# MCG-NJU/MeMOTR

Hardware: AMD Instinct MI355X
Metric: train_frames_per_sec (higher is better)
Workload: dtype f32

## Files before the change

include/clip_ops_hip.h:

```cpp
#ifndef CLIP_OPS_HIP_H
#define CLIP_OPS_HIP_H

#include <stdint.h>

#ifdef __cplusplus
extern "C" {
#endif

#define CLIPOPS_ABI_VERSION 12

int clipops_abi_version(void);
const char *clipops_last_error(void);

int clipops_match_cost_f32(const float *logits, long logit_sl, long logit_sq, const float *boxes, long box_sl,
                           long box_sq, const int64_t *gt_labels, const float *gt_boxes, int n_layers, int Q, int K,
                           int T, float w_class, float w_bbox, float w_giou, float *cost, void *stream);

int clipops_pair_box_loss_fwd_f32(const float *boxes, const int64_t *lay, const int64_t *qidx, long row_mul,
                                  long row_add, const float *tgt_boxes, const int64_t *gidx, const float *weight,
                                  int n, float *l1, float *giou_loss, void *stream);
int clipops_pair_box_loss_bwd_f32(const float *boxes, const int64_t *lay, const int64_t *qidx, long row_mul,
                                  long row_add, const float *tgt_boxes, const int64_t *gidx, const float *weight,
                                  int n, const float *grad_l1, const float *grad_giou, float *grad_boxes,
                                  void *stream);

int clipops_pair_iou_f32(const float *boxes, const float *tgt_boxes, const int64_t *gidx, int n, float *iou,
                         void *stream);

int clipops_track_ownership_i64(const int64_t *track_ids, int n_tracks, const int64_t *gt_ids, int n_gt,
                                int64_t *matched_idx, float *gt_free, void *stream);
int clipops_focal_labels_i64(const int64_t *lay, const int64_t *q, const int64_t *g, int n_pairs,
                             const int64_t *gt_labels, int n_gt, const int64_t *matched_idx, int n_tracks,
                             const uint8_t *late, int n_layers, int n_det, int K, int64_t *labels, void *stream);

int clipops_focal_fwd_f32(const float *logits, long sl, long sq, const int64_t *labels, int n_layers, int Nq, int K,
                          float alpha, float gamma, float *loss, void *stream);
int clipops_focal_bwd_f32(const float *logits, long sl, long sq, const int64_t *labels, int n_layers, int Nq, int K,
                          float alpha, float gamma, const float *grad_loss, float *grad_logits, void *stream);

int clipops_sine_embed_fwd_f32(const float *pos, const float *dim_t, long n, int K, int F, float scale, float *out,
                               void *stream);
int clipops_sine_embed_bwd_f32(const float *pos, const float *dim_t, long n, int K, int F, float scale,
                               const float *grad_out, float *grad_pos, void *stream);

int clipops_inverse_sigmoid_fwd_f32(const float *x, long n, float eps, float *y, void *stream);
int clipops_inverse_sigmoid_bwd_f32(const float *x, const float *grad_y, long n, float eps, float *grad_x, void *stream);

int clipops_refine_boxes_fwd_f32(const float *delta, const float *ref, long n, float eps, float *out, void *stream);
int clipops_refine_boxes_bwd_f32(const float *out, const float *ref, const float *grad_out, long n, float eps,
                                 float *grad_delta, float *grad_ref, void *stream);

int clipops_refine_boxes_split_fwd_f32(const float *delta, const float *ref, long n_rows, float eps,
                                       float *out_head, float *out_dec, void *stream);

int clipops_colsum_f32(const float *x, long rows, int cols, float *out, void *stream);
int clipops_colsum_partial_f32(const float *x, long rows, int cols, int chunk_rows, float *partial, void *stream);
int clipops_colsum_partial_bf16(const uint16_t *x, long rows, int cols, int chunk_rows, float *partial, void *stream);

#define CLIPOPS_MHA_MAX_L 512
int clipops_mha_fwd_f32(const float *q, const float *k, const float *v, long q_bs, long q_rs, long k_bs, long k_rs,
                        long v_bs, long v_rs, const uint8_t *key_mask, int B, int H, int L, float scale, float *out,
                        float *lse, void *stream);
int clipops_mha_bwd_f32(const float *q, const float *k, const float *v, long q_bs, long q_rs, long k_bs, long k_rs,
                        long v_bs, long v_rs, const uint8_t *key_mask, const float *out, const float *lse,
                        const float *grad_out, int B, int H, int L, float scale, float *grad_q, long gq_bs, long gq_rs,
                        float *grad_k, long gk_bs, long gk_rs, float *grad_v, long gv_bs, long gv_rs, void *stream);

#define CLIPOPS_LN_COLS 256
int clipops_add_layer_norm_fwd_f32(const float *x, const float *res, const float *gamma, const float *beta, long rows,
                                   float eps, float *sum, float *y, float *stats, void *stream);
int clipops_add_layer_norm_bwd_f32(const float *grad_y, const float *sum, const float *stats, const float *gamma,
                                   long rows, int chunk_rows, float *grad_sum, float *partial, void *stream);

int clipops_add_layer_norm_pos_fwd_f32(const float *x, const float *res, const float *gamma, const float *beta,
                                       const float *pos, long rows, float eps, float *sum, float *y, float *q,
                                       float *stats, void *stream);
int clipops_add_layer_norm_fanin_bwd_f32(const float *g0, const float *g1, const float *g2, const float *sum,
                                         const float *stats, const float *gamma, long rows, int chunk_rows,
                                         float *grad_sum, float *partial, float *colsum_partial, void *stream);

#define CLIPOPS_ASSIGN_MAX_DIM 2048
int clipops_assign_f32(const float *cost, long stride_problem, long stride_row, long stride_col, int n_problems,
                       int n_rows, int n_cols, int32_t *row_ind, int32_t *col_ind, int32_t *status, void *stream);

int clipops_shift_relu_f32(float *x, const float *shift, const float *res, long planes, int C, long HW, void *stream);
int clipops_shift_relu_bf16(uint16_t *x, const float *shift, const uint16_t *res, long planes, int C, long HW,
                            void *stream);

int clipops_linear_bwd_f32(const float *grad_y, const float *y_relu, const float *x, const float *w, int rows,
                           int in_features, int out_features, float *grad_x, float *grad_w, float *grad_b,
                           void *stream);

int clipops_linear_fwd_f32(const float *x, const float *w, const float *bias, int rows, int in_features,
                           int out_features, int relu, float *y, void *stream);

int clipops_relu_bwd_colsum_partial_f32(const float *g, const float *y, long rows, int cols, int chunk_rows, float *g2,
                                        float *partial, void *stream);

int clipops_result_rows_f32(const float *boxes, const float *scores, const int64_t *ids, const int64_t *labels, int n,
                            int K, int64_t frame, float ori_w, float ori_h, float score_thresh, float area_thresh,
                            float *rows_f, int64_t *rows_i, int32_t *counters, int capacity, void *stream);

#ifdef __cplusplus
}
#endif
#endif
```

memotr_amd/_clip_lib.py:

```python
from __future__ import annotations

import ctypes

from . import _cabi

LIB_PATH = _cabi.lib_path("libclip_ops_hip.so")

ABI_VERSION = 12

c_int, c_long, c_float, c_void_p = ctypes.c_int, ctypes.c_long, ctypes.c_float, ctypes.c_void_p

_PAIR = [c_void_p, c_void_p, c_void_p, c_long, c_long, c_void_p, c_void_p, c_void_p, c_int]
_FOCAL = [c_void_p, c_long, c_long, c_void_p, c_int, c_int, c_int, c_float, c_float]

SYMBOLS = {
    "clipops_abi_version": ([], c_int),
    "clipops_last_error": ([], ctypes.c_char_p),
    "clipops_match_cost_f32": ([c_void_p, c_long, c_long, c_void_p, c_long, c_long, c_void_p, c_void_p] + [c_int] * 4 +
                               [c_float] * 3 + [c_void_p, c_void_p], c_int),
    "clipops_pair_box_loss_fwd_f32": (_PAIR + [c_void_p, c_void_p, c_void_p], c_int),
    "clipops_pair_box_loss_bwd_f32": (_PAIR + [c_void_p, c_void_p, c_void_p, c_void_p], c_int),
    "clipops_pair_iou_f32": ([c_void_p, c_void_p, c_void_p, c_int, c_void_p, c_void_p], c_int),
    "clipops_track_ownership_i64": ([c_void_p, c_int, c_void_p, c_int, c_void_p, c_void_p, c_void_p], c_int),
    "clipops_focal_labels_i64": ([c_void_p, c_void_p, c_void_p, c_int, c_void_p, c_int, c_void_p, c_int, c_void_p, c_int,
                                  c_int, c_int, c_void_p, c_void_p], c_int),
    "clipops_focal_fwd_f32": (_FOCAL + [c_void_p, c_void_p], c_int),
    "clipops_focal_bwd_f32": (_FOCAL + [c_void_p, c_void_p, c_void_p], c_int),
    "clipops_colsum_f32": ([c_void_p, c_long, c_int, c_void_p, c_void_p], c_int),
    "clipops_colsum_partial_f32": ([c_void_p, c_long, c_int, c_int, c_void_p, c_void_p], c_int),
    "clipops_colsum_partial_bf16": ([c_void_p, c_long, c_int, c_int, c_void_p, c_void_p], c_int),
    "clipops_assign_f32": ([c_void_p, c_long, c_long, c_long, c_int, c_int, c_int, c_void_p, c_void_p, c_void_p,
                            c_void_p], c_int),
    "clipops_mha_fwd_f32": ([c_void_p] * 3 + [c_long] * 6 + [c_void_p] + [c_int] * 3 + [c_float, c_void_p, c_void_p,
                                                                                          c_void_p], c_int),
    "clipops_mha_bwd_f32": ([c_void_p] * 3 + [c_long] * 6 + [c_void_p] * 4 + [c_int] * 3 + [c_float] +
                            [c_void_p, c_long, c_long] * 3 + [c_void_p], c_int),
    "clipops_add_layer_norm_fwd_f32": ([c_void_p] * 4 + [c_long, c_float] + [c_void_p] * 4, c_int),
    "clipops_add_layer_norm_bwd_f32": ([c_void_p] * 4 + [c_long, c_int] + [c_void_p] * 3, c_int),
    "clipops_add_layer_norm_pos_fwd_f32": ([c_void_p] * 5 + [c_long, c_float] + [c_void_p] * 5, c_int),
    "clipops_add_layer_norm_fanin_bwd_f32": ([c_void_p] * 6 + [c_long, c_int] + [c_void_p] * 4, c_int),
    "clipops_sine_embed_fwd_f32": ([c_void_p, c_void_p, c_long, c_int, c_int, c_float, c_void_p, c_void_p], c_int),
    "clipops_sine_embed_bwd_f32": ([c_void_p, c_void_p, c_long, c_int, c_int, c_float, c_void_p, c_void_p, c_void_p],
                                   c_int),
    "clipops_inverse_sigmoid_fwd_f32": ([c_void_p, c_long, c_float, c_void_p, c_void_p], c_int),
    "clipops_inverse_sigmoid_bwd_f32": ([c_void_p, c_void_p, c_long, c_float, c_void_p, c_void_p], c_int),
    "clipops_refine_boxes_fwd_f32": ([c_void_p, c_void_p, c_long, c_float, c_void_p, c_void_p], c_int),
    "clipops_linear_bwd_f32": ([c_void_p] * 4 + [c_int] * 3 + [c_void_p] * 4, c_int),
    "clipops_linear_fwd_f32": ([c_void_p] * 3 + [c_int] * 4 + [c_void_p, c_void_p], c_int),
    "clipops_relu_bwd_colsum_partial_f32": ([c_void_p, c_void_p, c_long, c_int, c_int, c_void_p, c_void_p, c_void_p], c_int),
    "clipops_shift_relu_f32": ([c_void_p, c_void_p, c_void_p, c_long, c_int, c_long, c_void_p], c_int),
    "clipops_shift_relu_bf16": ([c_void_p, c_void_p, c_void_p, c_long, c_int, c_long, c_void_p], c_int),
    "clipops_refine_boxes_bwd_f32": ([c_void_p, c_void_p, c_void_p, c_long, c_float, c_void_p, c_void_p, c_void_p],
                                     c_int),
    "clipops_refine_boxes_split_fwd_f32": ([c_void_p, c_void_p, c_long, c_float, c_void_p, c_void_p, c_void_p], c_int),
    "clipops_result_rows_f32": ([c_void_p] * 4 + [c_int, c_int, ctypes.c_int64] + [c_float] * 4 + [c_void_p] * 3 +
                                [c_int, c_void_p], c_int),
}


lib, check = _cabi.bind("libclip_ops_hip.so", "clipops", SYMBOLS, ABI_VERSION)
```

memotr_amd/csrc/clip_ops.hip:

```cpp
#include <hip/hip_runtime.h>
#include <stdint.h>
#include <stdio.h>

#include <atomic>

#include "../../include/clip_ops_hip.h"
#include "assign_core.h"

namespace {

thread_local char g_err[256] = {0};

int fail(int code, const char *msg) {
    snprintf(g_err, sizeof(g_err), "%s", msg);
    return code;
}

int check_launch(const char *what) {
    const hipError_t e = hipGetLastError();
    if (e != hipSuccess) {
        snprintf(g_err, sizeof(g_err), "%s: %s", what, hipGetErrorString(e));
        return (int)e;
    }
    g_err[0] = 0;
    return 0;
}

typedef float f32x4_t __attribute__((ext_vector_type(4)));
typedef double f64x4_t __attribute__((ext_vector_type(4)));

struct Box {
    float x1, y1, x2, y2;
};

__device__ __forceinline__ Box to_xyxy(float cx, float cy, float w, float h) {
#pragma clang fp contract(off)
    Box b;
    b.x1 = cx - 0.5f * w;
    b.y1 = cy - 0.5f * h;
    b.x2 = cx + 0.5f * w;
    b.y2 = cy + 0.5f * h;
    return b;
}

__device__ __forceinline__ float giou_pair(const Box a, const Box b) {
#pragma clang fp contract(off)
    const float iw = fmaxf(fminf(a.x2, b.x2) - fmaxf(a.x1, b.x1), 0.f);
    const float ih = fmaxf(fminf(a.y2, b.y2) - fmaxf(a.y1, b.y1), 0.f);
    const float inter = iw * ih;
    const float area_a = (a.x2 - a.x1) * (a.y2 - a.y1);
    const float area_b = (b.x2 - b.x1) * (b.y2 - b.y1);
    const float uni = area_a + area_b - inter;
    const float iou = inter / uni;
    const float hw = fmaxf(fmaxf(a.x2, b.x2) - fminf(a.x1, b.x1), 0.f);
    const float hh = fmaxf(fmaxf(a.y2, b.y2) - fminf(a.y1, b.y1), 0.f);
    const float hull = hw * hh;
    return iou - (hull - uni) / hull;
}

__device__ __forceinline__ float sigmoidf(float x) { return 1.f / (1.f + expf(-x)); }

__device__ __forceinline__ float powg(float x, float gamma) { return gamma == 2.f ? x * x : powf(x, gamma); }

__global__ __launch_bounds__(256) void match_cost_kernel(const float *__restrict__ logits, long lsl, long lsq,
                                                        const float *__restrict__ boxes, long bsl, long bsq,
                                                        const int64_t *__restrict__ gt_labels,
                                                        const float *__restrict__ gt_boxes, int n_layers, int Q,
                                                        int K, int T, float w_class, float w_bbox, float w_giou,
                                                        float *__restrict__ cost) {
#pragma clang fp contract(off)
    const long total = (long)n_layers * Q * T;
    for (long i = (long)blockIdx.x * blockDim.x + threadIdx.x; i < total; i += (long)gridDim.x * blockDim.x) {
        const int t = (int)(i % T);
        const long lq = i / T;
        const int q = (int)(lq % Q), l = (int)(lq / Q);
        long lab = gt_labels[t];
        lab = lab < 0 ? 0 : (lab >= K ? K - 1 : lab);
        const float prob = sigmoidf(logits[l * lsl + q * lsq + lab]);
        const float alpha = 0.25f, gamma = 2.f;
        const float neg = ((1.f - alpha) * powg(prob, gamma)) * (-logf(1.f - prob + 1e-8f));
        const float pos = (alpha * powg(1.f - prob, gamma)) * (-logf(prob + 1e-8f));
        const float c_class = pos - neg;
        const float *pb = boxes + l * bsl + q * bsq;
        const float *tb = gt_boxes + (long)t * 4;
        const float p0 = pb[0], p1 = pb[1], p2 = pb[2], p3 = pb[3];
        const float t0 = tb[0], t1 = tb[1], t2 = tb[2], t3 = tb[3];
        const float c_bbox = ((fabsf(p0 - t0) + fabsf(p1 - t1)) + fabsf(p2 - t2)) + fabsf(p3 - t3);
        const float giou = giou_pair(to_xyxy(p0, p1, p2, p3), to_xyxy(t0, t1, t2, t3));
        cost[i] = (w_bbox * c_bbox + w_class * c_class) + w_giou * (-giou);
    }
}

__global__ __launch_bounds__(256) void pair_box_loss_fwd_kernel(const float *__restrict__ boxes,
                                                               const int64_t *__restrict__ lay,
                                                               const int64_t *__restrict__ qidx, long row_mul,
                                                               long row_add, const float *__restrict__ tgt,
                                                               const int64_t *__restrict__ gidx,
                                                               const float *__restrict__ weight, int n,
                                                               float *__restrict__ l1, float *__restrict__ gl) {
#pragma clang fp contract(off)
    const int i = blockIdx.x * blockDim.x + threadIdx.x;
    if (i >= n) return;
    const float *pb = boxes + (lay[i] * row_mul + row_add + qidx[i]) * 4;
    const float *tb = tgt + (gidx ? gidx[i] : (long)i) * 4;
    const float p0 = pb[0], p1 = pb[1], p2 = pb[2], p3 = pb[3];
    const float t0 = tb[0], t1 = tb[1], t2 = tb[2], t3 = tb[3];
    float a = ((fabsf(p0 - t0) + fabsf(p1 - t1)) + fabsf(p2 - t2)) + fabsf(p3 - t3);
    float g = 1.f - giou_pair(to_xyxy(p0, p1, p2, p3), to_xyxy(t0, t1, t2, t3));
    if (weight) {
        a *= weight[i];
        g *= weight[i];
    }
    l1[i] = a;
    gl[i] = g;
}

__global__ __launch_bounds__(256) void pair_iou_kernel(const float *__restrict__ boxes, const float *__restrict__ tgt,
                                                      const int64_t *__restrict__ gidx, int n,
                                                      float *__restrict__ iou) {
#pragma clang fp contract(off)
    const int i = blockIdx.x * blockDim.x + threadIdx.x;
    if (i >= n) return;
    const float *pb = boxes + (long)i * 4;
    const float *tb = tgt + (gidx ? gidx[i] : (long)i) * 4;
    const Box a = to_xyxy(pb[0], pb[1], pb[2], pb[3]), b = to_xyxy(tb[0], tb[1], tb[2], tb[3]);
    const float iw = fmaxf(fminf(a.x2, b.x2) - fmaxf(a.x1, b.x1), 0.f);
    const float ih = fmaxf(fminf(a.y2, b.y2) - fmaxf(a.y1, b.y1), 0.f);
    const float inter = iw * ih;
    const float uni = (a.x2 - a.x1) * (a.y2 - a.y1) + (b.x2 - b.x1) * (b.y2 - b.y1) - inter;
    iou[i] = inter / uni;
}

__device__ __forceinline__ float dmax_a(float a, float b) { return a > b ? 1.f : (a == b ? 0.5f : 0.f); }
__device__ __forceinline__ float dmin_a(float a, float b) { return a < b ? 1.f : (a == b ? 0.5f : 0.f); }
__device__ __forceinline__ float sgn(float x) { return x > 0.f ? 1.f : (x < 0.f ? -1.f : 0.f); }

__global__ __launch_bounds__(256) void pair_box_loss_bwd_kernel(const float *__restrict__ boxes,
                                                               const int64_t *__restrict__ lay,
                                                               const int64_t *__restrict__ qidx, long row_mul,
                                                               long row_add, const float *__restrict__ tgt,
                                                               const int64_t *__restrict__ gidx,
                                                               const float *__restrict__ weight, int n,
                                                               const float *__restrict__ g_l1,
                                                               const float *__restrict__ g_gl,
                                                               float *__restrict__ grad_boxes) {
    const int i = blockIdx.x * blockDim.x + threadIdx.x;
    if (i >= n) return;
    const long row = lay[i] * row_mul + row_add + qidx[i];
    const float *pb = boxes + row * 4;
    const float *tb = tgt + (gidx ? gidx[i] : (long)i) * 4;
    const float p0 = pb[0], p1 = pb[1], p2 = pb[2], p3 = pb[3];
    const float t0 = tb[0], t1 = tb[1], t2 = tb[2], t3 = tb[3];
    const float w = weight ? weight[i] : 1.f;
    const float ga = g_l1[i] * w;
    const float gg = -g_gl[i] * w;
    const Box a = to_xyxy(p0, p1, p2, p3), b = to_xyxy(t0, t1, t2, t3);
    const float ltx = fmaxf(a.x1, b.x1), lty = fmaxf(a.y1, b.y1), rbx = fminf(a.x2, b.x2), rby = fminf(a.y2, b.y2);
    const float dw = rbx - ltx, dh = rby - lty;
    const float iw = fmaxf(dw, 0.f), ih = fmaxf(dh, 0.f);
    const float inter = iw * ih;
    const float aw = a.x2 - a.x1, ah = a.y2 - a.y1;
    const float area_a = aw * ah, area_b = (b.x2 - b.x1) * (b.y2 - b.y1);
    const float uni = area_a + area_b - inter;
    const float hx1 = fminf(a.x1, b.x1), hy1 = fminf(a.y1, b.y1), hx2 = fmaxf(a.x2, b.x2), hy2 = fmaxf(a.y2, b.y2);
    const float ew = hx2 - hx1, eh = hy2 - hy1;
    const float hw = fmaxf(ew, 0.f), hh = fmaxf(eh, 0.f);
    const float hull = hw * hh;
    const float g_inter0 = gg / uni;
    const float g_uni = gg * (-inter / (uni * uni)) + gg / hull;
    const float g_hull = gg * (-(uni / (hull * hull)));
    const float g_inter = g_inter0 - g_uni;
    const float g_area_a = g_uni;
    const float g_dw = g_inter * ih * (dw >= 0.f ? 1.f : 0.f), g_dh = g_inter * iw * (dh >= 0.f ? 1.f : 0.f);
    const float g_ew = g_hull * hh * (ew >= 0.f ? 1.f : 0.f), g_eh = g_hull * hw * (eh >= 0.f ? 1.f : 0.f);
    float gx1 = -g_dw * dmax_a(a.x1, b.x1) - g_ew * dmin_a(a.x1, b.x1) - g_area_a * ah;
    float gy1 = -g_dh * dmax_a(a.y1, b.y1) - g_eh * dmin_a(a.y1, b.y1) - g_area_a * aw;
    float gx2 = g_dw * dmin_a(a.x2, b.x2) + g_ew * dmax_a(a.x2, b.x2) + g_area_a * ah;
    float gy2 = g_dh * dmin_a(a.y2, b.y2) + g_eh * dmax_a(a.y2, b.y2) + g_area_a * aw;
    float *go = grad_boxes + row * 4;
    go[0] = (gx1 + gx2) + ga * sgn(p0 - t0);
    go[1] = (gy1 + gy2) + ga * sgn(p1 - t1);
    go[2] = 0.5f * (gx2 - gx1) + ga * sgn(p2 - t2);
    go[3] = 0.5f * (gy2 - gy1) + ga * sgn(p3 - t3);
}

struct Focal {
    float loss, dloss;
};

__device__ __forceinline__ Focal focal_elem(float x, bool is_pos, float alpha, float gamma) {
    const float p = sigmoidf(x);
    const float ce = fmaxf(x, 0.f) - (is_pos ? x : 0.f) + log1pf(expf(-fabsf(x)));
    const float p_t = is_pos ? p : 1.f - p;
    const float q = 1.f - p_t;
    const float a_t = alpha >= 0.f ? (is_pos ? alpha : 1.f - alpha) : 1.f;
    const float mod = powg(q, gamma);
    Focal f;
    f.loss = a_t * (ce * mod);
    const float qg1 = gamma == 2.f ? q : (gamma == 0.f ? 0.f : powf(q, gamma - 1.f));
    const float d = a_t * (gamma * qg1 * (p_t * q) * ce + mod * q);
    f.dloss = is_pos ? -d : d;
    return f;
}

__global__ __launch_bounds__(256) void focal_fwd_kernel(const float *__restrict__ logits, long sl, long sq,
                                                       const int64_t *__restrict__ labels, int Nq, int K, float alpha,
                                                       float gamma, float *__restrict__ loss) {
    __shared__ float s_part[256];
    const int l = blockIdx.x;
    const int total = Nq * K;
    float acc = 0.f;
    for (int i = threadIdx.x; i < total; i += 256) {
        const int q = i / K, k = i - q * K;
        const float x = logits[l * sl + q * sq + k];
        acc += focal_elem(x, labels[(long)l * Nq + q] == k, alpha, gamma).loss;
    }
    s_part[threadIdx.x] = acc;
    __syncthreads();
    for (int o = 128; o > 0; o >>= 1) {
        if (threadIdx.x < o) s_part[threadIdx.x] += s_part[threadIdx.x + o];
        __syncthreads();
    }
    if (threadIdx.x == 0) loss[l] = s_part[0] / (float)K;
}

__global__ __launch_bounds__(256) void focal_bwd_kernel(const float *__restrict__ logits, long sl, long sq,
                                                       const int64_t *__restrict__ labels, int n_layers, int Nq,
                                                       int K, float alpha, float gamma,
                                                       const float *__restrict__ g_loss,
                                                       float *__restrict__ grad_logits) {
    const long total = (long)n_layers * Nq * K;
    for (long i = (long)blockIdx.x * blockDim.x + threadIdx.x; i < total; i += (long)gridDim.x * blockDim.x) {
        const int k = (int)(i % K);
        const long lq = i / K;
        const int q = (int)(lq % Nq), l = (int)(lq / Nq);
        const float x = logits[l * sl + q * sq + k];
        const Focal f = focal_elem(x, labels[lq] == k, alpha, gamma);
        grad_logits[i] = (g_loss[l] / (float)K) * f.dloss;
    }
}

__global__ __launch_bounds__(256) void sine_embed_fwd_kernel(const float *__restrict__ pos,
                                                            const float *__restrict__ dim_t, long n, int K, int F,
                                                            float scale, float *__restrict__ out) {
#pragma clang fp contract(off)
    const long total = n * K * F;
    for (long i = (long)blockIdx.x * blockDim.x + threadIdx.x; i < total; i += (long)gridDim.x * blockDim.x) {
        const int j = (int)(i % F);
        const long ik = i / F;
        const float e = (pos[ik] * scale) / dim_t[j];
        out[i] = (j & 1) ? cosf(e) : sinf(e);
    }
}

__global__ __launch_bounds__(256) void sine_embed_bwd_kernel(const float *__restrict__ pos,
                                                            const float *__restrict__ dim_t, long n, int K, int F,
                                                            float scale, const float *__restrict__ g,
                                                            float *__restrict__ gpos) {
    const int lane = threadIdx.x & 63;
    const long waves = ((long)gridDim.x * blockDim.x) >> 6;
    for (long ik = ((long)blockIdx.x * blockDim.x + threadIdx.x) >> 6; ik < n * K; ik += waves) {
        const float ps = pos[ik] * scale;
        float acc = 0.f;
        for (int j = lane; j < F; j += 64) {
            const float e = ps / dim_t[j];
            const float d = (j & 1) ? -sinf(e) : cosf(e);
            acc += (g[ik * F + j] * d) / dim_t[j];
        }
#pragma unroll
        for (int o = 32; o > 0; o >>= 1) acc += __shfl_xor(acc, o, 64);
        if (lane == 0) gpos[ik] = acc * scale;
    }
}

__device__ __forceinline__ float clamp_keep_nan(float x, float lo, float hi) { return x < lo ? lo : (x > hi ? hi : x); }

__device__ __forceinline__ float inv_sigmoid(float x, float eps) {
    return logf(clamp_keep_nan(x, eps, 1.f) / clamp_keep_nan(1.f - x, eps, 1.f));
}

__device__ __forceinline__ float inv_sigmoid_grad(float x, float eps) {
    const float u = 1.f - x;
    const float x1 = clamp_keep_nan(x, eps, 1.f), x2 = clamp_keep_nan(u, eps, 1.f);
    const float a = (x >= eps && x <= 1.f) ? 1.f / x1 : 0.f;
    const float b = (u >= eps && u <= 1.f) ? 1.f / x2 : 0.f;
    return a + b;
}

__global__ __launch_bounds__(256) void inverse_sigmoid_fwd_kernel(const float *__restrict__ x, long n, float eps,
                                                                 float *__restrict__ y) {
    for (long i = (long)blockIdx.x * blockDim.x + threadIdx.x; i < n; i += (long)gridDim.x * blockDim.x)
        y[i] = inv_sigmoid(x[i], eps);
}

__global__ __launch_bounds__(256) void inverse_sigmoid_bwd_kernel(const float *__restrict__ x,
                                                                 const float *__restrict__ g, long n, float eps,
                                                                 float *__restrict__ gx) {
    for (long i = (long)blockIdx.x * blockDim.x + threadIdx.x; i < n; i += (long)gridDim.x * blockDim.x)
        gx[i] = g[i] * inv_sigmoid_grad(x[i], eps);
}

__global__ __launch_bounds__(256) void refine_boxes_fwd_kernel(const float *__restrict__ delta,
                                                              const float *__restrict__ ref, long n, float eps,
                                                              float *__restrict__ out) {
    for (long i = (long)blockIdx.x * blockDim.x + threadIdx.x; i < n; i += (long)gridDim.x * blockDim.x)
        out[i] = sigmoidf(delta[i] + inv_sigmoid(ref[i], eps));
}

template <bool VEC>
__global__ __launch_bounds__(256) void refine_boxes_split_fwd_kernel(const float *__restrict__ delta,
                                                                    const float *__restrict__ ref, long n_rows,
                                                                    float eps, float *__restrict__ head,
                                                                    float *__restrict__ dec) {
    for (long r = (long)blockIdx.x * blockDim.x + threadIdx.x; r < n_rows; r += (long)gridDim.x * blockDim.x) {
        float4 d, f;
        if (VEC) {
            d = reinterpret_cast<const float4 *>(delta)[r];
            f = reinterpret_cast<const float4 *>(ref)[r];
        } else {
            d = make_float4(delta[4 * r], delta[4 * r + 1], delta[4 * r + 2], delta[4 * r + 3]);
            f = make_float4(ref[4 * r], ref[4 * r + 1], ref[4 * r + 2], ref[4 * r + 3]);
        }
        float4 h, c;
        h.x = sigmoidf(d.x + inv_sigmoid(f.x, eps));
        h.y = sigmoidf(d.y + inv_sigmoid(f.y, eps));
        h.z = sigmoidf(d.z + inv_sigmoid(f.z, eps));
        h.w = sigmoidf(d.w + inv_sigmoid(f.w, eps));
        c.x = h.x;
        c.y = h.y;
        c.z = sigmoidf(d.z);
        c.w = sigmoidf(d.w);
        if (VEC) {
            reinterpret_cast<float4 *>(head)[r] = h;
            reinterpret_cast<float4 *>(dec)[r] = c;
        } else {
            head[4 * r] = h.x; head[4 * r + 1] = h.y; head[4 * r + 2] = h.z; head[4 * r + 3] = h.w;
            dec[4 * r] = c.x; dec[4 * r + 1] = c.y; dec[4 * r + 2] = c.z; dec[4 * r + 3] = c.w;
        }
    }
}

__global__ __launch_bounds__(256) void refine_boxes_bwd_kernel(const float *__restrict__ out,
                                                              const float *__restrict__ ref,
                                                              const float *__restrict__ g, long n, float eps,
                                                              float *__restrict__ gdelta, float *__restrict__ gref) {
    for (long i = (long)blockIdx.x * blockDim.x + threadIdx.x; i < n; i += (long)gridDim.x * blockDim.x) {
        const float y = out[i];
        const float gs = (g[i] * (1.f - y)) * y;
        gdelta[i] = gs;
        if (gref) gref[i] = gs * inv_sigmoid_grad(ref[i], eps);
    }
}

__global__ __launch_bounds__(256) void colsum_kernel(const float *__restrict__ x, long rows, int cols,
                                                    float *__restrict__ out) {
    __shared__ double s_part[8][33];
    const int tx = threadIdx.x & 31, ty = threadIdx.x >> 5;
    const int c = blockIdx.x * 32 + tx;
    double a0 = 0., a1 = 0., a2 = 0., a3 = 0.;
    if (c < cols) {
        long r = ty;
        for (; r + 24 < rows; r += 32) {
            a0 += x[r * cols + c];
            a1 += x[(r + 8) * cols + c];
            a2 += x[(r + 16) * cols + c];
            a3 += x[(r + 24) * cols + c];
        }
        for (; r < rows; r += 8) a0 += x[r * cols + c];
    }
    s_part[ty][tx] = (a0 + a1) + (a2 + a3);
    __syncthreads();
    if (ty == 0 && c < cols) {
        double t = s_part[0][tx];
#pragma unroll
        for (int i = 1; i < 8; ++i) t += s_part[i][tx];
        out[c] = (float)t;
    }
}

__global__ __launch_bounds__(256) void colsum_quad_kernel(const float *__restrict__ x, long rows, int cols,
                                                         float *__restrict__ out) {
    __shared__ f64x4_t s_w[4];
    const int c = blockIdx.x * 4;
    f64x4_t a = {0., 0., 0., 0.};
    for (long r = threadIdx.x; r < rows; r += 256) {
        const f32x4_t v = *reinterpret_cast<const f32x4_t *>(x + r * cols + c);
        a.x += v.x; a.y += v.y; a.z += v.z; a.w += v.w;
    }
#pragma unroll
    for (int o = 32; o > 0; o >>= 1) {
        a.x += __shfl_xor(a.x, o, 64);
        a.y += __shfl_xor(a.y, o, 64);
        a.z += __shfl_xor(a.z, o, 64);
        a.w += __shfl_xor(a.w, o, 64);
    }
    if ((threadIdx.x & 63) == 0) s_w[threadIdx.x >> 6] = a;
    __syncthreads();
    if (threadIdx.x == 0) {
        const f64x4_t t = (s_w[0] + s_w[1]) + (s_w[2] + s_w[3]);
        const f32x4_t r = {(float)t.x, (float)t.y, (float)t.z, (float)t.w};
        *reinterpret_cast<f32x4_t *>(out + c) = r;
    }
}

__device__ __forceinline__ float colsum_ld(const float *x, long i) { return x[i]; }
__device__ __forceinline__ float colsum_ld(const uint16_t *x, long i) {
    return __uint_as_float(((unsigned)x[i]) << 16);
}

template <typename TX>
__global__ __launch_bounds__(256) void colsum_partial_kernel(const TX *__restrict__ x, long rows, int cols,
                                                            int chunk_rows, float *__restrict__ partial) {
    __shared__ double s_part[8][33];
    const int tx = threadIdx.x & 31, ty = threadIdx.x >> 5;
    const int c = blockIdx.x * 32 + tx;
    const long r0 = (long)blockIdx.y * chunk_rows;
    const long r1 = r0 + chunk_rows < rows ? r0 + chunk_rows : rows;
    double a0 = 0., a1 = 0., a2 = 0., a3 = 0.;
    if (c < cols) {
        long r = r0 + ty;
        for (; r + 24 < r1; r += 32) {
            a0 += colsum_ld(x, r * cols + c);
            a1 += colsum_ld(x, (r + 8) * cols + c);
            a2 += colsum_ld(x, (r + 16) * cols + c);
            a3 += colsum_ld(x, (r + 24) * cols + c);
        }
        for (; r < r1; r += 8) a0 += colsum_ld(x, r * cols + c);
    }
    s_part[ty][tx] = (a0 + a1) + (a2 + a3);
    __syncthreads();
    if (ty == 0 && c < cols) {
        double t = s_part[0][tx];
#pragma unroll
        for (int i = 1; i < 8; ++i) t += s_part[i][tx];
        partial[(long)blockIdx.y * cols + c] = (float)t;
    }
}

__device__ __forceinline__ void colsum_st(float *x, long i, float v) { x[i] = v; }

template <typename TX>
__global__ __launch_bounds__(256) void relu_bwd_colsum_partial_kernel(const TX *__restrict__ g, const TX *__restrict__ y,
                                                                     long rows, int cols, int chunk_rows,
                                                                     TX *__restrict__ g2, float *__restrict__ partial) {
    __shared__ double s_part[8][33];
    const int tx = threadIdx.x & 31, ty = threadIdx.x >> 5;
    const int c = blockIdx.x * 32 + tx;
    const long r0 = (long)blockIdx.y * chunk_rows;
    const long r1 = r0 + chunk_rows < rows ? r0 + chunk_rows : rows;
    double a0 = 0., a1 = 0., a2 = 0., a3 = 0.;
    if (c < cols) {
        long r = r0 + ty;
        for (; r + 24 < r1; r += 32) {
            const long i0 = r * cols + c, i1 = (r + 8) * cols + c, i2 = (r + 16) * cols + c, i3 = (r + 24) * cols + c;
            const float v0 = colsum_ld(y, i0) <= 0.f ? 0.f : colsum_ld(g, i0);
            const float v1 = colsum_ld(y, i1) <= 0.f ? 0.f : colsum_ld(g, i1);
            const float v2 = colsum_ld(y, i2) <= 0.f ? 0.f : colsum_ld(g, i2);
            const float v3 = colsum_ld(y, i3) <= 0.f ? 0.f : colsum_ld(g, i3);
            colsum_st(g2, i0, v0); colsum_st(g2, i1, v1); colsum_st(g2, i2, v2); colsum_st(g2, i3, v3);
            a0 += v0; a1 += v1; a2 += v2; a3 += v3;
        }
        for (; r < r1; r += 8) {
            const long i0 = r * cols + c;
            const float v0 = colsum_ld(y, i0) <= 0.f ? 0.f : colsum_ld(g, i0);
            colsum_st(g2, i0, v0);
            a0 += v0;
        }
    }
    s_part[ty][tx] = (a0 + a1) + (a2 + a3);
    __syncthreads();
    if (ty == 0 && c < cols) {
        double t = s_part[0][tx];
#pragma unroll
        for (int i = 1; i < 8; ++i) t += s_part[i][tx];
        partial[(long)blockIdx.y * cols + c] = (float)t;
    }
}

constexpr int kLanes = 16;
constexpr int kRows = 256 / kLanes;
constexpr int kHd = 32;
constexpr int kPitch = 36;

__device__ __forceinline__ void load_row32(const float *p, float *r) {
#pragma unroll
    for (int i = 0; i < 8; ++i) {
        const f32x4_t v = *reinterpret_cast<const f32x4_t *>(p + 4 * i);
        r[4 * i] = v.x; r[4 * i + 1] = v.y; r[4 * i + 2] = v.z; r[4 * i + 3] = v.w;
    }
}

__device__ __forceinline__ float dot32(const float *a, const float *lds_row) {
    float s0 = 0.f, s1 = 0.f;
#pragma unroll
    for (int i = 0; i < 8; ++i) {
        const f32x4_t v = *reinterpret_cast<const f32x4_t *>(lds_row + 4 * i);
        s0 = fmaf(a[4 * i], v.x, s0);
        s1 = fmaf(a[4 * i + 1], v.y, s1);
        s0 = fmaf(a[4 * i + 2], v.z, s0);
        s1 = fmaf(a[4 * i + 3], v.w, s1);
    }
    return s0 + s1;
}

__device__ __forceinline__ float dot32r(const float *a, const float *b) {
    float s0 = 0.f, s1 = 0.f;
#pragma unroll
    for (int i = 0; i < 8; ++i) {
        s0 = fmaf(a[4 * i], b[4 * i], s0);
        s1 = fmaf(a[4 * i + 1], b[4 * i + 1], s1);
        s0 = fmaf(a[4 * i + 2], b[4 * i + 2], s0);
        s1 = fmaf(a[4 * i + 3], b[4 * i + 3], s1);
    }
    return s0 + s1;
}

__device__ __forceinline__ void axpy32(float *acc, float w, const float *lds_row) {
#pragma unroll
    for (int i = 0; i < 8; ++i) {
        const f32x4_t v = *reinterpret_cast<const f32x4_t *>(lds_row + 4 * i);
        acc[4 * i] = fmaf(w, v.x, acc[4 * i]);
        acc[4 * i + 1] = fmaf(w, v.y, acc[4 * i + 1]);
        acc[4 * i + 2] = fmaf(w, v.z, acc[4 * i + 2]);
        acc[4 * i + 3] = fmaf(w, v.w, acc[4 * i + 3]);
    }
}

__device__ __forceinline__ float sum8l(float x) {
#pragma unroll
    for (int o = 1; o < kLanes; o <<= 1) x += __shfl_xor(x, o, 64);
    return x;
}
__device__ __forceinline__ float max8l(float x) {
#pragma unroll
    for (int o = 1; o < kLanes; o <<= 1) x = fmaxf(x, __shfl_xor(x, o, 64));
    return x;
}

__device__ __forceinline__ void stage_rows(float *dst, const float *src, long rs, int L) {
    for (int i = threadIdx.x; i < L * 8; i += blockDim.x) {
        const int r = i >> 3, c = (i & 7) * 4;
        *reinterpret_cast<f32x4_t *>(dst + r * kPitch + c) = *reinterpret_cast<const f32x4_t *>(src + r * rs + c);
    }
}

__global__ __launch_bounds__(256) void mha_fwd_kernel(const float *__restrict__ q, const float *__restrict__ k,
                                                     const float *__restrict__ v, long q_bs, long q_rs, long k_bs,
                                                     long k_rs, long v_bs, long v_rs,
                                                     const uint8_t *__restrict__ key_mask, int H, int L, float scale,
                                                     float *__restrict__ out, float *__restrict__ lse) {
    extern __shared__ __attribute__((aligned(16))) float s_mem[];
    float *Ks = s_mem, *Vs = s_mem + (size_t)L * kPitch;
    const int h = blockIdx.y, b = blockIdx.z;
    stage_rows(Ks, k + b * k_bs + h * kHd, k_rs, L);
    stage_rows(Vs, v + b * v_bs + h * kHd, v_rs, L);
    __syncthreads();
    const int row = blockIdx.x * kRows + threadIdx.x / kLanes, sub = threadIdx.x % kLanes;
    const bool row_ok = row < L;
    const int rowc = row_ok ? row : L - 1;
    float qr[kHd];
    load_row32(q + b * q_bs + rowc * q_rs + h * kHd, qr);
#pragma unroll
    for (int i = 0; i < kHd; ++i) qr[i] *= scale;
    const uint8_t *mk = key_mask ? key_mask + (long)b * L : nullptr;
    float m = -INFINITY, l = 0.f, acc[kHd];
#pragma unroll
    for (int i = 0; i < kHd; ++i) acc[i] = 0.f;
    for (int j = sub; j < L; j += kLanes) {
        if (mk && mk[j]) continue;
        const float s = dot32(qr, Ks + j * kPitch);
        const float m_new = fmaxf(m, s);
        const float corr = expf(m - m_new), p = expf(s - m_new);
        l = l * corr + p;
#pragma unroll
        for (int i = 0; i < kHd; ++i) acc[i] *= corr;
        axpy32(acc, p, Vs + j * kPitch);
        m = m_new;
    }
    const float M = max8l(m);
    const float w = (m == -INFINITY) ? 0.f : expf(m - M);
    const float Lsum = sum8l(l * w);
    const float inv = 1.f / Lsum;
    float *o = out + ((long)b * L + rowc) * (H * kHd) + h * kHd;
#pragma unroll
    for (int i = 0; i < kHd; ++i) {
        const float t = sum8l(acc[i] * w) * inv;
        if (row_ok && (i >> 2) == sub) o[i] = t;
    }
    if (row_ok && sub == 0) lse[((long)b * H + h) * L + row] = M + logf(Lsum);
}

__global__ __launch_bounds__(256) void mha_bwd_q_kernel(const float *__restrict__ q, const float *__restrict__ k,
                                                       const float *__restrict__ v, long q_bs, long q_rs, long k_bs,
                                                       long k_rs, long v_bs, long v_rs,
                                                       const uint8_t *__restrict__ key_mask,
                                                       const float *__restrict__ out, const float *__restrict__ lse,
                                                       const float *__restrict__ go, int H, int L, float scale,
                                                       float *__restrict__ gq, long gq_bs, long gq_rs) {
    extern __shared__ __attribute__((aligned(16))) float s_mem[];
    float *Ks = s_mem, *Vs = s_mem + (size_t)L * kPitch;
    const int h = blockIdx.y, b = blockIdx.z;
    stage_rows(Ks, k + b * k_bs + h * kHd, k_rs, L);
    stage_rows(Vs, v + b * v_bs + h * kHd, v_rs, L);
    __syncthreads();
    const int row = blockIdx.x * kRows + threadIdx.x / kLanes, sub = threadIdx.x % kLanes;
    const bool row_ok = row < L;
    const int rowc = row_ok ? row : L - 1;
    float qr[kHd], gr[kHd], acc[kHd];
    load_row32(q + b * q_bs + rowc * q_rs + h * kHd, qr);
    const long orow = ((long)b * L + rowc) * (H * kHd) + h * kHd;
    load_row32(go + orow, gr);
    float D = 0.f;
    {
        float orr[kHd];
        load_row32(out + orow, orr);
        D = dot32r(gr, orr);
    }
#pragma unroll
    for (int i = 0; i < kHd; ++i) { qr[i] *= scale; acc[i] = 0.f; }
    const float ls = lse[((long)b * H + h) * L + rowc];
    const uint8_t *mk = key_mask ? key_mask + (long)b * L : nullptr;
    for (int j = sub; j < L; j += kLanes) {
        if (mk && mk[j]) continue;
        const float p = expf(dot32(qr, Ks + j * kPitch) - ls);
        const float ds = p * (dot32(gr, Vs + j * kPitch) - D);
        axpy32(acc, ds, Ks + j * kPitch);
    }
    float *g = gq + b * gq_bs + rowc * gq_rs + h * kHd;
#pragma unroll
    for (int i = 0; i < kHd; ++i) {
        const float t = sum8l(acc[i]) * scale;
        if (row_ok && (i >> 2) == sub) g[i] = t;
    }
}

__global__ __launch_bounds__(256) void mha_bwd_kv_kernel(const float *__restrict__ q, const float *__restrict__ k,
                                                        const float *__restrict__ v, long q_bs, long q_rs, long k_bs,
                                                        long k_rs, long v_bs, long v_rs,
                                                        const uint8_t *__restrict__ key_mask,
                                                        const float *__restrict__ out, const float *__restrict__ lse,
                                                        const float *__restrict__ go, int H, int L, float scale,
                                                        float *__restrict__ gk, long gk_bs, long gk_rs,
                                                        float *__restrict__ gv, long gv_bs, long gv_rs) {
    extern __shared__ __attribute__((aligned(16))) float s_mem[];
    float *Qs = s_mem, *Gs = s_mem + (size_t)L * kPitch;
    float *s_lse = Gs + (size_t)L * kPitch, *s_D = s_lse + L;
    const int h = blockIdx.y, b = blockIdx.z;
    stage_rows(Qs, q + b * q_bs + h * kHd, q_rs, L);
    for (int i = threadIdx.x; i < L * 8; i += blockDim.x) {
        f32x4_t *p4 = reinterpret_cast<f32x4_t *>(Qs + (i >> 3) * kPitch + (i & 7) * 4);
        *p4 = *p4 * scale;
    }
    stage_rows(Gs, go + (long)b * L * (H * kHd) + h * kHd, (long)H * kHd, L);
    for (int i = threadIdx.x; i < L; i += blockDim.x) s_lse[i] = lse[((long)b * H + h) * L + i];
    __syncthreads();
    for (int i = threadIdx.x; i < L; i += blockDim.x) {
        const float *o = out + ((long)b * L + i) * (H * kHd) + h * kHd;
        float orr[kHd];
        load_row32(o, orr);
        s_D[i] = dot32(orr, Gs + i * kPitch);
    }
    __syncthreads();
    const int row = blockIdx.x * kRows + threadIdx.x / kLanes, sub = threadIdx.x % kLanes;
    const bool row_ok = row < L;
    const int rowc = row_ok ? row : L - 1;
    const bool dead = key_mask && key_mask[(long)b * L + rowc];
    float kr[kHd], vr[kHd], ak[kHd], av[kHd];
    load_row32(k + b * k_bs + rowc * k_rs + h * kHd, kr);
    load_row32(v + b * v_bs + rowc * v_rs + h * kHd, vr);
#pragma unroll
    for (int i = 0; i < kHd; ++i) { ak[i] = 0.f; av[i] = 0.f; }
    if (!dead) {
        for (int i = sub; i < L; i += kLanes) {
            const float p = expf(dot32(kr, Qs + i * kPitch) - s_lse[i]);
            const float ds = p * (dot32(vr, Gs + i * kPitch) - s_D[i]);
            axpy32(av, p, Gs + i * kPitch);
            axpy32(ak, ds, Qs + i * kPitch);
        }
    }
    float *pk = gk + b * gk_bs + rowc * gk_rs + h * kHd, *pv = gv + b * gv_bs + rowc * gv_rs + h * kHd;
#pragma unroll
    for (int i = 0; i < kHd; ++i) {
        const float tk = sum8l(ak[i]), tv = sum8l(av[i]);
        if (row_ok && (i >> 2) == sub) {
            pk[i] = tk;
            pv[i] = tv;
        }
    }
}

int allow_lds(const void *kernel, size_t lds, std::atomic<unsigned long long> &done) {
    if (lds <= 64 * 1024) return 0;
    int dev = 0;
    (void)hipGetDevice(&dev);
    const unsigned long long bit = 1ull << (dev & 63);
    if (done.load(std::memory_order_acquire) & bit) return 0;
    const hipError_t e = hipFuncSetAttribute(kernel, hipFuncAttributeMaxDynamicSharedMemorySize, 160 * 1024 - 2048);
    if (e != hipSuccess) {
        snprintf(g_err, sizeof(g_err), "hipFuncSetAttribute: %s", hipGetErrorString(e));
        return (int)e;
    }
    done.fetch_or(bit, std::memory_order_release);
    return 0;
}

std::atomic<unsigned long long> g_lds_fwd{0}, g_lds_bq{0}, g_lds_bkv{0};

int mha_check(const void *q, const void *k, const void *v, int B, int H, int L) {
    if (B < 0 || H <= 0 || L < 0) return fail(1, "clipops_mha: bad dimension");
    if (L > CLIPOPS_MHA_MAX_L) return fail(2, "clipops_mha: L exceeds CLIPOPS_MHA_MAX_L");
    if ((long)B * L > 0 && (!q || !k || !v)) return fail(1, "clipops_mha: null pointer");
    return 0;
}

__device__ __forceinline__ float wave_sum64(float x) {
#pragma unroll
    for (int o = 32; o > 0; o >>= 1) x += __shfl_xor(x, o, 64);
    return x;
}

template <bool WITH_Q>
__global__ __launch_bounds__(256) void add_layer_norm_fwd_kernel(const float *__restrict__ x,
                                                                const float *__restrict__ res,
                                                                const float *__restrict__ gamma,
                                                                const float *__restrict__ beta,
                                                                const float *__restrict__ pos, long rows, float eps,
                                                                float *__restrict__ sum, float *__restrict__ y,
                                                                float *__restrict__ q, float *__restrict__ stats) {
    const int lane = threadIdx.x & 63;
    const long row = (long)blockIdx.x * 4 + (threadIdx.x >> 6);
    if (row >= rows) return;
    const long off = row * CLIPOPS_LN_COLS + lane * 4;
    const f32x4_t a = *reinterpret_cast<const f32x4_t *>(x + off);
    const f32x4_t b = *reinterpret_cast<const f32x4_t *>(res + off);
    const f32x4_t s = a + b;
    *reinterpret_cast<f32x4_t *>(sum + off) = s;
    const float mean = wave_sum64((s.x + s.y) + (s.z + s.w)) * (1.f / CLIPOPS_LN_COLS);
    const f32x4_t d = s - mean;
    const float var = wave_sum64((d.x * d.x + d.y * d.y) + (d.z * d.z + d.w * d.w)) * (1.f / CLIPOPS_LN_COLS);
    const float rstd = rsqrtf(var + eps);
    const f32x4_t g = *reinterpret_cast<const f32x4_t *>(gamma + lane * 4);
    const f32x4_t be = *reinterpret_cast<const f32x4_t *>(beta + lane * 4);
    const f32x4_t yv = (d * rstd) * g + be;
    *reinterpret_cast<f32x4_t *>(y + off) = yv;
    if (WITH_Q) *reinterpret_cast<f32x4_t *>(q + off) = yv + *reinterpret_cast<const f32x4_t *>(pos + off);
    if (lane == 0) {
        stats[2 * row] = mean;
        stats[2 * row + 1] = rstd;
    }
}

__global__ __launch_bounds__(256) void add_layer_norm_bwd_kernel(const float *__restrict__ gy,
                                                                const float *__restrict__ sum,
                                                                const float *__restrict__ stats,
                                                                const float *__restrict__ gamma, long rows,
                                                                int chunk_rows, float *__restrict__ gsum,
                                                                float *__restrict__ partial) {
    __shared__ f32x4_t s_acc[4][2][64];
    const int lane = threadIdx.x & 63, wave = threadIdx.x >> 6;
    const f32x4_t gm = *reinterpret_cast<const f32x4_t *>(gamma + lane * 4);
    f32x4_t acc_g = {0.f, 0.f, 0.f, 0.f}, acc_b = {0.f, 0.f, 0.f, 0.f};
    const long r0 = (long)blockIdx.x * chunk_rows;
    const long r1 = r0 + chunk_rows < rows ? r0 + chunk_rows : rows;
    for (long row = r0 + wave; row < r1; row += 4) {
        const long off = row * CLIPOPS_LN_COLS + lane * 4;
        const f32x4_t g = *reinterpret_cast<const f32x4_t *>(gy + off);
        const f32x4_t s = *reinterpret_cast<const f32x4_t *>(sum + off);
        const float mean = stats[2 * row], rstd = stats[2 * row + 1];
        const f32x4_t xh = (s - mean) * rstd;
        const f32x4_t gh = g * gm;
        const float c1 = wave_sum64((gh.x + gh.y) + (gh.z + gh.w)) * (1.f / CLIPOPS_LN_COLS);
        const float c2 = wave_sum64((gh.x * xh.x + gh.y * xh.y) + (gh.z * xh.z + gh.w * xh.w)) * (1.f / CLIPOPS_LN_COLS);
        *reinterpret_cast<f32x4_t *>(gsum + off) = (gh - c1 - xh * c2) * rstd;
        acc_g += g * xh;
        acc_b += g;
    }
    s_acc[wave][0][lane] = acc_g;
    s_acc[wave][1][lane] = acc_b;
    __syncthreads();
    if (wave < 2) {
        const f32x4_t t = (s_acc[0][wave][lane] + s_acc[1][wave][lane]) + (s_acc[2][wave][lane] + s_acc[3][wave][lane]);
        *reinterpret_cast<f32x4_t *>(partial + (long)blockIdx.x * 2 * CLIPOPS_LN_COLS + wave * CLIPOPS_LN_COLS + lane * 4) = t;
    }
}

__global__ __launch_bounds__(256) void add_layer_norm_bwd_fanin_kernel(const float *__restrict__ ga,
                                                                      const float *__restrict__ gb,
                                                                      const float *__restrict__ gc,
                                                                      const float *__restrict__ sum,
                                                                      const float *__restrict__ stats,
                                                                      const float *__restrict__ gamma, long rows,
                                                                      int chunk_rows, float *__restrict__ gsum,
                                                                      float *__restrict__ partial,
                                                                      float *__restrict__ zpartial) {
    __shared__ f32x4_t s_acc[4][2][64];
    __shared__ f64x4_t s_z[4][64];
    const int lane = threadIdx.x & 63, wave = threadIdx.x >> 6;
    const f32x4_t gm = *reinterpret_cast<const f32x4_t *>(gamma + lane * 4);
    f32x4_t acc_g = {0.f, 0.f, 0.f, 0.f}, acc_b = {0.f, 0.f, 0.f, 0.f};
    f64x4_t acc_z = {0., 0., 0., 0.};
    const long r0 = (long)blockIdx.x * chunk_rows;
    const long r1 = r0 + chunk_rows < rows ? r0 + chunk_rows : rows;
    for (long row = r0 + wave; row < r1; row += 4) {
        const long off = row * CLIPOPS_LN_COLS + lane * 4;
        f32x4_t g = *reinterpret_cast<const f32x4_t *>(ga + off);
        if (gb) g += *reinterpret_cast<const f32x4_t *>(gb + off);
        if (gc) g += *reinterpret_cast<const f32x4_t *>(gc + off);
        const f32x4_t s = *reinterpret_cast<const f32x4_t *>(sum + off);
        const float mean = stats[2 * row], rstd = stats[2 * row + 1];
        const f32x4_t xh = (s - mean) * rstd;
        const f32x4_t gh = g * gm;
        const float c1 = wave_sum64((gh.x + gh.y) + (gh.z + gh.w)) * (1.f / CLIPOPS_LN_COLS);
        const float c2 = wave_sum64((gh.x * xh.x + gh.y * xh.y) + (gh.z * xh.z + gh.w * xh.w)) * (1.f / CLIPOPS_LN_COLS);
        const f32x4_t dz = (gh - c1 - xh * c2) * rstd;
        *reinterpret_cast<f32x4_t *>(gsum + off) = dz;
        acc_g += g * xh;
        acc_b += g;
        acc_z.x += dz.x; acc_z.y += dz.y; acc_z.z += dz.z; acc_z.w += dz.w;
    }
    s_acc[wave][0][lane] = acc_g;
    s_acc[wave][1][lane] = acc_b;
    s_z[wave][lane] = acc_z;
    __syncthreads();
    if (wave < 2) {
        const f32x4_t t = (s_acc[0][wave][lane] + s_acc[1][wave][lane]) + (s_acc[2][wave][lane] + s_acc[3][wave][lane]);
        *reinterpret_cast<f32x4_t *>(partial + (long)blockIdx.x * 2 * CLIPOPS_LN_COLS + wave * CLIPOPS_LN_COLS + lane * 4) = t;
    } else if (wave == 2) {
        const f64x4_t t = (s_z[0][lane] + s_z[1][lane]) + (s_z[2][lane] + s_z[3][lane]);
        const f32x4_t hi = {(float)t.x, (float)t.y, (float)t.z, (float)t.w};
        const f32x4_t lo = {(float)(t.x - (double)hi.x), (float)(t.y - (double)hi.y), (float)(t.z - (double)hi.z),
                            (float)(t.w - (double)hi.w)};
        float *zp = zpartial + (long)blockIdx.x * 2 * CLIPOPS_LN_COLS + lane * 4;
        *reinterpret_cast<f32x4_t *>(zp) = hi;
        *reinterpret_cast<f32x4_t *>(zp + CLIPOPS_LN_COLS) = lo;
    }
}

using assign::WaveLanes;

__global__ __launch_bounds__(64) void assign_kernel(const float *__restrict__ cost, long stride_p, long stride_r,
                                                    long stride_c, int n_rows, int n_cols,
                                                    int32_t *__restrict__ row_ind, int32_t *__restrict__ col_ind,
                                                    int32_t *__restrict__ status) {
#pragma clang fp contract(off)
    extern __shared__ __attribute__((aligned(16))) unsigned char s_assign[];
    const long p = blockIdx.x;
    const int k = n_rows < n_cols ? n_rows : n_cols;
    const WaveLanes lanes{(int)threadIdx.x};
    const int rc = assign::solve_problem(lanes, cost + p * stride_p, stride_r, stride_c, n_rows, n_cols, s_assign,
                                         row_ind + p * k, col_ind + p * k);
    if (threadIdx.x == 0 && status != nullptr) status[p] = rc;
}

int grid_for(long total) {
    long g = (total + 255) / 256;
    if (g < 1) g = 1;
    return (int)(g > 4096 ? 4096 : g);
}


__device__ __forceinline__ float sr_bf16(uint16_t h) { return __uint_as_float((unsigned)h << 16); }
__device__ __forceinline__ uint16_t sr_to_bf16(float f) {
    unsigned u = __float_as_uint(f);
    if ((u & 0x7fffffffu) > 0x7f800000u) return (uint16_t)((u >> 16) | 0x40u);
    return (uint16_t)((u + 0x7fffu + ((u >> 16) & 1u)) >> 16);
}

template <bool RES>
__global__ __launch_bounds__(256) void shift_relu_f32_kernel(float *__restrict__ x, const float *__restrict__ shift,
                                                             const float *__restrict__ res, long planes, int C, long HW,
                                                             int vec) {
    for (long plane = blockIdx.y; plane < planes; plane += gridDim.y) {
        const float b = shift[plane % C];
        float *xp = x + plane * HW;
        const float *rp = RES ? res + plane * HW : nullptr;
        if (vec) {
            const long n4 = HW >> 2;
            for (long i = (long)blockIdx.x * blockDim.x + threadIdx.x; i < n4; i += (long)gridDim.x * blockDim.x) {
                float4 v = reinterpret_cast<float4 *>(xp)[i];
                if (RES) {
                    const float4 r = reinterpret_cast<const float4 *>(rp)[i];
                    v.x = (v.x + b) + r.x; v.y = (v.y + b) + r.y; v.z = (v.z + b) + r.z; v.w = (v.w + b) + r.w;
                } else {
                    v.x += b; v.y += b; v.z += b; v.w += b;
                }
                v.x = v.x < 0.f ? 0.f : v.x; v.y = v.y < 0.f ? 0.f : v.y;
                v.z = v.z < 0.f ? 0.f : v.z; v.w = v.w < 0.f ? 0.f : v.w;
                reinterpret_cast<float4 *>(xp)[i] = v;
            }
        } else {
            for (long i = (long)blockIdx.x * blockDim.x + threadIdx.x; i < HW; i += (long)gridDim.x * blockDim.x) {
                float v = xp[i] + b;
                if (RES) v += rp[i];
                xp[i] = v < 0.f ? 0.f : v;
            }
        }
    }
}

template <bool RES>
__global__ __launch_bounds__(256) void shift_relu_bf16_kernel(uint16_t *__restrict__ x, const float *__restrict__ shift,
                                                              const uint16_t *__restrict__ res, long planes, int C,
                                                              long HW, int vec) {
    for (long plane = blockIdx.y; plane < planes; plane += gridDim.y) {
        const float b = sr_bf16(sr_to_bf16(shift[plane % C]));
        uint16_t *xp = x + plane * HW;
        const uint16_t *rp = RES ? res + plane * HW : nullptr;
        if (vec) {
            const long n8 = HW >> 3;
            for (long i = (long)blockIdx.x * blockDim.x + threadIdx.x; i < n8; i += (long)gridDim.x * blockDim.x) {
                uint4 v = reinterpret_cast<uint4 *>(xp)[i];
                uint4 r = {0u, 0u, 0u, 0u};
                if (RES) r = reinterpret_cast<const uint4 *>(rp)[i];
                unsigned *vw = reinterpret_cast<unsigned *>(&v);
                const unsigned *rw = reinterpret_cast<const unsigned *>(&r);
#pragma unroll
                for (int k = 0; k < 4; ++k) {
                    float lo = sr_bf16((uint16_t)(vw[k] & 0xffffu)) + b, hi = sr_bf16((uint16_t)(vw[k] >> 16)) + b;
                    if (RES) {
                        lo = sr_bf16(sr_to_bf16(lo)) + sr_bf16((uint16_t)(rw[k] & 0xffffu));
                        hi = sr_bf16(sr_to_bf16(hi)) + sr_bf16((uint16_t)(rw[k] >> 16));
                    }
                    lo = lo < 0.f ? 0.f : lo;
                    hi = hi < 0.f ? 0.f : hi;
                    vw[k] = (unsigned)sr_to_bf16(lo) | ((unsigned)sr_to_bf16(hi) << 16);
                }
                reinterpret_cast<uint4 *>(xp)[i] = v;
            }
        } else {
            for (long i = (long)blockIdx.x * blockDim.x + threadIdx.x; i < HW; i += (long)gridDim.x * blockDim.x) {
                float v = sr_bf16(xp[i]) + b;
                if (RES) v = sr_bf16(sr_to_bf16(v)) + sr_bf16(rp[i]);
                xp[i] = sr_to_bf16(v < 0.f ? 0.f : v);
            }
        }
    }
}


typedef float lb_f32x16 __attribute__((ext_vector_type(16)));

#ifndef MSDA_LB_U
#define MSDA_LB_U 4
#endif
constexpr int LB_U = MSDA_LB_U;

template <bool GX, bool RELU>
__device__ __forceinline__ void linear_bwd_tile(const float *__restrict__ g, const float *__restrict__ y,
                                                const float *__restrict__ Bp, int M, int N, int K, int OUT, int i0, int j0,
                                                float *__restrict__ C, float *__restrict__ gb, float (*s_c)[16][64],
                                                float (*s_b)[32]) {
    const int lane = threadIdx.x & 63, wave = threadIdx.x >> 6;
    const int i = i0 + (lane & 31), j = j0 + (lane & 31), kq = (lane >> 5) * 4;
    const bool iok = i < M, jok = j < N;
    const int chunks = (K + 7) / 8, per = (chunks + 3) / 4;
    const int c_lo = wave * per, c_hi = (c_lo + per) < chunks ? (c_lo + per) : chunks;
    const bool vec = GX && (OUT % 4 == 0);
    lb_f32x16 acc = {0.f, 0.f, 0.f, 0.f, 0.f, 0.f, 0.f, 0.f, 0.f, 0.f, 0.f, 0.f, 0.f, 0.f, 0.f, 0.f};
    float bsum = 0.f;
    for (int c = c_lo; c < c_hi; c += LB_U) {
        float a[LB_U][4], b[LB_U][4], m[LB_U][4];
#pragma unroll
        for (int u = 0; u < LB_U; ++u) {
            const int k0 = (c + u) * 8 + kq;
            const bool cok = c + u < c_hi;
            if (vec) {
                float4 av = {0.f, 0.f, 0.f, 0.f}, mv = {1.f, 1.f, 1.f, 1.f};
                if (cok && iok && k0 < K) {
                    av = *reinterpret_cast<const float4 *>(g + (long)i * OUT + k0);
                    if (RELU) mv = *reinterpret_cast<const float4 *>(y + (long)i * OUT + k0);
                }
                a[u][0] = av.x; a[u][1] = av.y; a[u][2] = av.z; a[u][3] = av.w;
                m[u][0] = mv.x; m[u][1] = mv.y; m[u][2] = mv.z; m[u][3] = mv.w;
            }
#pragma unroll
            for (int q = 0; q < 4; ++q) {
                const int k = k0 + q;
                const bool kok = cok && k < K;
                if (!vec) {
                    const long idx = GX ? (long)i * OUT + k : (long)k * OUT + i;
                    a[u][q] = (iok && kok) ? g[idx] : 0.f;
                    m[u][q] = (RELU && iok && kok) ? y[idx] : 1.f;
                }
                b[u][q] = (jok && kok) ? Bp[(long)k * N + j] : 0.f;
            }
        }
#pragma unroll
        for (int u = 0; u < LB_U; ++u) {
#pragma unroll
            for (int q = 0; q < 4; ++q) {
                const float av = RELU ? (m[u][q] <= 0.f ? 0.f : a[u][q]) : a[u][q];
                acc = __builtin_amdgcn_mfma_f32_32x32x2f32(av, b[u][q], acc, 0, 0, 0);
                bsum += av;
            }
        }
    }
#pragma unroll
    for (int r = 0; r < 16; ++r) s_c[wave][r][lane] = acc[r];
    bsum += __shfl_xor(bsum, 32, 64);
    if (lane < 32) s_b[wave][lane] = bsum;
    __syncthreads();
#pragma unroll
    for (int rr = 0; rr < 4; ++rr) {
        const int r = wave * 4 + rr;
        const float v = (s_c[0][r][lane] + s_c[1][r][lane]) + (s_c[2][r][lane] + s_c[3][r][lane]);
        const int row = i0 + (r & 3) + 8 * (r >> 2) + 4 * (lane >> 5);
        if (row < M && jok) C[(long)row * N + j] = v;
    }
    if (!GX && gb != nullptr && j0 == 0 && wave == 0 && lane < 32 && i0 + lane < M)
        gb[i0 + lane] = (s_b[0][lane] + s_b[1][lane]) + (s_b[2][lane] + s_b[3][lane]);
}

template <bool RELU>
__global__ __launch_bounds__(256) void linear_bwd_kernel(const float *__restrict__ g, const float *__restrict__ y,
                                                         const float *__restrict__ x, const float *__restrict__ w,
                                                         int R, int IN, int OUT, float *__restrict__ gx,
                                                         float *__restrict__ gw, float *__restrict__ gb, int n_gx,
                                                         int gx_tj, int gw_tj) {
    __shared__ float s_c[4][16][64];
    __shared__ float s_b[4][32];
    const int tile = blockIdx.x;
    if (tile < n_gx) {
        linear_bwd_tile<true, RELU>(g, y, w, R, IN, OUT, OUT, (tile / gx_tj) * 32, (tile % gx_tj) * 32, gx, nullptr, s_c, s_b);
    } else {
        const int t = tile - n_gx;
        linear_bwd_tile<false, RELU>(g, y, x, OUT, IN, R, OUT, (t / gw_tj) * 32, (t % gw_tj) * 32, gw, gb, s_c, s_b);
    }
}

template <bool RELU>
__global__ __launch_bounds__(256) void linear_fwd_kernel(const float *__restrict__ x, const float *__restrict__ w,
                                                         const float *__restrict__ bias, int R, int IN, int OUT,
                                                         float *__restrict__ yout, int tj) {
    __shared__ float s_c[4][16][64];
    const int lane = threadIdx.x & 63, wave = threadIdx.x >> 6;
    const int i0 = (blockIdx.x / tj) * 32, j0 = (blockIdx.x % tj) * 32;
    const int i = i0 + (lane & 31), j = j0 + (lane & 31), kq = (lane >> 5) * 4;
    const bool iok = i < R, jok = j < OUT;
    const int chunks = (IN + 7) / 8, per = (chunks + 3) / 4;
    const int c_lo = wave * per, c_hi = (c_lo + per) < chunks ? (c_lo + per) : chunks;
    lb_f32x16 acc = {0.f, 0.f, 0.f, 0.f, 0.f, 0.f, 0.f, 0.f, 0.f, 0.f, 0.f, 0.f, 0.f, 0.f, 0.f, 0.f};
    for (int c = c_lo; c < c_hi; c += LB_U) {
        float4 a[LB_U], b[LB_U];
#pragma unroll
        for (int u = 0; u < LB_U; ++u) {
            const int k0 = (c + u) * 8 + kq;
            const bool kok = c + u < c_hi && k0 < IN;
            a[u] = (iok && kok) ? *reinterpret_cast<const float4 *>(x + (long)i * IN + k0) : float4{0.f, 0.f, 0.f, 0.f};
            b[u] = (jok && kok) ? *reinterpret_cast<const float4 *>(w + (long)j * IN + k0) : float4{0.f, 0.f, 0.f, 0.f};
        }
#pragma unroll
        for (int u = 0; u < LB_U; ++u) {
            acc = __builtin_amdgcn_mfma_f32_32x32x2f32(a[u].x, b[u].x, acc, 0, 0, 0);
            acc = __builtin_amdgcn_mfma_f32_32x32x2f32(a[u].y, b[u].y, acc, 0, 0, 0);
            acc = __builtin_amdgcn_mfma_f32_32x32x2f32(a[u].z, b[u].z, acc, 0, 0, 0);
            acc = __builtin_amdgcn_mfma_f32_32x32x2f32(a[u].w, b[u].w, acc, 0, 0, 0);
        }
    }
#pragma unroll
    for (int r = 0; r < 16; ++r) s_c[wave][r][lane] = acc[r];
    __syncthreads();
    const float bj = (bias != nullptr && jok) ? bias[j] : 0.f;
#pragma unroll
    for (int rr = 0; rr < 4; ++rr) {
        const int r = wave * 4 + rr;
        float v = ((s_c[0][r][lane] + s_c[1][r][lane]) + (s_c[2][r][lane] + s_c[3][r][lane])) + bj;
        if (RELU) v = v < 0.f ? 0.f : v;
        const int row = i0 + (r & 3) + 8 * (r >> 2) + 4 * (lane >> 5);
        if (row < R && jok) yout[(long)row * OUT + j] = v;
    }
}

}

__global__ __launch_bounds__(256) void track_ownership_kernel(const int64_t *__restrict__ tr_ids, int n_tr,
                                                              const int64_t *__restrict__ gt_ids, int n_gt,
                                                              int64_t *__restrict__ matched, float *__restrict__ free_out) {
    for (int i = threadIdx.x; i < n_tr; i += blockDim.x) {
        const int64_t id = tr_ids[i];
        int64_t m = -1;
        for (int j = 0; j < n_gt; ++j)
            if (gt_ids[j] == id) m = j;
        matched[i] = m;
    }
    for (int j = threadIdx.x; j < n_gt; j += blockDim.x) {
        const int64_t id = gt_ids[j];
        bool owned = false;
        for (int i = 0; i < n_tr; ++i) owned = owned || tr_ids[i] == id;
        free_out[j] = owned ? 0.f : 1.f;
    }
}

__global__ __launch_bounds__(256) void focal_labels_kernel(const int64_t *__restrict__ lay, const int64_t *__restrict__ q,
                                                           const int64_t *__restrict__ g, int n_pairs,
                                                           const int64_t *__restrict__ gt_labels, int n_gt,
                                                           const int64_t *__restrict__ matched, int n_tr,
                                                           const unsigned char *__restrict__ late, int n_layers, int nd,
                                                           int K, int64_t *__restrict__ labels) {
    const int nq = nd + n_tr;
    for (int e = threadIdx.x; e < n_layers * nq; e += blockDim.x) {
        const int l = e / nq, c = e - l * nq;
        int64_t v = K;
        if (c >= nd && late[l]) {
            const int64_t m = matched[c - nd];
            if (m >= 0 && m < n_gt) v = gt_labels[m];
        }
        labels[e] = v;
    }
    __syncthreads();
    for (int p = threadIdx.x; p < n_pairs; p += blockDim.x) {
        const int64_t l = lay[p], c = q[p], t = g[p];
        if (l >= 0 && l < n_layers && c >= 0 && c < nq && t >= 0 && t < n_gt) labels[l * nq + c] = gt_labels[t];
    }
}

__global__ __launch_bounds__(256) void result_rows_kernel(const float *__restrict__ boxes, const float *__restrict__ scores,
                                                          const int64_t *__restrict__ ids,
                                                          const int64_t *__restrict__ labels, int n, int K, int64_t frame,
                                                          float ori_w, float ori_h, float score_thresh, float area_thresh,
                                                          float *__restrict__ rows_f, int64_t *__restrict__ rows_i,
                                                          int32_t *__restrict__ counters, int capacity) {
    __shared__ int wave_total[4];
    const int lane = threadIdx.x & 63, wave = threadIdx.x >> 6;
    const int stored0 = counters[0], dropped0 = counters[1];
    int base = 0;
    for (int c0 = 0; c0 < n; c0 += 256) {
        const int i = c0 + (int)threadIdx.x;
        bool keep = false;
        float s = 0.f, cx = 0.f, cy = 0.f, w = 0.f, h = 0.f;
        if (i < n) {
            const float *sc = scores + (long)i * K;
            s = sc[0];
            for (int k = 1; k < K; ++k) {
                const float v = sc[k];
                if (v > s || v != v) s = v;
            }
            cx = boxes[4 * i], cy = boxes[4 * i + 1], w = boxes[4 * i + 2], h = boxes[4 * i + 3];
            const float area = __fmul_rn(__fmul_rn(__fmul_rn(w, ori_w), h), ori_h);
            keep = s > score_thresh && area > area_thresh;
        }
        const unsigned long long m = __ballot(keep);
        const int below = __popcll(m & ((1ull << lane) - 1ull));
        if (lane == 0) wave_total[wave] = __popcll(m);
        __syncthreads();
        int before = 0, total = 0;
        for (int v = 0; v < 4; ++v) {
            const int t = wave_total[v];
            before += v < wave ? t : 0;
            total += t;
        }
        if (keep) {
            const long pos = (long)stored0 + base + before + below;
            if (pos >= 0 && pos < capacity) {
                const float hw = __fmul_rn(0.5f, w), hh = __fmul_rn(0.5f, h);
                float *rf = rows_f + pos * 5;
                rf[0] = __fmul_rn(__fsub_rn(cx, hw), ori_w);
                rf[1] = __fmul_rn(__fsub_rn(cy, hh), ori_h);
                rf[2] = __fmul_rn(__fadd_rn(cx, hw), ori_w);
                rf[3] = __fmul_rn(__fadd_rn(cy, hh), ori_h);
                rf[4] = s;
                int64_t *ri = rows_i + pos * 3;
                ri[0] = frame;
                ri[1] = ids[i];
                ri[2] = labels[i];
            }
        }
        base += total;
        __syncthreads();
    }
    if (threadIdx.x == 0) {
        const int room = stored0 < 0 ? 0 : (capacity > stored0 ? capacity - stored0 : 0);
        const int stored = base < room ? base : room;
        counters[0] = stored0 + stored;
        counters[1] = dropped0 + (base - stored);
    }
}

extern "C" {

int clipops_abi_version(void) { return CLIPOPS_ABI_VERSION; }

int clipops_result_rows_f32(const float *boxes, const float *scores, const int64_t *ids, const int64_t *labels, int n,
                            int K, int64_t frame, float ori_w, float ori_h, float score_thresh, float area_thresh,
                            float *rows_f, int64_t *rows_i, int32_t *counters, int capacity, void *stream) {
    if (n < 0 || capacity < 0) return fail(1, "clipops_result_rows_f32: negative size");
    if (K < 1) return fail(1, "clipops_result_rows_f32: K < 1");
    if (n == 0) { g_err[0] = 0; return 0; }
    if (!boxes || !scores || !ids || !labels || !counters || (capacity > 0 && (!rows_f || !rows_i)))
        return fail(1, "clipops_result_rows_f32: null pointer");
    hipLaunchKernelGGL(result_rows_kernel, dim3(1), dim3(256), 0, (hipStream_t)stream, boxes, scores, ids, labels, n, K,
                       frame, ori_w, ori_h, score_thresh, area_thresh, rows_f, rows_i, counters, capacity);
    return check_launch("result_rows_kernel") ? 3 : 0;
}

const char *clipops_last_error(void) { return g_err; }

int clipops_match_cost_f32(const float *logits, long logit_sl, long logit_sq, const float *boxes, long box_sl,
                           long box_sq, const int64_t *gt_labels, const float *gt_boxes, int n_layers, int Q, int K,
                           int T, float w_class, float w_bbox, float w_giou, float *cost, void *stream) {
    if (n_layers < 0 || Q < 0 || T < 0 || K <= 0) return fail(1, "clipops_match_cost_f32: bad dimension");
    if ((long)n_layers * Q * T == 0) { g_err[0] = 0; return 0; }
    if (!logits || !boxes || !gt_labels || !gt_boxes || !cost) return fail(1, "clipops_match_cost_f32: null pointer");
    hipLaunchKernelGGL(match_cost_kernel, dim3(grid_for((long)n_layers * Q * T)), dim3(256), 0, (hipStream_t)stream,
                       logits, logit_sl, logit_sq, boxes, box_sl, box_sq, gt_labels, gt_boxes, n_layers, Q, K, T,
                       w_class, w_bbox, w_giou, cost);
    return check_launch("match_cost_kernel");
}

int clipops_pair_box_loss_fwd_f32(const float *boxes, const int64_t *lay, const int64_t *qidx, long row_mul,
                                  long row_add, const float *tgt_boxes, const int64_t *gidx, const float *weight,
                                  int n, float *l1, float *giou_loss, void *stream) {
    if (n < 0) return fail(1, "clipops_pair_box_loss_fwd_f32: negative count");
    if (n == 0) { g_err[0] = 0; return 0; }
    if (!boxes || !lay || !qidx || !tgt_boxes || !l1 || !giou_loss)
        return fail(1, "clipops_pair_box_loss_fwd_f32: null pointer");
    hipLaunchKernelGGL(pair_box_loss_fwd_kernel, dim3((n + 255) / 256), dim3(256), 0, (hipStream_t)stream, boxes, lay,
                       qidx, row_mul, row_add, tgt_boxes, gidx, weight, n, l1, giou_loss);
    return check_launch("pair_box_loss_fwd_kernel");
}

int clipops_pair_box_loss_bwd_f32(const float *boxes, const int64_t *lay, const int64_t *qidx, long row_mul,
                                  long row_add, const float *tgt_boxes, const int64_t *gidx, const float *weight,
                                  int n, const float *grad_l1, const float *grad_giou, float *grad_boxes,
                                  void *stream) {
    if (n < 0) return fail(1, "clipops_pair_box_loss_bwd_f32: negative count");
    if (n == 0) { g_err[0] = 0; return 0; }
    if (!boxes || !lay || !qidx || !tgt_boxes || !grad_l1 || !grad_giou || !grad_boxes)
        return fail(1, "clipops_pair_box_loss_bwd_f32: null pointer");
    hipLaunchKernelGGL(pair_box_loss_bwd_kernel, dim3((n + 255) / 256), dim3(256), 0, (hipStream_t)stream, boxes, lay,
                       qidx, row_mul, row_add, tgt_boxes, gidx, weight, n, grad_l1, grad_giou, grad_boxes);
    return check_launch("pair_box_loss_bwd_kernel");
}

int clipops_track_ownership_i64(const int64_t *track_ids, int n_tracks, const int64_t *gt_ids, int n_gt,
                                int64_t *matched_idx, float *gt_free, void *stream) {
    if (n_tracks < 0 || n_gt < 0) return fail(1, "clipops_track_ownership_i64: negative count");
    if (n_tracks + n_gt == 0) { g_err[0] = 0; return 0; }
    if ((n_tracks > 0 && (!track_ids || !matched_idx)) || (n_gt > 0 && (!gt_ids || !gt_free)))
        return fail(1, "clipops_track_ownership_i64: null pointer");
    hipLaunchKernelGGL(track_ownership_kernel, dim3(1), dim3(256), 0, (hipStream_t)stream, track_ids, n_tracks, gt_ids,
                       n_gt, matched_idx, gt_free);
    return check_launch("track_ownership_kernel");
}

int clipops_focal_labels_i64(const int64_t *lay, const int64_t *q, const int64_t *g, int n_pairs,
                             const int64_t *gt_labels, int n_gt, const int64_t *matched_idx, int n_tracks,
                             const uint8_t *late, int n_layers, int n_det, int K, int64_t *labels, void *stream) {
    if (n_pairs < 0 || n_gt < 0 || n_tracks < 0 || n_layers < 0 || n_det < 0) return fail(1, "clipops_focal_labels_i64: negative count");
    if ((long)n_layers * (n_det + n_tracks) == 0) { g_err[0] = 0; return 0; }
    if (!labels || !late || (n_pairs > 0 && (!lay || !q || !g || !gt_labels)) || (n_tracks > 0 && !matched_idx) ||
        (n_gt > 0 && !gt_labels))
        return fail(1, "clipops_focal_labels_i64: null pointer");
    hipLaunchKernelGGL(focal_labels_kernel, dim3(1), dim3(256), 0, (hipStream_t)stream, lay, q, g, n_pairs, gt_labels, n_gt,
                       matched_idx, n_tracks, late, n_layers, n_det, K, labels);
    return check_launch("focal_labels_kernel");
}

int clipops_pair_iou_f32(const float *boxes, const float *tgt_boxes, const int64_t *gidx, int n, float *iou,
                         void *stream) {
    if (n < 0) return fail(1, "clipops_pair_iou_f32: negative count");
    if (n == 0) { g_err[0] = 0; return 0; }
    if (!boxes || !tgt_boxes || !iou) return fail(1, "clipops_pair_iou_f32: null pointer");
    hipLaunchKernelGGL(pair_iou_kernel, dim3((n + 255) / 256), dim3(256), 0, (hipStream_t)stream, boxes, tgt_boxes,
                       gidx, n, iou);
    return check_launch("pair_iou_kernel");
}

int clipops_focal_fwd_f32(const float *logits, long sl, long sq, const int64_t *labels, int n_layers, int Nq, int K,
                          float alpha, float gamma, float *loss, void *stream) {
    if (n_layers < 0 || Nq < 0 || K <= 0) return fail(1, "clipops_focal_fwd_f32: bad dimension");
    if (n_layers == 0) { g_err[0] = 0; return 0; }
    if (!loss || (Nq > 0 && (!logits || !labels))) return fail(1, "clipops_focal_fwd_f32: null pointer");
    hipLaunchKernelGGL(focal_fwd_kernel, dim3(n_layers), dim3(256), 0, (hipStream_t)stream, logits, sl, sq, labels, Nq,
                       K, alpha, gamma, loss);
    return check_launch("focal_fwd_kernel");
}

int clipops_focal_bwd_f32(const float *logits, long sl, long sq, const int64_t *labels, int n_layers, int Nq, int K,
                          float alpha, float gamma, const float *grad_loss, float *grad_logits, void *stream) {
    if (n_layers < 0 || Nq < 0 || K <= 0) return fail(1, "clipops_focal_bwd_f32: bad dimension");
    if ((long)n_layers * Nq == 0) { g_err[0] = 0; return 0; }
    if (!logits || !labels || !grad_loss || !grad_logits) return fail(1, "clipops_focal_bwd_f32: null pointer");
    hipLaunchKernelGGL(focal_bwd_kernel, dim3(grid_for((long)n_layers * Nq * K)), dim3(256), 0, (hipStream_t)stream,
                       logits, sl, sq, labels, n_layers, Nq, K, alpha, gamma, grad_loss, grad_logits);
    return check_launch("focal_bwd_kernel");
}

int clipops_sine_embed_fwd_f32(const float *pos, const float *dim_t, long n, int K, int F, float scale, float *out,
                               void *stream) {
    if (n < 0 || K <= 0 || F <= 0) return fail(1, "clipops_sine_embed_fwd_f32: bad dimension");
    if (n == 0) { g_err[0] = 0; return 0; }
    if (!pos || !dim_t || !out) return fail(1, "clipops_sine_embed_fwd_f32: null pointer");
    hipLaunchKernelGGL(sine_embed_fwd_kernel, dim3(grid_for(n * K * F)), dim3(256), 0, (hipStream_t)stream, pos, dim_t,
                       n, K, F, scale, out);
    return check_launch("sine_embed_fwd_kernel");
}

int clipops_sine_embed_bwd_f32(const float *pos, const float *dim_t, long n, int K, int F, float scale,
                               const float *grad_out, float *grad_pos, void *stream) {
    if (n < 0 || K <= 0 || F <= 0) return fail(1, "clipops_sine_embed_bwd_f32: bad dimension");
    if (n == 0) { g_err[0] = 0; return 0; }
    if (!pos || !dim_t || !grad_out || !grad_pos) return fail(1, "clipops_sine_embed_bwd_f32: null pointer");
    hipLaunchKernelGGL(sine_embed_bwd_kernel, dim3(grid_for(n * K * 64)), dim3(256), 0, (hipStream_t)stream, pos,
                       dim_t, n, K, F, scale, grad_out, grad_pos);
    return check_launch("sine_embed_bwd_kernel");
}

int clipops_inverse_sigmoid_fwd_f32(const float *x, long n, float eps, float *y, void *stream) {
    if (n < 0) return fail(1, "clipops_inverse_sigmoid_fwd_f32: negative count");
    if (n == 0) { g_err[0] = 0; return 0; }
    if (!x || !y) return fail(1, "clipops_inverse_sigmoid_fwd_f32: null pointer");
    hipLaunchKernelGGL(inverse_sigmoid_fwd_kernel, dim3(grid_for(n)), dim3(256), 0, (hipStream_t)stream, x, n, eps, y);
    return check_launch("inverse_sigmoid_fwd_kernel");
}

int clipops_inverse_sigmoid_bwd_f32(const float *x, const float *grad_y, long n, float eps, float *grad_x,
                                    void *stream) {
    if (n < 0) return fail(1, "clipops_inverse_sigmoid_bwd_f32: negative count");
    if (n == 0) { g_err[0] = 0; return 0; }
    if (!x || !grad_y || !grad_x) return fail(1, "clipops_inverse_sigmoid_bwd_f32: null pointer");
    hipLaunchKernelGGL(inverse_sigmoid_bwd_kernel, dim3(grid_for(n)), dim3(256), 0, (hipStream_t)stream, x, grad_y, n,
                       eps, grad_x);
    return check_launch("inverse_sigmoid_bwd_kernel");
}

int clipops_refine_boxes_fwd_f32(const float *delta, const float *ref, long n, float eps, float *out, void *stream) {
    if (n < 0) return fail(1, "clipops_refine_boxes_fwd_f32: negative count");
    if (n == 0) { g_err[0] = 0; return 0; }
    if (!delta || !ref || !out) return fail(1, "clipops_refine_boxes_fwd_f32: null pointer");
    hipLaunchKernelGGL(refine_boxes_fwd_kernel, dim3(grid_for(n)), dim3(256), 0, (hipStream_t)stream, delta, ref, n,
                       eps, out);
    return check_launch("refine_boxes_fwd_kernel");
}

int clipops_refine_boxes_split_fwd_f32(const float *delta, const float *ref, long n_rows, float eps, float *out_head,
                                       float *out_dec, void *stream) {
    if (n_rows < 0) return fail(1, "clipops_refine_boxes_split_fwd_f32: negative count");
    if (n_rows == 0) { g_err[0] = 0; return 0; }
    if (!delta || !ref || !out_head || !out_dec) return fail(1, "clipops_refine_boxes_split_fwd_f32: null pointer");
    if (out_head == out_dec) return fail(1, "clipops_refine_boxes_split_fwd_f32: the two outputs alias");
    const bool vec = (((uintptr_t)delta | (uintptr_t)ref | (uintptr_t)out_head | (uintptr_t)out_dec) & 15) == 0;
    if (vec)
        hipLaunchKernelGGL(refine_boxes_split_fwd_kernel<true>, dim3(grid_for(n_rows)), dim3(256), 0,
                           (hipStream_t)stream, delta, ref, n_rows, eps, out_head, out_dec);
    else
        hipLaunchKernelGGL(refine_boxes_split_fwd_kernel<false>, dim3(grid_for(n_rows)), dim3(256), 0,
                           (hipStream_t)stream, delta, ref, n_rows, eps, out_head, out_dec);
    return check_launch("refine_boxes_split_fwd_kernel");
}

int clipops_refine_boxes_bwd_f32(const float *out, const float *ref, const float *grad_out, long n, float eps,
                                 float *grad_delta, float *grad_ref, void *stream) {
    if (n < 0) return fail(1, "clipops_refine_boxes_bwd_f32: negative count");
    if (n == 0) { g_err[0] = 0; return 0; }
    if (!out || !ref || !grad_out || !grad_delta) return fail(1, "clipops_refine_boxes_bwd_f32: null pointer");
    hipLaunchKernelGGL(refine_boxes_bwd_kernel, dim3(grid_for(n)), dim3(256), 0, (hipStream_t)stream, out, ref,
                       grad_out, n, eps, grad_delta, grad_ref);
    return check_launch("refine_boxes_bwd_kernel");
}

int clipops_colsum_f32(const float *x, long rows, int cols, float *out, void *stream) {
    if (rows < 0 || cols < 0) return fail(1, "clipops_colsum_f32: bad dimension");
    if (cols == 0) { g_err[0] = 0; return 0; }
    if (!out || (rows > 0 && !x)) return fail(1, "clipops_colsum_f32: null pointer");
    if (cols % 4 == 0 && rows <= 2048 && (((uintptr_t)x | (uintptr_t)out) & 15) == 0) {
        hipLaunchKernelGGL(colsum_quad_kernel, dim3(cols / 4), dim3(256), 0, (hipStream_t)stream, x, rows, cols, out);
        return check_launch("colsum_quad_kernel");
    }
    hipLaunchKernelGGL(colsum_kernel, dim3((cols + 31) / 32), dim3(256), 0, (hipStream_t)stream, x, rows, cols, out);
    return check_launch("colsum_kernel");
}

int clipops_colsum_partial_f32(const float *x, long rows, int cols, int chunk_rows, float *partial, void *stream) {
    if (rows < 0 || cols < 0 || chunk_rows <= 0) return fail(1, "clipops_colsum_partial_f32: bad dimension");
    if (cols == 0 || rows == 0) { g_err[0] = 0; return 0; }
    if (!x || !partial) return fail(1, "clipops_colsum_partial_f32: null pointer");
    const long chunks = (rows + chunk_rows - 1) / chunk_rows;
    if (chunks > 65535) return fail(1, "clipops_colsum_partial_f32: too many chunks");
    hipLaunchKernelGGL(colsum_partial_kernel<float>, dim3((cols + 31) / 32, (unsigned)chunks), dim3(256), 0,
                       (hipStream_t)stream, x, rows, cols, chunk_rows, partial);
    return check_launch("colsum_partial_kernel");
}

int clipops_colsum_partial_bf16(const uint16_t *x, long rows, int cols, int chunk_rows, float *partial, void *stream) {
    if (rows < 0 || cols < 0 || chunk_rows <= 0) return fail(1, "clipops_colsum_partial_bf16: bad dimension");
    if (cols == 0 || rows == 0) { g_err[0] = 0; return 0; }
    if (!x || !partial) return fail(1, "clipops_colsum_partial_bf16: null pointer");
    const long chunks = (rows + chunk_rows - 1) / chunk_rows;
    if (chunks > 65535) return fail(1, "clipops_colsum_partial_bf16: too many chunks");
    hipLaunchKernelGGL(colsum_partial_kernel<uint16_t>, dim3((cols + 31) / 32, (unsigned)chunks), dim3(256), 0,
                       (hipStream_t)stream, x, rows, cols, chunk_rows, partial);
    return check_launch("colsum_partial_kernel<bf16>");
}

static int relu_bwd_colsum_check(const void *g, const void *y, const void *g2, const void *partial, long rows, int cols,
                                 int chunk_rows, long *chunks) {
    if (rows < 0 || cols < 0 || chunk_rows <= 0) return fail(1, "clipops_relu_bwd_colsum_partial: bad dimension");
    *chunks = (rows + chunk_rows - 1) / chunk_rows;
    if (cols == 0 || rows == 0) return 0;
    if (!g || !y || !g2 || !partial) return fail(1, "clipops_relu_bwd_colsum_partial: null pointer");
    if (*chunks > 65535) return fail(1, "clipops_relu_bwd_colsum_partial: too many chunks");
    return 0;
}

int clipops_relu_bwd_colsum_partial_f32(const float *g, const float *y, long rows, int cols, int chunk_rows, float *g2,
                                        float *partial, void *stream) {
    long chunks = 0;
    if (relu_bwd_colsum_check(g, y, g2, partial, rows, cols, chunk_rows, &chunks)) return 1;
    if (cols == 0 || rows == 0) { g_err[0] = 0; return 0; }
    hipLaunchKernelGGL(relu_bwd_colsum_partial_kernel<float>, dim3((cols + 31) / 32, (unsigned)chunks), dim3(256), 0,
                       (hipStream_t)stream, g, y, rows, cols, chunk_rows, g2, partial);
    return check_launch("relu_bwd_colsum_partial_kernel");
}

int clipops_mha_fwd_f32(const float *q, const float *k, const float *v, long q_bs, long q_rs, long k_bs, long k_rs,
                        long v_bs, long v_rs, const uint8_t *key_mask, int B, int H, int L, float scale, float *out,
                        float *lse, void *stream) {
    int rc = mha_check(q, k, v, B, H, L);
    if (rc) return rc;
    if ((long)B * L == 0) { g_err[0] = 0; return 0; }
    if (!out || !lse) return fail(1, "clipops_mha_fwd_f32: null pointer");
    const size_t lds = (size_t)2 * L * kPitch * sizeof(float);
    if ((rc = allow_lds(reinterpret_cast<const void *>(mha_fwd_kernel), lds, g_lds_fwd))) return rc;
    hipLaunchKernelGGL(mha_fwd_kernel, dim3((L + kRows - 1) / kRows, H, B), dim3(256), lds, (hipStream_t)stream, q, k, v, q_bs,
                       q_rs, k_bs, k_rs, v_bs, v_rs, key_mask, H, L, scale, out, lse);
    return check_launch("mha_fwd_kernel");
}

int clipops_mha_bwd_f32(const float *q, const float *k, const float *v, long q_bs, long q_rs, long k_bs, long k_rs,
                        long v_bs, long v_rs, const uint8_t *key_mask, const float *out, const float *lse,
                        const float *grad_out, int B, int H, int L, float scale, float *grad_q, long gq_bs, long gq_rs,
                        float *grad_k, long gk_bs, long gk_rs, float *grad_v, long gv_bs, long gv_rs, void *stream) {
    int rc = mha_check(q, k, v, B, H, L);
    if (rc) return rc;
    if ((long)B * L == 0) { g_err[0] = 0; return 0; }
    if (!out || !lse || !grad_out || !grad_q || !grad_k || !grad_v) return fail(1, "clipops_mha_bwd_f32: null pointer");
    const size_t lds_q = (size_t)2 * L * kPitch * sizeof(float);
    const size_t lds_kv = lds_q + (size_t)2 * L * sizeof(float);
    if ((rc = allow_lds(reinterpret_cast<const void *>(mha_bwd_q_kernel), lds_q, g_lds_bq))) return rc;
    if ((rc = allow_lds(reinterpret_cast<const void *>(mha_bwd_kv_kernel), lds_kv, g_lds_bkv))) return rc;
    const dim3 grid((L + kRows - 1) / kRows, H, B);
    hipLaunchKernelGGL(mha_bwd_q_kernel, grid, dim3(256), lds_q, (hipStream_t)stream, q, k, v, q_bs, q_rs, k_bs, k_rs,
                       v_bs, v_rs, key_mask, out, lse, grad_out, H, L, scale, grad_q, gq_bs, gq_rs);
    if ((rc = check_launch("mha_bwd_q_kernel"))) return rc;
    hipLaunchKernelGGL(mha_bwd_kv_kernel, grid, dim3(256), lds_kv, (hipStream_t)stream, q, k, v, q_bs, q_rs, k_bs, k_rs,
                       v_bs, v_rs, key_mask, out, lse, grad_out, H, L, scale, grad_k, gk_bs, gk_rs, grad_v, gv_bs, gv_rs);
    return check_launch("mha_bwd_kv_kernel");
}

int clipops_add_layer_norm_fwd_f32(const float *x, const float *res, const float *gamma, const float *beta, long rows,
                                   float eps, float *sum, float *y, float *stats, void *stream) {
    if (rows < 0) return fail(1, "clipops_add_layer_norm_fwd_f32: negative row count");
    if (rows == 0) { g_err[0] = 0; return 0; }
    if (!x || !res || !gamma || !beta || !sum || !y || !stats) return fail(1, "clipops_add_layer_norm_fwd_f32: null pointer");
    hipLaunchKernelGGL(add_layer_norm_fwd_kernel<false>, dim3((unsigned)((rows + 3) / 4)), dim3(256), 0, (hipStream_t)stream,
                       x, res, gamma, beta, nullptr, rows, eps, sum, y, nullptr, stats);
    return check_launch("add_layer_norm_fwd_kernel");
}

int clipops_add_layer_norm_pos_fwd_f32(const float *x, const float *res, const float *gamma, const float *beta,
                                       const float *pos, long rows, float eps, float *sum, float *y, float *q,
                                       float *stats, void *stream) {
    if (rows < 0) return fail(1, "clipops_add_layer_norm_pos_fwd_f32: negative row count");
    if (rows == 0) { g_err[0] = 0; return 0; }
    if (!x || !res || !gamma || !beta || !pos || !sum || !y || !q || !stats)
        return fail(1, "clipops_add_layer_norm_pos_fwd_f32: null pointer");
    hipLaunchKernelGGL(add_layer_norm_fwd_kernel<true>, dim3((unsigned)((rows + 3) / 4)), dim3(256), 0, (hipStream_t)stream,
                       x, res, gamma, beta, pos, rows, eps, sum, y, q, stats);
    return check_launch("add_layer_norm_fwd_kernel<pos>");
}

int clipops_add_layer_norm_bwd_f32(const float *grad_y, const float *sum, const float *stats, const float *gamma,
                                   long rows, int chunk_rows, float *grad_sum, float *partial, void *stream) {
    if (rows < 0 || chunk_rows <= 0) return fail(1, "clipops_add_layer_norm_bwd_f32: bad dimension");
    if (rows == 0) { g_err[0] = 0; return 0; }
    if (!grad_y || !sum || !stats || !gamma || !grad_sum || !partial)
        return fail(1, "clipops_add_layer_norm_bwd_f32: null pointer");
    hipLaunchKernelGGL(add_layer_norm_bwd_kernel, dim3((unsigned)((rows + chunk_rows - 1) / chunk_rows)), dim3(256), 0,
                       (hipStream_t)stream, grad_y, sum, stats, gamma, rows, chunk_rows, grad_sum, partial);
    return check_launch("add_layer_norm_bwd_kernel");
}

int clipops_add_layer_norm_fanin_bwd_f32(const float *g0, const float *g1, const float *g2, const float *sum,
                                         const float *stats, const float *gamma, long rows, int chunk_rows,
                                         float *grad_sum, float *partial, float *colsum_partial, void *stream) {
    if (rows < 0 || chunk_rows <= 0) return fail(1, "clipops_add_layer_norm_fanin_bwd_f32: bad dimension");
    if (rows == 0) { g_err[0] = 0; return 0; }
    const float *g[3] = {nullptr, nullptr, nullptr};
    int n = 0;
    if (g0) g[n++] = g0;
    if (g1) g[n++] = g1;
    if (g2) g[n++] = g2;
    if (n == 0) return fail(1, "clipops_add_layer_norm_fanin_bwd_f32: no gradient input");
    if (!sum || !stats || !gamma || !grad_sum || !partial || !colsum_partial)
        return fail(1, "clipops_add_layer_norm_fanin_bwd_f32: null pointer");
    hipLaunchKernelGGL(add_layer_norm_bwd_fanin_kernel, dim3((unsigned)((rows + chunk_rows - 1) / chunk_rows)), dim3(256), 0,
                       (hipStream_t)stream, g[0], g[1], g[2], sum, stats, gamma, rows, chunk_rows, grad_sum, partial,
                       colsum_partial);
    return check_launch("add_layer_norm_bwd_fanin_kernel");
}

int clipops_assign_f32(const float *cost, long stride_problem, long stride_row, long stride_col, int n_problems,
                       int n_rows, int n_cols, int32_t *row_ind, int32_t *col_ind, int32_t *status, void *stream) {
    if (n_problems < 0 || n_rows < 0 || n_cols < 0) return fail(1, "clipops_assign_f32: bad dimension");
    if (n_problems == 0 || n_rows == 0 || n_cols == 0) { g_err[0] = 0; return 0; }
    if (!cost || !row_ind || !col_ind) return fail(1, "clipops_assign_f32: null pointer");
    const int nr = n_rows < n_cols ? n_rows : n_cols, nc = n_rows < n_cols ? n_cols : n_rows;
    if (nc > CLIPOPS_ASSIGN_MAX_DIM) return fail(2, "clipops_assign_f32: problem exceeds CLIPOPS_ASSIGN_MAX_DIM");
    const size_t lds = (assign::work_bytes(nr, nc) + 15) & ~(size_t)15;
    if (lds > 64 * 1024) {
        static std::atomic<size_t> allowed{0};
        if (lds > 160 * 1024) return fail(2, "clipops_assign_f32: problem does not fit the LDS of a CU");
        if (lds > allowed.load()) {
            if (hipFuncSetAttribute(reinterpret_cast<const void *>(assign_kernel),
                                    hipFuncAttributeMaxDynamicSharedMemorySize, 160 * 1024) != hipSuccess) {
                (void)hipGetLastError();
                return fail(3, "clipops_assign_f32: hipFuncSetAttribute(MaxDynamicSharedMemorySize) failed");
            }
            allowed.store(160 * 1024);
        }
    }
    hipLaunchKernelGGL(assign_kernel, dim3(n_problems), dim3(64), lds, (hipStream_t)stream, cost, stride_problem,
                       stride_row, stride_col, n_rows, n_cols, row_ind, col_ind, status);
    return check_launch("assign_kernel");
}

static int shift_relu_check(const void *x, const void *shift, long planes, int C, long HW, const char *who) {
    if (planes < 0 || C <= 0 || HW < 0) return fail(1, who);
    if (planes && HW && (!x || !shift)) return fail(1, who);
    return 0;
}

int clipops_shift_relu_f32(float *x, const float *shift, const float *res, long planes, int C, long HW, void *stream) {
    if (shift_relu_check(x, shift, planes, C, HW, "clipops_shift_relu_f32: bad argument")) return 1;
    if (planes == 0 || HW == 0) { g_err[0] = 0; return 0; }
    const int vec = (HW % 4 == 0) && ((uintptr_t)x % 16 == 0) && (!res || (uintptr_t)res % 16 == 0);
    const long per = vec ? HW / 4 : HW;
    const dim3 grid((unsigned)((per + 1023) / 1024 > 64 ? 64 : (per + 1023) / 1024 < 1 ? 1 : (per + 1023) / 1024),
                    (unsigned)(planes > 65535 ? 65535 : planes));
    if (res) hipLaunchKernelGGL(shift_relu_f32_kernel<true>, grid, dim3(256), 0, (hipStream_t)stream, x, shift, res, planes, C, HW, vec);
    else hipLaunchKernelGGL(shift_relu_f32_kernel<false>, grid, dim3(256), 0, (hipStream_t)stream, x, shift, res, planes, C, HW, vec);
    return check_launch("shift_relu_f32_kernel");
}

int clipops_shift_relu_bf16(uint16_t *x, const float *shift, const uint16_t *res, long planes, int C, long HW, void *stream) {
    if (shift_relu_check(x, shift, planes, C, HW, "clipops_shift_relu_bf16: bad argument")) return 1;
    if (planes == 0 || HW == 0) { g_err[0] = 0; return 0; }
    const int vec = (HW % 8 == 0) && ((uintptr_t)x % 16 == 0) && (!res || (uintptr_t)res % 16 == 0);
    const long per = vec ? HW / 8 : HW;
    const dim3 grid((unsigned)((per + 1023) / 1024 > 64 ? 64 : (per + 1023) / 1024 < 1 ? 1 : (per + 1023) / 1024),
                    (unsigned)(planes > 65535 ? 65535 : planes));
    if (res) hipLaunchKernelGGL(shift_relu_bf16_kernel<true>, grid, dim3(256), 0, (hipStream_t)stream, x, shift, res, planes, C, HW, vec);
    else hipLaunchKernelGGL(shift_relu_bf16_kernel<false>, grid, dim3(256), 0, (hipStream_t)stream, x, shift, res, planes, C, HW, vec);
    return check_launch("shift_relu_bf16_kernel");
}

int clipops_linear_bwd_f32(const float *grad_y, const float *y_relu, const float *x, const float *w, int rows,
                           int in_features, int out_features, float *grad_x, float *grad_w, float *grad_b,
                           void *stream) {
    if (rows < 0 || in_features <= 0 || out_features <= 0) return fail(1, "clipops_linear_bwd_f32: bad dimension");
    if (!grad_y || !x || !w) return fail(1, "clipops_linear_bwd_f32: null pointer");
    if (grad_b && !grad_w) return fail(1, "clipops_linear_bwd_f32: grad_b is computed with grad_w");
    const int gx_ti = (rows + 31) / 32, gx_tj = (in_features + 31) / 32;
    const int gw_ti = (out_features + 31) / 32, gw_tj = gx_tj;
    const int n_gx = grad_x ? gx_ti * gx_tj : 0, n_gw = grad_w ? gw_ti * gw_tj : 0;
    if (n_gx + n_gw == 0) { g_err[0] = 0; return 0; }
    if (rows == 0) {
        if (grad_w && hipMemsetAsync(grad_w, 0, sizeof(float) * (size_t)out_features * in_features, (hipStream_t)stream) != hipSuccess)
            return fail(3, "clipops_linear_bwd_f32: memset failed");
        if (grad_b && hipMemsetAsync(grad_b, 0, sizeof(float) * (size_t)out_features, (hipStream_t)stream) != hipSuccess)
            return fail(3, "clipops_linear_bwd_f32: memset failed");
        g_err[0] = 0;
        return 0;
    }
    if (y_relu) hipLaunchKernelGGL(linear_bwd_kernel<true>, dim3(n_gx + n_gw), dim3(256), 0, (hipStream_t)stream, grad_y, y_relu, x, w, rows, in_features, out_features, grad_x, grad_w, grad_b, n_gx, gx_tj, gw_tj);
    else hipLaunchKernelGGL(linear_bwd_kernel<false>, dim3(n_gx + n_gw), dim3(256), 0, (hipStream_t)stream, grad_y, y_relu, x, w, rows, in_features, out_features, grad_x, grad_w, grad_b, n_gx, gx_tj, gw_tj);
    return check_launch("linear_bwd_kernel");
}

int clipops_linear_fwd_f32(const float *x, const float *w, const float *bias, int rows, int in_features,
                           int out_features, int relu, float *y, void *stream) {
    if (rows < 0 || in_features <= 0 || out_features <= 0) return fail(1, "clipops_linear_fwd_f32: bad dimension");
    if (in_features % 4) return fail(2, "clipops_linear_fwd_f32: in_features must be a multiple of 4");
    if (rows == 0) { g_err[0] = 0; return 0; }
    if (!x || !w || !y) return fail(1, "clipops_linear_fwd_f32: null pointer");
    const int ti = (rows + 31) / 32, tj = (out_features + 31) / 32;
    if (relu) hipLaunchKernelGGL(linear_fwd_kernel<true>, dim3(ti * tj), dim3(256), 0, (hipStream_t)stream, x, w, bias, rows, in_features, out_features, y, tj);
    else hipLaunchKernelGGL(linear_fwd_kernel<false>, dim3(ti * tj), dim3(256), 0, (hipStream_t)stream, x, w, bias, rows, in_features, out_features, y, tj);
    return check_launch("linear_fwd_kernel");
}

}
```

memotr_amd/functions/clip_ops.py:

```python
from __future__ import annotations

import os

import torch
import torch.nn.functional as F


def fused(*tensors) -> bool:
    return (os.environ.get("MEMOTR_FUSED_CLIP_OPS", "1") != "0"
            and all(t.is_cuda and (t.dtype == torch.float32 or not t.is_floating_point()) for t in tensors))


def config_key() -> tuple:
    return (os.environ.get("MEMOTR_FUSED_CLIP_OPS", "1"), os.environ.get("MEMOTR_COLSUM_TALL", "1"),
            os.environ.get("MEMOTR_ATTN_KERNELS", "1"), os.environ.get("MEMOTR_FUSED_LN", "1"),
            os.environ.get("MEMOTR_FUSED_SHIFT_RELU", "1"), os.environ.get("MEMOTR_FUSED_LINEAR_BWD", "1"),
            os.environ.get("MEMOTR_FUSED_LINEAR_FWD", "1"))


def _lib():
    from .. import _clip_lib
    return _clip_lib


def _stream(t: torch.Tensor) -> int:
    idx = t.device.index
    if idx is not None and idx != torch.cuda.current_device():
        raise RuntimeError(f"clip_ops: tensor on cuda:{idx} but cuda:{torch.cuda.current_device()} is current; "
                           "call torch.cuda.set_device(tensor.device) (one device per process)")
    return torch.cuda.current_stream(t.device).cuda_stream


def _strides3(t: torch.Tensor):
    if t.dim() != 3 or (t.shape[2] > 1 and t.stride(2) != 1):
        raise RuntimeError("expected a (layers, rows, C) tensor with a dense last axis")
    return t.stride(0), t.stride(1)


def match_cost(logits: torch.Tensor, boxes: torch.Tensor, gt_labels: torch.Tensor, gt_boxes: torch.Tensor,
               w_class: float, w_bbox: float, w_giou: float, out: torch.Tensor = None) -> torch.Tensor:
    n_layers, Q, K = logits.shape
    T = gt_labels.shape[0]
    if out is not None:
        assert out.is_contiguous() and out.dtype == torch.float32 and out.numel() == n_layers * Q * T
        cost = out.view(n_layers, Q, T)
    else:
        cost = torch.empty((n_layers, Q, T), dtype=torch.float32, device=logits.device)
    lsl, lsq = _strides3(logits)
    bsl, bsq = _strides3(boxes)
    gt_labels, gt_boxes = gt_labels.contiguous(), gt_boxes.contiguous()
    L = _lib()
    L.check(L.lib.clipops_match_cost_f32(logits.data_ptr(), lsl, lsq, boxes.data_ptr(), bsl, bsq, gt_labels.data_ptr(),
                                         gt_boxes.data_ptr(), n_layers, Q, K, T, float(w_class), float(w_bbox),
                                         float(w_giou), cost.data_ptr(), _stream(logits)), "clipops_match_cost_f32")
    return cost


def track_ownership(track_ids: torch.Tensor, gt_ids: torch.Tensor, free_out: torch.Tensor = None):
    n_tr, n_gt = track_ids.shape[0], gt_ids.shape[0]
    matched = torch.empty((n_tr,), dtype=torch.int64, device=gt_ids.device)
    free = free_out if free_out is not None else torch.empty((n_gt,), dtype=torch.float32, device=gt_ids.device)
    assert free.is_contiguous() and free.dtype == torch.float32 and free.numel() == n_gt
    track_ids, gt_ids = track_ids.contiguous(), gt_ids.contiguous()
    L = _lib()
    L.check(L.lib.clipops_track_ownership_i64(track_ids.data_ptr(), n_tr, gt_ids.data_ptr(), n_gt, matched.data_ptr(),
                                              free.data_ptr(), _stream(gt_ids)), "clipops_track_ownership_i64")
    return matched, free


def track_ownership_reference(track_ids, gt_ids):
    n_gt = gt_ids.shape[0]
    eq = track_ids[:, None] == gt_ids[None, :]
    order = torch.arange(1, n_gt + 1, device=eq.device)
    return (eq * order).amax(1) - 1 if n_gt > 0 else torch.full_like(track_ids, -1), (~eq.any(0)).to(torch.float32)


def focal_labels(lay: torch.Tensor, q: torch.Tensor, g: torch.Tensor, gt_labels: torch.Tensor, matched_idx,
                 late: torch.Tensor, n_det: int, n_tracks: int, num_classes: int) -> torch.Tensor:
    n_layers = late.shape[0]
    labels = torch.empty((n_layers, n_det + n_tracks), dtype=torch.int64, device=late.device)
    lay, q, g, gt_labels = lay.contiguous(), q.contiguous(), g.contiguous(), gt_labels.contiguous()
    L = _lib()
    L.check(L.lib.clipops_focal_labels_i64(lay.data_ptr(), q.data_ptr(), g.data_ptr(), lay.shape[0], gt_labels.data_ptr(),
                                           gt_labels.shape[0], None if matched_idx is None else matched_idx.contiguous().data_ptr(),
                                           n_tracks, late.contiguous().data_ptr(), n_layers, n_det, num_classes,
                                           labels.data_ptr(), _stream(late)), "clipops_focal_labels_i64")
    return labels


def focal_labels_reference(lay, q, g, gt_labels, matched_idx, late, n_det, n_tracks, num_classes):
    n_layers = late.shape[0]
    labels = torch.full((n_layers, n_det + n_tracks), num_classes, dtype=torch.int64, device=late.device)
    labels[lay, q] = gt_labels[g]
    if n_tracks > 0:
        has = matched_idx >= 0
        tr_lab = torch.where(has, gt_labels[matched_idx.clamp(min=0)] if gt_labels.shape[0] > 0
                             else torch.full_like(matched_idx, num_classes), torch.full_like(matched_idx, num_classes))
        labels[:, n_det:] = torch.where(late[:, None], tr_lab[None, :], labels[:, n_det:])
    return labels


class _PairBoxLoss(torch.autograd.Function):
    @staticmethod
    def forward(ctx, boxes_all, lay, qidx, b, tgt_boxes, gidx, weight):
        n_layers, B, Nq, _ = boxes_all.shape
        n = lay.shape[0]
        l1 = torch.empty((n,), dtype=torch.float32, device=boxes_all.device)
        gl = torch.empty_like(l1)
        L = _lib()
        L.check(L.lib.clipops_pair_box_loss_fwd_f32(
            boxes_all.data_ptr(), lay.data_ptr(), qidx.data_ptr(), B * Nq, b * Nq, tgt_boxes.data_ptr(),
            None if gidx is None else gidx.data_ptr(), None if weight is None else weight.data_ptr(), n,
            l1.data_ptr(), gl.data_ptr(), _stream(boxes_all)), "clipops_pair_box_loss_fwd_f32")
        ctx.save_for_backward(boxes_all, lay, qidx, tgt_boxes, gidx, weight)
        ctx.b = b
        return l1, gl

    @staticmethod
    def backward(ctx, g_l1, g_gl):
        boxes_all, lay, qidx, tgt_boxes, gidx, weight = ctx.saved_tensors
        n_layers, B, Nq, _ = boxes_all.shape
        grad = torch.zeros_like(boxes_all)
        L = _lib()
        L.check(L.lib.clipops_pair_box_loss_bwd_f32(
            boxes_all.data_ptr(), lay.data_ptr(), qidx.data_ptr(), B * Nq, ctx.b * Nq, tgt_boxes.data_ptr(),
            None if gidx is None else gidx.data_ptr(), None if weight is None else weight.data_ptr(), lay.shape[0],
            g_l1.contiguous().data_ptr(), g_gl.contiguous().data_ptr(), grad.data_ptr(), _stream(boxes_all)),
            "clipops_pair_box_loss_bwd_f32")
        return grad, None, None, None, None, None, None


def pair_box_loss(boxes_all: torch.Tensor, lay: torch.Tensor, qidx: torch.Tensor, b: int, tgt_boxes: torch.Tensor,
                  gidx: torch.Tensor = None, weight: torch.Tensor = None):
    if not boxes_all.is_contiguous():
        boxes_all = boxes_all.contiguous()
    return _PairBoxLoss.apply(boxes_all, lay.contiguous(), qidx.contiguous(), int(b), tgt_boxes.contiguous(),
                              None if gidx is None else gidx.contiguous(),
                              None if weight is None else weight.contiguous())


def pair_box_loss_reference(boxes_all, lay, qidx, b, tgt_boxes, gidx=None, weight=None):
    from ..models.criterion import paired_giou
    from ..utils.box_ops import box_cxcywh_to_xyxy
    pb = boxes_all[lay, b, qidx]
    tb = tgt_boxes if gidx is None else tgt_boxes[gidx]
    l1 = F.l1_loss(pb, tb, reduction="none").sum(-1)
    gl = 1 - paired_giou(box_cxcywh_to_xyxy(pb), box_cxcywh_to_xyxy(tb))
    if weight is not None:
        l1, gl = l1 * weight, gl * weight
    return l1, gl


def pair_iou(boxes: torch.Tensor, tgt_boxes: torch.Tensor, gidx: torch.Tensor = None) -> torch.Tensor:
    boxes, tgt_boxes = boxes.detach().contiguous(), tgt_boxes.contiguous()
    n = boxes.shape[0]
    out = torch.empty((n,), dtype=torch.float32, device=boxes.device)
    L = _lib()
    L.check(L.lib.clipops_pair_iou_f32(boxes.data_ptr(), tgt_boxes.data_ptr(), None if gidx is None else
                                       gidx.contiguous().data_ptr(), n, out.data_ptr(), _stream(boxes)),
            "clipops_pair_iou_f32")
    return out


def assign(cost: torch.Tensor):
    if cost.dim() != 3 or cost.dtype != torch.float32 or not cost.is_cuda:
        raise RuntimeError("assign expects a float32 CUDA tensor of shape (problems, rows, cols)")
    P, R, C = cost.shape
    k = min(R, C)
    row = torch.empty((P, k), dtype=torch.int32, device=cost.device)
    col = torch.empty((P, k), dtype=torch.int32, device=cost.device)
    status = torch.empty((P,), dtype=torch.int32, device=cost.device)
    L = _lib()
    L.check(L.lib.clipops_assign_f32(cost.data_ptr(), cost.stride(0), cost.stride(1), cost.stride(2), P, R, C,
                                     row.data_ptr(), col.data_ptr(), status.data_ptr(), _stream(cost)),
            "clipops_assign_f32")
    return row, col, status


def pair_iou_reference(boxes, tgt_boxes, gidx=None):
    from ..models.criterion import paired_iou
    from ..utils.box_ops import box_cxcywh_to_xyxy
    tb = tgt_boxes if gidx is None else tgt_boxes[gidx]
    return paired_iou(box_cxcywh_to_xyxy(boxes), box_cxcywh_to_xyxy(tb))


class _FocalPerLayer(torch.autograd.Function):
    @staticmethod
    def forward(ctx, logits, labels, alpha, gamma):
        n_layers, Nq, K = logits.shape
        sl, sq = _strides3(logits)
        loss = torch.empty((n_layers,), dtype=torch.float32, device=logits.device)
        L = _lib()
        L.check(L.lib.clipops_focal_fwd_f32(logits.data_ptr(), sl, sq, labels.data_ptr(), n_layers, Nq, K, alpha, gamma,
                                            loss.data_ptr(), _stream(logits)), "clipops_focal_fwd_f32")
        ctx.save_for_backward(logits, labels)
        ctx.alpha, ctx.gamma = alpha, gamma
        return loss

    @staticmethod
    def backward(ctx, g):
        logits, labels = ctx.saved_tensors
        n_layers, Nq, K = logits.shape
        sl, sq = _strides3(logits)
        grad = torch.empty((n_layers, Nq, K), dtype=torch.float32, device=logits.device)
        L = _lib()
        L.check(L.lib.clipops_focal_bwd_f32(logits.data_ptr(), sl, sq, labels.data_ptr(), n_layers, Nq, K, ctx.alpha,
                                            ctx.gamma, g.contiguous().data_ptr(), grad.data_ptr(), _stream(logits)),
                "clipops_focal_bwd_f32")
        return grad, None, None, None


def focal_loss_per_layer(logits: torch.Tensor, labels: torch.Tensor, alpha: float = 0.25, gamma: float = 2.0):
    return _FocalPerLayer.apply(logits, labels.contiguous(), float(alpha), float(gamma))


def focal_loss_per_layer_reference(logits, labels, alpha: float = 0.25, gamma: float = 2.0):
    from ..models.criterion import sigmoid_focal_loss_per_layer
    K = logits.shape[-1]
    one_hot = F.one_hot(labels, K + 1)[..., :-1].to(logits.dtype)
    return sigmoid_focal_loss_per_layer(logits, one_hot, alpha, gamma)


class _SineEmbed(torch.autograd.Function):
    @staticmethod
    def forward(ctx, pos, dim_t, scale):
        K, F_ = pos.shape[-1], dim_t.shape[0]
        n = pos.numel() // K
        out = torch.empty(pos.shape[:-1] + (K * F_,), dtype=torch.float32, device=pos.device)
        L = _lib()
        L.check(L.lib.clipops_sine_embed_fwd_f32(pos.data_ptr(), dim_t.data_ptr(), n, K, F_, scale, out.data_ptr(),
                                                 _stream(pos)), "clipops_sine_embed_fwd_f32")
        ctx.save_for_backward(pos, dim_t)
        ctx.scale = scale
        return out

    @staticmethod
    def backward(ctx, g):
        pos, dim_t = ctx.saved_tensors
        K, F_ = pos.shape[-1], dim_t.shape[0]
        grad = torch.empty_like(pos)
        L = _lib()
        L.check(L.lib.clipops_sine_embed_bwd_f32(pos.data_ptr(), dim_t.data_ptr(), pos.numel() // K, K, F_, ctx.scale,
                                                 g.contiguous().data_ptr(), grad.data_ptr(), _stream(pos)),
                "clipops_sine_embed_bwd_f32")
        return grad, None, None


def sine_embed(pos: torch.Tensor, dim_t: torch.Tensor, scale: float) -> torch.Tensor:
    return _SineEmbed.apply(pos.contiguous(), dim_t, float(scale))


class _InverseSigmoid(torch.autograd.Function):
    @staticmethod
    def forward(ctx, x, eps):
        y = torch.empty_like(x)
        L = _lib()
        L.check(L.lib.clipops_inverse_sigmoid_fwd_f32(x.data_ptr(), x.numel(), eps, y.data_ptr(), _stream(x)),
                "clipops_inverse_sigmoid_fwd_f32")
        ctx.save_for_backward(x)
        ctx.eps = eps
        return y

    @staticmethod
    def backward(ctx, g):
        x, = ctx.saved_tensors
        gx = torch.empty_like(x)
        L = _lib()
        L.check(L.lib.clipops_inverse_sigmoid_bwd_f32(x.data_ptr(), g.contiguous().data_ptr(), x.numel(), ctx.eps,
                                                      gx.data_ptr(), _stream(x)), "clipops_inverse_sigmoid_bwd_f32")
        return gx, None


def inverse_sigmoid(x: torch.Tensor, eps: float = 1e-5) -> torch.Tensor:
    return _InverseSigmoid.apply(x.contiguous(), float(eps))


class _RefineBoxes(torch.autograd.Function):
    @staticmethod
    def forward(ctx, delta, ref, eps):
        out = torch.empty_like(delta)
        L = _lib()
        L.check(L.lib.clipops_refine_boxes_fwd_f32(delta.data_ptr(), ref.data_ptr(), delta.numel(), eps, out.data_ptr(),
                                                   _stream(delta)), "clipops_refine_boxes_fwd_f32")
        ctx.save_for_backward(out, ref)
        ctx.eps = eps
        return out

    @staticmethod
    def backward(ctx, g):
        out, ref = ctx.saved_tensors
        gd = torch.empty_like(out)
        gr = torch.empty_like(out) if ctx.needs_input_grad[1] else None
        L = _lib()
        L.check(L.lib.clipops_refine_boxes_bwd_f32(out.data_ptr(), ref.data_ptr(), g.contiguous().data_ptr(),
                                                   out.numel(), ctx.eps, gd.data_ptr(),
                                                   None if gr is None else gr.data_ptr(), _stream(out)),
                "clipops_refine_boxes_bwd_f32")
        return gd, gr, None


def refine_boxes(delta: torch.Tensor, ref: torch.Tensor, eps: float = 1e-5) -> torch.Tensor:
    if delta.shape != ref.shape:
        raise RuntimeError("refine_boxes: delta and ref must have the same shape")
    return _RefineBoxes.apply(delta.contiguous(), ref.contiguous(), float(eps))


class _RefineBoxesSplit(torch.autograd.Function):
    @staticmethod
    def forward(ctx, delta, ref, eps):
        head, dec = torch.empty_like(delta), torch.empty_like(delta)
        L = _lib()
        L.check(L.lib.clipops_refine_boxes_split_fwd_f32(delta.data_ptr(), ref.data_ptr(), delta.numel() // 4, eps,
                                                         head.data_ptr(), dec.data_ptr(), _stream(delta)),
                "clipops_refine_boxes_split_fwd_f32")
        ctx.save_for_backward(head, ref)
        ctx.eps = eps
        ctx.mark_non_differentiable(dec)
        return head, dec

    @staticmethod
    def backward(ctx, g, _g_dec):
        return _RefineBoxes.backward(ctx, g)


def refine_boxes_split_reference(delta: torch.Tensor, ref: torch.Tensor, eps: float = 1e-5):
    from ..utils.utils import inverse_sigmoid_reference
    head = (delta + inverse_sigmoid_reference(ref, eps)).sigmoid()
    with torch.no_grad():
        xy = delta[..., :2] + inverse_sigmoid_reference(ref[..., :2], eps)
        dec = torch.cat((xy, delta[..., 2:]), -1).sigmoid()
    return head, dec


def refine_boxes_split(delta: torch.Tensor, ref: torch.Tensor, eps: float = 1e-5):
    if delta.shape != ref.shape or delta.shape[-1] != 4:
        raise RuntimeError("refine_boxes_split: delta and ref must have the same (..., 4) shape")
    if fused(delta, ref) and delta.dtype == torch.float32 and ref.dtype == torch.float32:
        return _RefineBoxesSplit.apply(delta.contiguous(), ref.contiguous(), float(eps))
    return refine_boxes_split_reference(delta, ref, eps)


COLSUM_MAX_ROWS = 2048
COLSUM_CHUNK_ROWS = 256


def colsum(x: torch.Tensor, out: torch.Tensor = None) -> torch.Tensor:
    b16 = x.dtype == torch.bfloat16
    ok = (x.dim() == 2 and x.is_contiguous() and x.is_cuda and (x.dtype == torch.float32 or b16)
          and os.environ.get("MEMOTR_FUSED_CLIP_OPS", "1") != "0"
          and (out is None or (out.is_contiguous() and out.dtype == torch.float32))
          and 0 < x.shape[0] <= COLSUM_MAX_ROWS * COLSUM_CHUNK_ROWS)
    if not ok:
        return torch.sum(x, 0, out=out) if out is not None else x.sum(0)
    if x.shape[0] > COLSUM_MAX_ROWS and not b16 and os.environ.get("MEMOTR_COLSUM_TALL", "1") == "0":
        return torch.sum(x, 0, out=out) if out is not None else x.sum(0)
    L = _lib()
    if x.shape[0] > COLSUM_MAX_ROWS or b16:
        chunks = -(-x.shape[0] // COLSUM_CHUNK_ROWS)
        partial = torch.empty((chunks, x.shape[1]), dtype=torch.float32, device=x.device)
        fn = L.lib.clipops_colsum_partial_bf16 if b16 else L.lib.clipops_colsum_partial_f32
        L.check(fn(x.data_ptr(), x.shape[0], x.shape[1], COLSUM_CHUNK_ROWS, partial.data_ptr(), _stream(x)),
                "clipops_colsum_partial")
        x = partial
    if out is None:
        out = torch.empty((x.shape[1],), dtype=torch.float32, device=x.device)
    L.check(L.lib.clipops_colsum_f32(x.data_ptr(), x.shape[0], x.shape[1], out.data_ptr(), _stream(x)),
            "clipops_colsum_f32")
    return out


def relu_bwd_colsum_usable(g: torch.Tensor, y: torch.Tensor) -> bool:
    return (os.environ.get("MEMOTR_FUSED_CLIP_OPS", "1") != "0" and os.environ.get("MEMOTR_FUSED_RELU_COLSUM", "1") != "0"
            and g.is_cuda and g.dim() == 2 and g.is_contiguous() and y.is_contiguous() and y.shape == g.shape
            and g.dtype == y.dtype and g.dtype == torch.float32
            and COLSUM_MAX_ROWS < g.shape[0] <= COLSUM_MAX_ROWS * COLSUM_CHUNK_ROWS)


def relu_bwd_colsum(g: torch.Tensor, y: torch.Tensor):
    rows, cols = g.shape
    chunks = -(-rows // COLSUM_CHUNK_ROWS)
    g2 = torch.empty_like(g)
    partial = torch.empty((chunks, cols), dtype=torch.float32, device=g.device)
    out = torch.empty((cols,), dtype=torch.float32, device=g.device)
    L = _lib()
    fn = L.lib.clipops_relu_bwd_colsum_partial_f32
    L.check(fn(g.data_ptr(), y.data_ptr(), rows, cols, COLSUM_CHUNK_ROWS, g2.data_ptr(), partial.data_ptr(), _stream(g)),
            "clipops_relu_bwd_colsum_partial")
    L.check(L.lib.clipops_colsum_f32(partial.data_ptr(), chunks, cols, out.data_ptr(), _stream(g)), "clipops_colsum_f32")
    return g2, out


class _AddRowBias(torch.autograd.Function):

    @staticmethod
    def forward(ctx, x, bias):
        return x + bias

    @staticmethod
    def backward(ctx, g):
        gb = None
        if ctx.needs_input_grad[1]:
            g2 = g.reshape(-1, g.shape[-1])
            gb = colsum(g2 if g2.is_contiguous() else g2.contiguous())
        return (g if ctx.needs_input_grad[0] else None), gb


def add_row_bias(x: torch.Tensor, bias: torch.Tensor) -> torch.Tensor:
    if x.is_cuda and bias.requires_grad and torch.is_grad_enabled() and bias.dim() == 1:
        return _AddRowBias.apply(x, bias)
    return x + bias


LINEAR_BWD_MAX_ROWS = 1024
LINEAR_BWD_MAX_OUT = 512


def linear_bwd_usable(g2: torch.Tensor, x2: torch.Tensor, weight: torch.Tensor) -> bool:
    return (os.environ.get("MEMOTR_FUSED_LINEAR_BWD", "1") != "0" and fused(g2, x2, weight)
            and g2.dtype == torch.float32 and x2.dtype == torch.float32 and weight.dtype == torch.float32
            and 0 < g2.shape[0] <= LINEAR_BWD_MAX_ROWS and g2.shape[1] <= LINEAR_BWD_MAX_OUT
            and x2.is_contiguous() and weight.is_contiguous())


def linear_bwd(g2: torch.Tensor, y_relu, x2: torch.Tensor, weight: torch.Tensor, need_x=True, need_w=True, need_b=True,
               gw_out: torch.Tensor = None, gb_out: torch.Tensor = None):
    g2 = g2.contiguous()
    rows, out_f = g2.shape
    in_f = x2.shape[1]
    need_w = need_w or need_b
    gx = torch.empty((rows, in_f), dtype=torch.float32, device=g2.device) if need_x else None
    gw = (gw_out if gw_out is not None else torch.empty((out_f, in_f), dtype=torch.float32, device=g2.device)) if need_w else None
    gb = (gb_out if gb_out is not None else torch.empty((out_f,), dtype=torch.float32, device=g2.device)) if need_b else None
    assert gw is None or (gw.is_contiguous() and gw.shape == (out_f, in_f)), "gw_out must be a contiguous (out, in) buffer"
    assert gb is None or (gb.is_contiguous() and gb.shape == (out_f,)), "gb_out must be a contiguous (out,) buffer"
    L_ = _lib()
    L_.check(L_.lib.clipops_linear_bwd_f32(g2.data_ptr(), None if y_relu is None else y_relu.data_ptr(), x2.data_ptr(),
                                           weight.data_ptr(), rows, in_f, out_f,
                                           None if gx is None else gx.data_ptr(), None if gw is None else gw.data_ptr(),
                                           None if gb is None else gb.data_ptr(), _stream(g2)), "clipops_linear_bwd_f32")
    return gx, gw, gb


LINEAR_FWD_MAX_IN = 256


def linear_fwd_usable(x2: torch.Tensor, weight: torch.Tensor, bias) -> bool:
    return (os.environ.get("MEMOTR_FUSED_LINEAR_FWD", "1") != "0" and fused(x2, weight)
            and x2.dtype == torch.float32 and weight.dtype == torch.float32
            and 0 < x2.shape[0] <= LINEAR_BWD_MAX_ROWS and weight.shape[0] <= LINEAR_BWD_MAX_OUT
            and x2.shape[1] % 4 == 0 and x2.shape[1] <= LINEAR_FWD_MAX_IN and x2.is_contiguous() and weight.is_contiguous()
            and (bias is None or (bias.dtype == torch.float32 and bias.is_contiguous())))


def linear_fwd(x2: torch.Tensor, weight: torch.Tensor, bias, relu: bool) -> torch.Tensor:
    rows, in_f = x2.shape
    out_f = weight.shape[0]
    y = torch.empty((rows, out_f), dtype=torch.float32, device=x2.device)
    L_ = _lib()
    L_.check(L_.lib.clipops_linear_fwd_f32(x2.data_ptr(), weight.data_ptr(), None if bias is None else bias.data_ptr(),
                                           rows, in_f, out_f, 1 if relu else 0, y.data_ptr(), _stream(x2)),
             "clipops_linear_fwd_f32")
    return y


def linear_bwd_reference(g2, y_relu, x2, weight):
    if y_relu is not None:
        g2 = g2 * (y_relu > 0).to(g2.dtype)
    return g2 @ weight, g2.t() @ x2, g2.sum(0)


class _ShiftRelu(torch.autograd.Function):

    @staticmethod
    def forward(ctx, x, shift, res):
        N, C, H, W = x.shape
        L_ = _lib()
        fn = L_.lib.clipops_shift_relu_bf16 if x.dtype == torch.bfloat16 else L_.lib.clipops_shift_relu_f32
        L_.check(fn(x.data_ptr(), shift.data_ptr(), None if res is None else res.data_ptr(), N * C, C, H * W,
                    _stream(x)), "clipops_shift_relu")
        ctx.mark_dirty(x)
        ctx.save_for_backward(x)
        ctx.has_res = res is not None
        return x

    @staticmethod
    def backward(ctx, g):
        (y,) = ctx.saved_tensors
        gx = torch.ops.aten.threshold_backward(g, y, 0)
        return gx, None, (gx if ctx.has_res else None)


def shift_relu_reference(x: torch.Tensor, shift: torch.Tensor, res: torch.Tensor = None) -> torch.Tensor:
    y = x + shift.to(x.dtype)[None, :, None, None]
    if res is not None:
        y = y + res
    return F.relu(y)


def shift_relu_(x: torch.Tensor, shift: torch.Tensor, res: torch.Tensor = None) -> torch.Tensor:
    ok = (os.environ.get("MEMOTR_FUSED_CLIP_OPS", "1") != "0" and os.environ.get("MEMOTR_FUSED_SHIFT_RELU", "1") != "0"
          and x.is_cuda and x.dim() == 4 and x.dtype in (torch.float32, torch.bfloat16) and x.is_contiguous()
          and not x._is_view() and shift.dtype == torch.float32 and shift.is_contiguous() and not shift.requires_grad
          and (res is None or (res.dtype == x.dtype and res.shape == x.shape and res.is_contiguous())))
    if not ok:
        return shift_relu_reference(x, shift, res)
    return _ShiftRelu.apply(x, shift, res)


MHA_MAX_L = 512
MHA_HEAD_DIM = 32


class _SelfAttention(torch.autograd.Function):
    @staticmethod
    def forward(ctx, qk_p, v_p, key_mask, n_heads):
        B, L, E2 = qk_p.shape
        E = E2 // 2
        out = torch.empty((B, L, E), dtype=torch.float32, device=qk_p.device)
        lse = torch.empty((B, n_heads, L), dtype=torch.float32, device=qk_p.device)
        scale = 1.0 / (E // n_heads) ** 0.5
        mk = None if key_mask is None else key_mask.data_ptr()
        L_ = _lib()
        L_.check(L_.lib.clipops_mha_fwd_f32(qk_p.data_ptr(), qk_p.data_ptr() + 4 * E, v_p.data_ptr(), L * E2, E2, L * E2,
                                            E2, L * E, E, mk, B, n_heads, L, scale, out.data_ptr(), lse.data_ptr(),
                                            _stream(qk_p)), "clipops_mha_fwd_f32")
        ctx.save_for_backward(qk_p, v_p, key_mask, out, lse)
        ctx.n_heads, ctx.scale = n_heads, scale
        return out

    @staticmethod
    def backward(ctx, g):
        qk_p, v_p, key_mask, out, lse = ctx.saved_tensors
        B, L, E2 = qk_p.shape
        E = E2 // 2
        g = g.contiguous()
        g_qk, g_v = torch.empty_like(qk_p), torch.empty_like(v_p)
        mk = None if key_mask is None else key_mask.data_ptr()
        L_ = _lib()
        L_.check(L_.lib.clipops_mha_bwd_f32(qk_p.data_ptr(), qk_p.data_ptr() + 4 * E, v_p.data_ptr(), L * E2, E2, L * E2,
                                            E2, L * E, E, mk, out.data_ptr(), lse.data_ptr(), g.data_ptr(), B, ctx.n_heads,
                                            L, ctx.scale, g_qk.data_ptr(), L * E2, E2, g_qk.data_ptr() + 4 * E, L * E2,
                                            E2, g_v.data_ptr(), L * E, E, _stream(qk_p)), "clipops_mha_bwd_f32")
        return g_qk, g_v, None, None


class _Attention3(torch.autograd.Function):

    @staticmethod
    def forward(ctx, q_p, k_p, v_p, key_mask, n_heads):
        B, L, E = q_p.shape
        out = torch.empty((B, L, E), dtype=torch.float32, device=q_p.device)
        lse = torch.empty((B, n_heads, L), dtype=torch.float32, device=q_p.device)
        scale = 1.0 / (E // n_heads) ** 0.5
        mk = None if key_mask is None else key_mask.data_ptr()
        L_ = _lib()
        L_.check(L_.lib.clipops_mha_fwd_f32(q_p.data_ptr(), k_p.data_ptr(), v_p.data_ptr(), L * E, E, L * E, E, L * E, E,
                                            mk, B, n_heads, L, scale, out.data_ptr(), lse.data_ptr(), _stream(q_p)),
                 "clipops_mha_fwd_f32")
        ctx.save_for_backward(q_p, k_p, v_p, key_mask, out, lse)
        ctx.n_heads, ctx.scale = n_heads, scale
        return out

    @staticmethod
    def backward(ctx, g):
        q_p, k_p, v_p, key_mask, out, lse = ctx.saved_tensors
        B, L, E = q_p.shape
        g = g.contiguous()
        g_q, g_k, g_v = torch.empty_like(q_p), torch.empty_like(k_p), torch.empty_like(v_p)
        mk = None if key_mask is None else key_mask.data_ptr()
        L_ = _lib()
        L_.check(L_.lib.clipops_mha_bwd_f32(q_p.data_ptr(), k_p.data_ptr(), v_p.data_ptr(), L * E, E, L * E, E, L * E, E,
                                            mk, out.data_ptr(), lse.data_ptr(), g.data_ptr(), B, ctx.n_heads, L,
                                            ctx.scale, g_q.data_ptr(), L * E, E, g_k.data_ptr(), L * E, E,
                                            g_v.data_ptr(), L * E, E, _stream(q_p)), "clipops_mha_bwd_f32")
        return g_q, g_k, g_v, None, None


def attention(q_p: torch.Tensor, k_p: torch.Tensor, v_p: torch.Tensor, n_heads: int, key_padding_mask=None) -> torch.Tensor:
    mask = None if key_padding_mask is None else key_padding_mask.contiguous()
    return _Attention3.apply(q_p.contiguous(), k_p.contiguous(), v_p.contiguous(), mask, int(n_heads))


def attention_supported(q_p: torch.Tensor, k_p: torch.Tensor, n_heads: int) -> bool:
    return (os.environ.get("MEMOTR_ATTN_KERNELS", "1") != "0" and q_p.dim() == 3 and q_p.shape == k_p.shape
            and fused(q_p, k_p) and q_p.dtype == torch.float32
            and q_p.shape[2] % n_heads == 0 and q_p.shape[2] // n_heads == MHA_HEAD_DIM and 0 < q_p.shape[1] <= MHA_MAX_L)


def self_attention_supported(qk_p: torch.Tensor, n_heads: int, any_float: bool = False) -> bool:
    B, L, E2 = qk_p.shape
    dtype_ok = qk_p.is_floating_point() if any_float else qk_p.dtype == torch.float32
    return (os.environ.get("MEMOTR_ATTN_KERNELS", "1") != "0" and os.environ.get("MEMOTR_FUSED_CLIP_OPS", "1") != "0"
            and qk_p.is_cuda and dtype_ok and E2 % (2 * n_heads) == 0
            and E2 // 2 // n_heads == MHA_HEAD_DIM and 0 < L <= MHA_MAX_L)


def self_attention(qk_p: torch.Tensor, v_p: torch.Tensor, key_padding_mask, n_heads: int) -> torch.Tensor:
    mask = None if key_padding_mask is None else key_padding_mask.contiguous()
    return _SelfAttention.apply(qk_p.contiguous(), v_p.contiguous(), mask, int(n_heads))


def self_attention_reference(qk_p, v_p, key_padding_mask, n_heads):
    B, L, E2 = qk_p.shape
    E, d = E2 // 2, E2 // 2 // n_heads
    q, k = (t.transpose(1, 2) for t in qk_p.view(B, L, 2, n_heads, d).unbind(2))
    v = v_p.view(B, L, n_heads, d).transpose(1, 2)
    att = (q @ k.transpose(-1, -2)) / d ** 0.5
    if key_padding_mask is not None:
        att = att.masked_fill(key_padding_mask.view(B, 1, 1, L), float("-inf"))
    return (att.softmax(-1) @ v).transpose(1, 2).reshape(B, L, E)


LN_COLS = 256


class _AddLayerNorm(torch.autograd.Function):
    @staticmethod
    def forward(ctx, x, res, weight, bias, eps):
        s, y, _, stats = add_layer_norm_fwd(x, res, weight, bias, eps)
        ctx.save_for_backward(s, stats, weight)
        return y

    @staticmethod
    def backward(ctx, g):
        s, stats, weight = ctx.saved_tensors
        rows = s.numel() // LN_COLS
        g = g.contiguous()
        gs = torch.empty_like(s)
        chunk = 16 if rows <= 4096 else 64
        partial = torch.empty((-(-rows // chunk), 2 * LN_COLS), dtype=torch.float32, device=s.device)
        L = _lib()
        L.check(L.lib.clipops_add_layer_norm_bwd_f32(g.data_ptr(), s.data_ptr(), stats.data_ptr(), weight.data_ptr(), rows,
                                                     chunk, gs.data_ptr(), partial.data_ptr(), _stream(s)),
                "clipops_add_layer_norm_bwd_f32")
        gwb = colsum(partial)
        return gs, gs, gwb[:LN_COLS], gwb[LN_COLS:], None


def add_layer_norm_fwd(x: torch.Tensor, res: torch.Tensor, weight: torch.Tensor, bias: torch.Tensor, eps: float,
                       pos: torch.Tensor = None):
    rows = x.numel() // LN_COLS
    s, y = torch.empty_like(x), torch.empty_like(x)
    stats = torch.empty((rows, 2), dtype=torch.float32, device=x.device)
    L = _lib()
    if pos is None:
        L.check(L.lib.clipops_add_layer_norm_fwd_f32(x.data_ptr(), res.data_ptr(), weight.data_ptr(), bias.data_ptr(),
                                                     rows, eps, s.data_ptr(), y.data_ptr(), stats.data_ptr(), _stream(x)),
                "clipops_add_layer_norm_fwd_f32")
        return s, y, None, stats
    assert pos.shape == x.shape and pos.is_contiguous() and pos.dtype == torch.float32
    q = torch.empty_like(x)
    L.check(L.lib.clipops_add_layer_norm_pos_fwd_f32(x.data_ptr(), res.data_ptr(), weight.data_ptr(), bias.data_ptr(),
                                                     pos.data_ptr(), rows, eps, s.data_ptr(), y.data_ptr(), q.data_ptr(),
                                                     stats.data_ptr(), _stream(x)), "clipops_add_layer_norm_pos_fwd_f32")
    return s, y, q, stats


def _fanin_chunk_rows(rows: int) -> int:
    if rows <= 4096:
        return 16
    per_chunk = -(-rows // 1024)
    return max(64, (per_chunk + 3) // 4 * 4)


def add_layer_norm_bwd_fanin(grads, s: torch.Tensor, stats: torch.Tensor, weight: torch.Tensor):
    g0, g1, g2 = grads
    for g in grads:
        assert g is None or (g.is_contiguous() and g.dtype == torch.float32 and g.numel() == s.numel())
    rows = s.numel() // LN_COLS
    chunk = _fanin_chunk_rows(rows)
    chunks = -(-rows // chunk)
    gs = torch.empty_like(s)
    partial = torch.empty((chunks, 2 * LN_COLS), dtype=torch.float32, device=s.device)
    zpartial = torch.empty((2 * chunks, LN_COLS), dtype=torch.float32, device=s.device)
    out = torch.empty((3 * LN_COLS,), dtype=torch.float32, device=s.device)
    ptr = lambda t: None if t is None else t.data_ptr()
    L = _lib()
    st = _stream(s)
    L.check(L.lib.clipops_add_layer_norm_fanin_bwd_f32(ptr(g0), ptr(g1), ptr(g2), s.data_ptr(), stats.data_ptr(),
                                                       weight.data_ptr(), rows, chunk, gs.data_ptr(), partial.data_ptr(),
                                                       zpartial.data_ptr(), st), "clipops_add_layer_norm_fanin_bwd_f32")
    L.check(L.lib.clipops_colsum_f32(partial.data_ptr(), chunks, 2 * LN_COLS, out.data_ptr(), st), "clipops_colsum_f32")
    L.check(L.lib.clipops_colsum_f32(zpartial.data_ptr(), 2 * chunks, LN_COLS, out.data_ptr() + 8 * LN_COLS, st),
            "clipops_colsum_f32")
    return gs, out[:LN_COLS], out[LN_COLS:2 * LN_COLS], out[2 * LN_COLS:]


def add_layer_norm_supported(x: torch.Tensor, res: torch.Tensor, norm) -> bool:
    island = torch.is_autocast_enabled()
    ok_dtype = (lambda t: t.is_floating_point()) if island else (lambda t: t.dtype == torch.float32)
    return (isinstance(norm, torch.nn.LayerNorm) and norm.elementwise_affine and norm.bias is not None
            and tuple(norm.normalized_shape) == (LN_COLS,) and x.shape == res.shape and x.shape[-1] == LN_COLS
            and x.is_cuda and res.is_cuda and ok_dtype(x) and ok_dtype(res) and norm.weight.dtype == torch.float32
            and os.environ.get("MEMOTR_FUSED_CLIP_OPS", "1") != "0" and os.environ.get("MEMOTR_FUSED_LN", "1") != "0")


def add_layer_norm(x: torch.Tensor, res: torch.Tensor, norm) -> torch.Tensor:
    if add_layer_norm_supported(x, res, norm):
        return _AddLayerNorm.apply(x.float().contiguous(), res.float().contiguous(), norm.weight, norm.bias,
                                   float(norm.eps))
    return norm(x + res)
```

memotr_amd/models/deformable_decoder.py:

```python
from __future__ import annotations

import torch
import torch.nn as nn
from torch.utils.checkpoint import checkpoint

from ..modules import MSDeformAttn
from ..modules.ms_deform_attn import project_values
from ..functions.clip_ops import add_layer_norm, refine_boxes_split
from ..modules.attention import self_attention
from ..modules.linear import row_linear
from ..utils.utils import refine_boxes
from .decoder_graphs import DecoderGraphs
from .mlp import MLP
from .utils import get_activation_layer, get_clones, pos_to_pos_embed


class DeformableDecoder(nn.Module):
    def __init__(self, decoder_layer, num_layers, return_intermediate=False, merge_det_track_layer: int = 0,
                 n_det_queries: int = 300, d_model: int = 256, use_checkpoint: bool = False, use_dab: bool = False,
                 visualize: bool = False):
        super().__init__()
        self.layers = get_clones(module=decoder_layer, n=num_layers)
        self.num_layers = num_layers
        self.return_intermediate = return_intermediate
        self.merge_det_track_layer = merge_det_track_layer
        self.n_det_queries = n_det_queries
        self.d_model = d_model
        self.bbox_embed = None
        self.class_embed = None
        self.use_checkpoint = use_checkpoint
        self.use_dab = use_dab
        self.visualize = visualize
        if self.use_dab:
            self.query_scale = MLP(d_model, d_model, d_model, 2)
            self.ref_point_head = MLP(d_model * 2, d_model, d_model, 2)

    def __getstate__(self):
        state = self.__dict__.copy()
        state.pop("_decoder_graphs", None)
        state.pop("_infer_graphs", None)
        return state

    def graphs(self) -> DecoderGraphs:
        g = self.__dict__.get("_decoder_graphs")
        if g is None:
            g = self.__dict__["_decoder_graphs"] = DecoderGraphs(self)
        return g

    def infer_graphs(self):
        g = self.__dict__.get("_infer_graphs")
        if g is None:
            from .infer_graphs import InferGraphs
            g = self.__dict__["_infer_graphs"] = InferGraphs(None)
        return g

    def _forward_graphed(self, tgt, reference_points, src, spatial_shapes, level_start_index, valid_ratios, query_pos,
                         query_mask, src_padding_mask, frame_slot, clip_key=None, infer=False):
        graphs = self.graphs()
        nd = self.n_det_queries
        B, nq, C = tgt.shape
        nb = graphs.bucket(nq, nd)
        if nb > nq:
            pad = nb - nq
            tgt = torch.cat((tgt, tgt.new_zeros(B, pad, C)), 1)
            reference_points = torch.cat((reference_points, reference_points.new_full((B, pad, 4), 0.5)), 1)
            query_mask = torch.cat((query_mask, query_mask.new_ones(B, pad)), 1)
            if not self.use_dab:
                query_pos = torch.cat((query_pos, query_pos.new_zeros(B, pad, C)), 1)
        ratios4 = torch.cat([valid_ratios, valid_ratios], -1)[:, None].contiguous()
        query_mask = query_mask.contiguous()
        if self.use_dab:
            args = (tgt.contiguous(), reference_points.contiguous(), src, ratios4, query_mask, src_padding_mask)
        else:
            args = (tgt.contiguous(), reference_points.contiguous(), query_pos.contiguous(), src,
                    valid_ratios.contiguous(), ratios4, query_mask, src_padding_mask)
        if infer:
            res = self.infer_graphs().run_decode(self, args, spatial_shapes, level_start_index)
        else:
            res = graphs.run(frame_slot, args, spatial_shapes, level_start_index, clip_key)
        if res is None:
            return None
        outs, refs, layer_inputs, boxes = res
        if nb > nq:
            outs, refs, layer_inputs, boxes = (x[:, :, :nq] for x in (outs, refs, layer_inputs, boxes))
        return outs, refs, layer_inputs, boxes

    def forward(self, tgt, reference_points, src, src_spatial_shapes, src_level_start_index, src_valid_ratios,
                query_pos, query_mask, src_padding_mask, frame_slot=None, clip_key=None):
        if not self.return_intermediate:
            raise NotImplementedError("Not Support for no Inter Outputs.")
        if (frame_slot is not None and reference_points.shape[-1] == 4 and src_padding_mask is not None
                and self.graphs().usable(tgt, src)):
            res = self._forward_graphed(tgt, reference_points, src, src_spatial_shapes, src_level_start_index,
                                        src_valid_ratios, query_pos, query_mask, src_padding_mask, frame_slot,
                                        clip_key)
            if res is not None:
                return res
        if (not torch.is_grad_enabled() and reference_points.shape[-1] == 4 and src_padding_mask is not None
                and self.infer_graphs().decode_usable(self, tgt, src)):
            res = self._forward_graphed(tgt, reference_points, src, src_spatial_shapes, src_level_start_index,
                                        src_valid_ratios, query_pos, query_mask, src_padding_mask, None,
                                        infer=True)
            if res is not None:
                return res
        nd = self.n_det_queries
        output = tgt
        outs, refs, layer_inputs, boxes = [], [], [], []
        ref_backup = None
        ratios4 = torch.cat([src_valid_ratios, src_valid_ratios], -1)[:, None]
        values = None if self.use_checkpoint else project_values([layer.cross_attn for layer in self.layers], src,
                                                                 src_padding_mask)
        for lid, layer in enumerate(self.layers):
            if lid == 0 and not self.use_dab:
                ref_backup = reference_points.clone()
                reference_points = reference_points[:, :, :2]
            if reference_points.shape[-1] == 4:
                ref_in = reference_points[:, :, None] * ratios4
            else:
                assert reference_points.shape[-1] == 2
                ref_in = reference_points[:, :, None] * src_valid_ratios[:, None]
            if self.use_dab:
                anchor = pos_to_pos_embed(ref_in[:, :, 0, :], num_pos_feats=self.d_model // 2)
                raw_pos = self.ref_point_head(anchor)
                query_pos = raw_pos if lid == 0 else self.query_scale(output) * raw_pos
            layer_inputs.append(output)
            merge = lid >= self.merge_det_track_layer
            if self.use_checkpoint:
                output = checkpoint(layer, output, query_pos, ref_in, src, src_spatial_shapes, src_level_start_index,
                                    query_mask, src_padding_mask, merge, use_reentrant=False)
            else:
                output = layer(output, query_pos, ref_in, src, src_spatial_shapes, src_level_start_index, query_mask,
                               src_padding_mask, merge, None if values is None else values[lid])
            if self.bbox_embed is not None:
                delta = self.bbox_embed[lid](output)
                if reference_points.shape[-1] == 4:
                    box = new_ref = refine_boxes(delta, reference_points)
                else:
                    box, new_ref = refine_boxes_split(delta, ref_backup)
                boxes.append(box)
                if not merge:
                    keep = reference_points if self.use_dab else ref_backup
                    reference_points = torch.cat((new_ref[:, :nd].detach(), keep[:, nd:]), dim=1)
                else:
                    reference_points = new_ref.detach()
            outs.append(output)
            refs.append(reference_points)
        return (torch.stack(outs), torch.stack(refs), torch.stack(layer_inputs),
                torch.stack(boxes) if len(boxes) == len(outs) else None)


class DeformableDecoderLayer(nn.Module):
    def __init__(self, d_model=256, d_ffn=1024, dropout=0.1, activation="ReLU", n_levels=4, n_heads=8, n_points=4,
                 sigmoid_attn=False, extra_track_attn=False, n_det_queries=300, visualize: bool = False):
        super().__init__()
        self.visualize = visualize
        self.n_det_queries = n_det_queries
        self.n_heads = n_heads
        self.self_attn = nn.MultiheadAttention(embed_dim=d_model, num_heads=n_heads, dropout=dropout,
                                               batch_first=True)
        self.dropout2 = nn.Dropout(dropout)
        self.norm2 = nn.LayerNorm(d_model)
        self.cross_attn = MSDeformAttn(d_model=d_model, n_levels=n_levels, n_heads=n_heads, n_points=n_points,
                                       sigmoid_attn=sigmoid_attn, visualize=visualize)
        self.dropout1 = nn.Dropout(dropout)
        self.norm1 = nn.LayerNorm(d_model)
        self.linear1 = nn.Linear(d_model, d_ffn)
        self.activation = get_activation_layer(activation=activation)
        self.dropout3 = nn.Dropout(dropout)
        self.linear2 = nn.Linear(d_ffn, d_model)
        self.dropout4 = nn.Dropout(dropout)
        self.norm3 = nn.LayerNorm(d_model)
        self.extra_track_attn = extra_track_attn
        if extra_track_attn:
            self.track_attn = nn.MultiheadAttention(embed_dim=d_model, num_heads=n_heads, dropout=dropout,
                                                    batch_first=True)
            self.dropout5 = nn.Dropout(dropout)
            self.norm4 = nn.LayerNorm(d_model)

    @staticmethod
    def with_pos_embed(tensor, pos):
        return tensor if pos is None else tensor + pos

    def forward_self_attn(self, tgt, query_pos, query_mask):
        qk = self.with_pos_embed(tgt, query_pos)
        attn = self_attention(self.self_attn, qk, tgt, key_padding_mask=query_mask)
        return add_layer_norm(tgt, self.dropout2(attn), self.norm2)

    def forward_track_attn(self, tgt, query_pos, query_mask):
        nd = self.n_det_queries
        if tgt.shape[1] <= nd:
            return tgt
        qk = self.with_pos_embed(tgt, query_pos)[:, nd:]
        track_mask = query_mask[:, nd:]
        track_mask._no_padding = getattr(query_mask, "_no_padding", False)
        attn = self_attention(self.track_attn, qk, tgt[:, nd:], key_padding_mask=track_mask)
        return torch.cat([tgt[:, :nd], self.norm4(tgt[:, nd:] + self.dropout5(attn))], dim=1)

    def forward_ffn(self, tgt):
        if isinstance(self.activation, nn.ReLU):
            hidden = row_linear(tgt, self.linear1.weight, self.linear1.bias, relu=True)
        else:
            hidden = self.activation(row_linear(tgt, self.linear1.weight, self.linear1.bias))
        hidden = self.dropout3(hidden)
        return add_layer_norm(tgt, self.dropout4(row_linear(hidden, self.linear2.weight, self.linear2.bias)), self.norm3)

    def forward(self, tgt, query_pos, reference_points, src, src_spatial_shapes, level_start_index, query_mask,
                src_padding_mask=None, merge_det_track=False, value=None):
        nd = self.n_det_queries
        track_tgt = None
        if not merge_det_track:
            tgt, track_tgt = tgt.split((nd, tgt.shape[1] - nd), dim=1)
            query_pos = query_pos[:, :nd, :]
            reference_points, query_mask = reference_points[:, :nd], query_mask[:, :nd]
            query_mask._no_padding = True
        if self.extra_track_attn:
            tgt = self.forward_track_attn(tgt, query_pos, query_mask)
        tgt = self.forward_self_attn(tgt, query_pos, query_mask)
        cross = self.cross_attn(self.with_pos_embed(tgt, query_pos), reference_points, src, src_spatial_shapes,
                                level_start_index, src_padding_mask, value)
        tgt = add_layer_norm(tgt, self.dropout1(cross), self.norm1)
        tgt = self.forward_ffn(tgt)
        if track_tgt is not None:
            tgt = torch.cat((tgt, track_tgt), dim=1)
        return tgt
```

memotr_amd/modules/ms_deform_attn.py:

```python
from __future__ import annotations

import math
import os
import warnings

import torch
import torch.nn.functional as F
from torch import nn
from torch.nn.init import constant_, xavier_uniform_

from .. import MultiScaleDeformableAttention as MSDA
from ..functions import BankSlices, MSDeformAttnFunction, MSDeformAttnFusedFunction, ValueBank
from .linear import long_linear

FUSED_PROLOGUE = os.environ.get("MEMOTR_FUSED_PROLOGUE", "1") != "0"


def _is_power_of_2(n) -> bool:
    if (not isinstance(n, int)) or (n < 0):
        raise ValueError("invalid input for _is_power_of_2: {} (type: {})".format(n, type(n)))
    return (n & (n - 1) == 0) and n != 0


def _level_sizes(spatial_shapes: torch.Tensor, dtype: torch.dtype) -> torch.Tensor:
    cached = getattr(spatial_shapes, "_msda_wh", None)
    if cached is None or cached[0] != (spatial_shapes._version, dtype):
        cached = ((spatial_shapes._version, dtype), spatial_shapes.flip(-1).to(dtype))
        try:
            spatial_shapes._msda_wh = cached
        except AttributeError:
            pass
    return cached[1]


MASKED_ROWS_ATTR = "_msda_masked_rows"


def tag_masked_rows(mask: torch.Tensor) -> torch.Tensor:
    if mask is not None and mask.is_cuda and not torch.cuda.is_current_stream_capturing():
        setattr(mask, MASKED_ROWS_ATTR, mask.reshape(-1).nonzero().squeeze(1))
    return mask


class _ZeroRows(torch.autograd.Function):

    @staticmethod
    def forward(ctx, x, rows, consumer_zeroes=None):
        ctx.rows = rows
        ctx.consumer_zeroes = consumer_zeroes
        if x._is_view() or not x.is_contiguous():
            return x.reshape(-1, x.shape[-1]).index_fill(0, rows, 0).view(x.shape)
        x.view(-1, x.shape[-1]).index_fill_(0, rows, 0)
        ctx.mark_dirty(x)
        return x

    @staticmethod
    def backward(ctx, g):
        if ctx.consumer_zeroes is not None and ctx.consumer_zeroes[0]:
            return g, None, None
        return g.reshape(-1, g.shape[-1]).index_fill(0, ctx.rows, 0).view(g.shape), None, None


class ProjectedValue:
    __slots__ = ("value", "bank", "index", "mask")

    def __init__(self, value, bank, index, mask):
        self.value, self.bank, self.index, self.mask = value, bank, index, mask


BATCHED_VALUE_PROJ = os.environ.get("MEMOTR_BATCHED_VALUE_PROJ", "1") != "0"


def project_values(modules, input_flatten: torch.Tensor, input_padding_mask=None):
    mods = list(modules)
    if not mods or not BATCHED_VALUE_PROJ or not FUSED_PROLOGUE or len(mods) < 2:
        return None
    m0 = mods[0]
    M, L, P, C = m0.n_heads, m0.n_levels, m0.n_points, m0.d_model
    x = input_flatten
    if not (x.is_cuda and x.dim() == 3 and x.dtype == torch.float32 and not torch.is_autocast_enabled() and C // M == 32
            and MSDA.fused_supported(x.dtype, C // M, L, P)
            and all(isinstance(m, MSDeformAttn) and not m.sigmoid_attn and (m.n_heads, m.n_levels, m.n_points, m.d_model)
                    == (M, L, P, C) and m.value_proj.weight.dtype == torch.float32 for m in mods)):
        return None
    N, S, _ = x.shape
    G = len(mods)
    if (G * C * 4) % 16 != 0 or N * S * G * C >= (1 << 29):
        return None
    mask = input_padding_mask
    rows = getattr(mask, MASKED_ROWS_ATTR, None) if mask is not None else None
    zero = None
    if rows is not None:
        mask = None
        if rows.numel():
            zero = lambda y: _ZeroRows.apply(y, rows, None)
    w = torch.cat([m.value_proj.weight for m in mods], 0)
    b = torch.cat([m.value_proj.bias for m in mods], 0)
    value_all = long_linear(x, w, b, activation=zero)
    bank = ValueBank(G)
    slices = BankSlices.apply(value_all.view(N, S, G, M, C // M), bank)
    return [ProjectedValue(v, bank, i, mask) for i, v in enumerate(slices)]


class MSDeformAttn(nn.Module):
    def __init__(self, d_model=256, n_levels=4, n_heads=8, n_points=4, sigmoid_attn=False, visualize=False):
        super().__init__()
        if d_model % n_heads != 0:
            raise ValueError("d_model must be divisible by n_heads, but got {} and {}".format(d_model, n_heads))
        if not _is_power_of_2(d_model // n_heads):
            warnings.warn("MSDeformAttn: a power-of-2 head dimension (32 for MeMOTR) takes the specialised "
                          "gfx950 kernels; other sizes run the generic ones.")
        self.im2col_step = 64
        self.sigmoid_attn = sigmoid_attn
        self.d_model = d_model
        self.n_levels = n_levels
        self.n_heads = n_heads
        self.n_points = n_points
        self.visualize = visualize

        self.sampling_offsets = nn.Linear(d_model, n_heads * n_levels * n_points * 2)
        self.attention_weights = nn.Linear(d_model, n_heads * n_levels * n_points)
        self.value_proj = nn.Linear(d_model, d_model)
        self.output_proj = nn.Linear(d_model, d_model)
        self.reset_parameters()

    def reset_parameters(self):
        constant_(self.sampling_offsets.weight.data, 0.0)
        thetas = torch.arange(self.n_heads, dtype=torch.float32) * (2.0 * math.pi / self.n_heads)
        grid = torch.stack([thetas.cos(), thetas.sin()], -1)
        grid = grid / grid.abs().max(-1, keepdim=True)[0]
        grid = grid.view(self.n_heads, 1, 1, 2).repeat(1, self.n_levels, self.n_points, 1)
        grid = grid * torch.arange(1, self.n_points + 1, dtype=torch.float32).view(1, 1, self.n_points, 1)
        with torch.no_grad():
            self.sampling_offsets.bias = nn.Parameter(grid.reshape(-1))
        constant_(self.attention_weights.weight.data, 0.0)
        constant_(self.attention_weights.bias.data, 0.0)
        xavier_uniform_(self.value_proj.weight.data)
        constant_(self.value_proj.bias.data, 0.0)
        xavier_uniform_(self.output_proj.weight.data)
        constant_(self.output_proj.bias.data, 0.0)

    def _forward_projected(self, query, reference_points, pv: "ProjectedValue", input_spatial_shapes,
                           input_level_start_index):
        M, P = self.n_heads, self.n_points
        site = self.__dict__.get("_msda_site")
        if site is None:
            site = self.__dict__["_msda_site"] = MSDA.new_call_site()
        MSDA.set_call_site(site)
        w, b = self._fused_query_projection()
        proj = long_linear(query, w, b)
        if reference_points.shape[-1] not in (2, 4):
            raise ValueError("Last dim of reference_points must be 2 or 4, but get {} instead.".format(
                reference_points.shape[-1]))
        out = MSDeformAttnFusedFunction.apply(pv.value, input_spatial_shapes, input_level_start_index, proj.contiguous(),
                                              reference_points.contiguous(),
                                              None if pv.mask is None else pv.mask.contiguous(), M, P, None,
                                              (pv.bank, pv.index))
        return long_linear(out, self.output_proj.weight, self.output_proj.bias)

    def _fused_query_projection(self):
        so, aw = self.sampling_offsets, self.attention_weights
        pre = getattr(so.weight, "_msda_fused_qproj", None)
        if pre is not None:
            return pre
        if so.weight.is_cuda and torch.cuda.is_current_stream_capturing():
            return torch.cat((so.weight, aw.weight), 0), torch.cat((so.bias, aw.bias), 0)
        key = (id(so.weight), id(aw.weight), so.weight._version, aw.weight._version, so.bias._version,
               aw.bias._version, so.weight.device, so.weight.dtype, torch.is_grad_enabled())
        cached = self.__dict__.get("_fused_qproj")
        if cached is None or cached[0] != key:
            w = torch.cat((so.weight, aw.weight), 0)
            b = torch.cat((so.bias, aw.bias), 0)
            if w.requires_grad:
                w.register_hook(self._forget_fused_query_projection)
            cached = (key, w, b)
            self.__dict__["_fused_qproj"] = cached
        return cached[1], cached[2]

    def _forget_fused_query_projection(self, grad=None):
        self.__dict__.pop("_fused_qproj", None)
        return None

    def train(self, mode: bool = True):
        self._forget_fused_query_projection()
        return super().train(mode)

    def _apply(self, fn, *args, **kwargs):
        self._forget_fused_query_projection()
        return super()._apply(fn, *args, **kwargs)

    def _load_from_state_dict(self, *args, **kwargs):
        self._forget_fused_query_projection()
        return super()._load_from_state_dict(*args, **kwargs)

    def __getstate__(self):
        state = dict(self.__dict__)
        state.pop("_fused_qproj", None)
        state.pop("_msda_site", None)
        return state

    def __deepcopy__(self, memo):
        import copy
        new = self.__class__.__new__(self.__class__)
        memo[id(self)] = new
        for k, v in self.__dict__.items():
            if k not in ("_fused_qproj", "_msda_site"):
                new.__dict__[k] = copy.deepcopy(v, memo)
        return new

    def forward(self, query, reference_points, input_flatten, input_spatial_shapes, input_level_start_index,
                input_padding_mask=None, value: "ProjectedValue" = None):
        N, Lq, _ = query.shape
        S = input_flatten.shape[1]
        M, L, P = self.n_heads, self.n_levels, self.n_points
        if value is not None:
            return self._forward_projected(query, reference_points, value, input_spatial_shapes,
                                           input_level_start_index)
        if input_flatten.is_cuda:
            site = self.__dict__.get("_msda_site")
            if site is None:
                site = self.__dict__["_msda_site"] = MSDA.new_call_site()
            MSDA.set_call_site(site)

        mask = input_padding_mask
        rows = getattr(mask, MASKED_ROWS_ATTR, None) if mask is not None else None
        if rows is not None and not (FUSED_PROLOGUE and input_flatten.is_cuda and not self.sigmoid_attn):
            rows = None
        zero = None
        fused_zeroes = [False]
        if rows is not None:
            mask = None
            if rows.numel():
                zero = lambda y: _ZeroRows.apply(y, rows, fused_zeroes)
        value = long_linear(input_flatten, self.value_proj.weight, self.value_proj.bias, activation=zero)

        n_off = M * L * P * 2
        w, b = self._fused_query_projection()
        proj = long_linear(query, w, b)
        if proj.dtype == torch.bfloat16:
            proj = proj.float()
            reference_points = reference_points.float()
        if reference_points.shape[-1] not in (2, 4):
            raise ValueError("Last dim of reference_points must be 2 or 4, but get {} instead.".format(
                reference_points.shape[-1]))

        if (FUSED_PROLOGUE and value.is_cuda and not self.sigmoid_attn and proj.dtype == torch.float32
                and reference_points.dtype == torch.float32
                and MSDA.fused_supported(value.dtype, self.d_model // M, L, P)):
            fused_zeroes[0] = zero is not None
            out = MSDeformAttnFusedFunction.apply(value.view(N, S, M, self.d_model // M), input_spatial_shapes,
                                                  input_level_start_index, proj.contiguous(),
                                                  reference_points.contiguous(),
                                                  None if mask is None else mask.contiguous(),
                                                  M, P, rows if zero is not None else None)
            return long_linear(out, self.output_proj.weight, self.output_proj.bias)

        if mask is not None:
            value = value.masked_fill(mask[..., None], 0.0)
        value = value.view(N, S, M, self.d_model // M)
        offsets = proj[..., :n_off].unflatten(-1, (M, L, P, 2))
        logits = proj[..., n_off:].unflatten(-1, (M, L * P))
        if self.sigmoid_attn:
            attn = logits.sigmoid()
        else:
            attn = F.softmax(logits, -1)
        attn = attn.view(N, Lq, M, L, P)

        if reference_points.shape[-1] == 2:
            wh = _level_sizes(input_spatial_shapes, offsets.dtype)
            loc = reference_points[:, :, None, :, None, :] + offsets / wh[None, None, None, :, None, :]
        else:
            if P & (P - 1) == 0:
                loc = reference_points[:, :, None, :, None, :2] \
                    + offsets * (reference_points[:, :, None, :, None, 2:] * (0.5 / P))
            else:
                loc = reference_points[:, :, None, :, None, :2] \
                    + offsets / P * reference_points[:, :, None, :, None, 2:] * 0.5

        out = MSDeformAttnFunction.apply(value.contiguous(), input_spatial_shapes, input_level_start_index,
                                         loc.contiguous(), attn.contiguous(), self.im2col_step)
        return long_linear(out, self.output_proj.weight, self.output_proj.bias)
```

Baseline: 42.08.

## Fuse decoder self-attention block into a custom autograd node with joined linear backward

Adds a custom autograd node for the decoder self-attention block covering the QK/V projection, attention, output projection and add+LayerNorm. Its backward uses a new joined linear-backward kernel that computes grad_x and grad_w in one launch, accumulates into existing gradient buffers, and folds the positional-embedding add into the weight-gradient input. Also adds a forward linear kernel that adds query_pos inside the cross-attention query projection, so the tgt+pos tensor is never materialised. The aim is fewer kernel launches, fewer intermediate tensors and less autograd overhead, at the cost of more kernel variants and more custom code to keep correct.

```diff
diff --git a/include/clip_ops_hip.h b/include/clip_ops_hip.h
--- a/include/clip_ops_hip.h
+++ b/include/clip_ops_hip.h
@@ -94,6 +94,13 @@
 int clipops_linear_fwd_f32(const float *x, const float *w, const float *bias, int rows, int in_features,
                            int out_features, int relu, float *y, void *stream);
 
+int clipops_linear_bwd_join_f32(const float *grad_y, const float *grad_y2, const float *y_relu, const float *x,
+                                const float *x_add, const float *w, int rows, int in_features, int out_features, float *grad_x,
+                                float *grad_x2, float *grad_w, float *grad_b, int accumulate, void *stream);
+
+int clipops_linear_fwd_add_f32(const float *x, const float *p, const float *w, const float *bias, int rows,
+                               int in_features, int out_features, int relu, float *y, void *stream);
+
 int clipops_relu_bwd_colsum_partial_f32(const float *g, const float *y, long rows, int cols, int chunk_rows, float *g2,
                                         float *partial, void *stream);
 
diff --git a/memotr_amd/_clip_lib.py b/memotr_amd/_clip_lib.py
--- a/memotr_amd/_clip_lib.py
+++ b/memotr_amd/_clip_lib.py
@@ -47,6 +47,8 @@
     "clipops_refine_boxes_fwd_f32": ([c_void_p, c_void_p, c_long, c_float, c_void_p, c_void_p], c_int),
     "clipops_linear_bwd_f32": ([c_void_p] * 4 + [c_int] * 3 + [c_void_p] * 4, c_int),
     "clipops_linear_fwd_f32": ([c_void_p] * 3 + [c_int] * 4 + [c_void_p, c_void_p], c_int),
+    "clipops_linear_bwd_join_f32": ([c_void_p] * 6 + [c_int] * 3 + [c_void_p] * 4 + [c_int, c_void_p], c_int),
+    "clipops_linear_fwd_add_f32": ([c_void_p] * 4 + [c_int] * 4 + [c_void_p, c_void_p], c_int),
     "clipops_relu_bwd_colsum_partial_f32": ([c_void_p, c_void_p, c_long, c_int, c_int, c_void_p, c_void_p, c_void_p], c_int),
     "clipops_shift_relu_f32": ([c_void_p, c_void_p, c_void_p, c_long, c_int, c_long, c_void_p], c_int),
     "clipops_shift_relu_bf16": ([c_void_p, c_void_p, c_void_p, c_long, c_int, c_long, c_void_p], c_int),
diff --git a/memotr_amd/csrc/clip_ops.hip b/memotr_amd/csrc/clip_ops.hip
--- a/memotr_amd/csrc/clip_ops.hip
+++ b/memotr_amd/csrc/clip_ops.hip
@@ -945,11 +945,13 @@
 #endif
 constexpr int LB_U = MSDA_LB_U;
 
-template <bool GX, bool RELU>
+template <bool GX, bool RELU, bool JOIN = false, bool G2 = false, bool XADD = false>
 __device__ __forceinline__ void linear_bwd_tile(const float *__restrict__ g, const float *__restrict__ y,
                                                 const float *__restrict__ Bp, int M, int N, int K, int OUT, int i0, int j0,
                                                 float *__restrict__ C, float *__restrict__ gb, float (*s_c)[16][64],
-                                                float (*s_b)[32]) {
+                                                float (*s_b)[32], const float *__restrict__ g2 = nullptr,
+                                                bool c_acc = false, bool gb_acc = false, float *__restrict__ C2 = nullptr,
+                                                const float *__restrict__ Bp2 = nullptr) {
     const int lane = threadIdx.x & 63, wave = threadIdx.x >> 6;
     const int i = i0 + (lane & 31), j = j0 + (lane & 31), kq = (lane >> 5) * 4;
     const bool iok = i < M, jok = j < N;
@@ -958,6 +960,18 @@
     const bool vec = GX && (OUT % 4 == 0);
     lb_f32x16 acc = {0.f, 0.f, 0.f, 0.f, 0.f, 0.f, 0.f, 0.f, 0.f, 0.f, 0.f, 0.f, 0.f, 0.f, 0.f, 0.f};
     float bsum = 0.f;
+    float old[4] = {0.f, 0.f, 0.f, 0.f}, old2[4] = {0.f, 0.f, 0.f, 0.f};
+    if (JOIN && (c_acc || C2 != nullptr)) {
+#pragma unroll
+        for (int rr = 0; rr < 4; ++rr) {
+            const int r = wave * 4 + rr;
+            const int row = i0 + (r & 3) + 8 * (r >> 2) + 4 * (lane >> 5);
+            if (row < M && jok) {
+                if (c_acc) old[rr] = C[(long)row * N + j];
+                if (C2 != nullptr) old2[rr] = C2[(long)row * N + j];
+            }
+        }
+    }
     for (int c = c_lo; c < c_hi; c += LB_U) {
         float a[LB_U][4], b[LB_U][4], m[LB_U][4];
 #pragma unroll
@@ -968,6 +982,10 @@
                 float4 av = {0.f, 0.f, 0.f, 0.f}, mv = {1.f, 1.f, 1.f, 1.f};
                 if (cok && iok && k0 < K) {
                     av = *reinterpret_cast<const float4 *>(g + (long)i * OUT + k0);
+                    if (G2) {
+                        const float4 bv = *reinterpret_cast<const float4 *>(g2 + (long)i * OUT + k0);
+                        av.x += bv.x; av.y += bv.y; av.z += bv.z; av.w += bv.w;
+                    }
                     if (RELU) mv = *reinterpret_cast<const float4 *>(y + (long)i * OUT + k0);
                 }
                 a[u][0] = av.x; a[u][1] = av.y; a[u][2] = av.z; a[u][3] = av.w;
@@ -980,9 +998,11 @@
                 if (!vec) {
                     const long idx = GX ? (long)i * OUT + k : (long)k * OUT + i;
                     a[u][q] = (iok && kok) ? g[idx] : 0.f;
+                    if (G2) a[u][q] += (iok && kok) ? g2[idx] : 0.f;
                     m[u][q] = (RELU && iok && kok) ? y[idx] : 1.f;
                 }
                 b[u][q] = (jok && kok) ? Bp[(long)k * N + j] : 0.f;
+                if (XADD) b[u][q] += (jok && kok) ? Bp2[(long)k * N + j] : 0.f;
             }
         }
 #pragma unroll
@@ -1005,10 +1025,20 @@
         const int r = wave * 4 + rr;
         const float v = (s_c[0][r][lane] + s_c[1][r][lane]) + (s_c[2][r][lane] + s_c[3][r][lane]);
         const int row = i0 + (r & 3) + 8 * (r >> 2) + 4 * (lane >> 5);
-        if (row < M && jok) C[(long)row * N + j] = v;
-    }
-    if (!GX && gb != nullptr && j0 == 0 && wave == 0 && lane < 32 && i0 + lane < M)
-        gb[i0 + lane] = (s_b[0][lane] + s_b[1][lane]) + (s_b[2][lane] + s_b[3][lane]);
+        if (row < M && jok) {
+            const long idx = (long)row * N + j;
+            if (JOIN) {
+                C[idx] = c_acc ? old[rr] + v : v;
+                if (C2 != nullptr) C2[idx] = old2[rr] + v;
+            } else {
+                C[idx] = v;
+            }
+        }
+    }
+    if (!GX && gb != nullptr && j0 == 0 && wave == 0 && lane < 32 && i0 + lane < M) {
+        const float v = (s_b[0][lane] + s_b[1][lane]) + (s_b[2][lane] + s_b[3][lane]);
+        gb[i0 + lane] = (JOIN && gb_acc) ? gb[i0 + lane] + v : v;
+    }
 }
 
 template <bool RELU>
@@ -1028,10 +1058,32 @@
     }
 }
 
-template <bool RELU>
+template <bool RELU, bool G2, bool XADD>
+__global__ __launch_bounds__(256) void linear_bwd_join_kernel(const float *__restrict__ g, const float *__restrict__ g2,
+                                                              const float *__restrict__ y, const float *__restrict__ x,
+                                                              const float *__restrict__ xp, const float *__restrict__ w,
+                                                              int R, int IN, int OUT,
+                                                              float *__restrict__ gx, float *__restrict__ gx2,
+                                                              float *__restrict__ gw, float *__restrict__ gb, int acc,
+                                                              int n_gx, int gx_tj, int gw_tj) {
+    __shared__ float s_c[4][16][64];
+    __shared__ float s_b[4][32];
+    const int tile = blockIdx.x;
+    if (tile < n_gx) {
+        linear_bwd_tile<true, RELU, true, G2, false>(g, y, w, R, IN, OUT, OUT, (tile / gx_tj) * 32, (tile % gx_tj) * 32, gx, nullptr, s_c,
+                                          s_b, g2, (acc & 1) != 0, false, gx2);
+    } else {
+        const int t = tile - n_gx;
+        linear_bwd_tile<false, RELU, true, G2, XADD>(g, y, x, OUT, IN, R, OUT, (t / gw_tj) * 32, (t % gw_tj) * 32, gw, gb, s_c, s_b, g2,
+                                           (acc & 2) != 0, (acc & 4) != 0, nullptr, xp);
+    }
+}
+
+template <bool RELU, bool ADD = false>
 __global__ __launch_bounds__(256) void linear_fwd_kernel(const float *__restrict__ x, const float *__restrict__ w,
                                                          const float *__restrict__ bias, int R, int IN, int OUT,
-                                                         float *__restrict__ yout, int tj) {
+                                                         float *__restrict__ yout, int tj,
+                                                         const float *__restrict__ p = nullptr) {
     __shared__ float s_c[4][16][64];
     const int lane = threadIdx.x & 63, wave = threadIdx.x >> 6;
     const int i0 = (blockIdx.x / tj) * 32, j0 = (blockIdx.x % tj) * 32;
@@ -1047,6 +1099,10 @@
             const int k0 = (c + u) * 8 + kq;
             const bool kok = c + u < c_hi && k0 < IN;
             a[u] = (iok && kok) ? *reinterpret_cast<const float4 *>(x + (long)i * IN + k0) : float4{0.f, 0.f, 0.f, 0.f};
+            if (ADD && iok && kok) {
+                const float4 pv = *reinterpret_cast<const float4 *>(p + (long)i * IN + k0);
+                a[u].x += pv.x; a[u].y += pv.y; a[u].z += pv.z; a[u].w += pv.w;
+            }
             b[u] = (jok && kok) ? *reinterpret_cast<const float4 *>(w + (long)j * IN + k0) : float4{0.f, 0.f, 0.f, 0.f};
         }
 #pragma unroll
@@ -1590,4 +1646,58 @@
     return check_launch("linear_fwd_kernel");
 }
 
-}
+int clipops_linear_bwd_join_f32(const float *grad_y, const float *grad_y2, const float *y_relu, const float *x,
+                                const float *x_add, const float *w, int rows, int in_features, int out_features, float *grad_x,
+                                float *grad_x2, float *grad_w, float *grad_b, int accumulate, void *stream) {
+    if (rows < 0 || in_features <= 0 || out_features <= 0) return fail(1, "clipops_linear_bwd_join_f32: bad dimension");
+    if (!grad_y || !x || !w) return fail(1, "clipops_linear_bwd_join_f32: null pointer");
+    if (grad_b && !grad_w) return fail(1, "clipops_linear_bwd_join_f32: grad_b is computed with grad_w");
+    if (grad_x2 && !grad_x) return fail(1, "clipops_linear_bwd_join_f32: grad_x2 is computed with grad_x");
+    if (accumulate & ~7) return fail(1, "clipops_linear_bwd_join_f32: bad accumulate mask");
+    if (grad_x && (grad_x == grad_y || grad_x == grad_y2 || grad_x == x || grad_x == x_add || grad_x == grad_x2))
+        return fail(1, "clipops_linear_bwd_join_f32: grad_x aliases an input");
+    if (grad_x2 && (grad_x2 == grad_y || grad_x2 == grad_y2 || grad_x2 == x || grad_x2 == x_add))
+        return fail(1, "clipops_linear_bwd_join_f32: grad_x2 aliases an input");
+    const int gx_ti = (rows + 31) / 32, gx_tj = (in_features + 31) / 32;
+    const int gw_ti = (out_features + 31) / 32, gw_tj = gx_tj;
+    const int n_gx = grad_x ? gx_ti * gx_tj : 0, n_gw = grad_w ? gw_ti * gw_tj : 0;
+    if (n_gx + n_gw == 0) { g_err[0] = 0; return 0; }
+    if (rows == 0) {
+        if (grad_w && !(accumulate & 2) && hipMemsetAsync(grad_w, 0, sizeof(float) * (size_t)out_features * in_features, (hipStream_t)stream) != hipSuccess)
+            return fail(3, "clipops_linear_bwd_join_f32: memset failed");
+        if (grad_b && !(accumulate & 4) && hipMemsetAsync(grad_b, 0, sizeof(float) * (size_t)out_features, (hipStream_t)stream) != hipSuccess)
+            return fail(3, "clipops_linear_bwd_join_f32: memset failed");
+        g_err[0] = 0;
+        return 0;
+    }
+#define CLIPOPS_JOIN_LAUNCH(RELU, G2, XADD)                                                                                   \
+    hipLaunchKernelGGL((linear_bwd_join_kernel<RELU, G2, XADD>), dim3(n_gx + n_gw), dim3(256), 0, (hipStream_t)stream, grad_y, \
+                       grad_y2, y_relu, x, x_add, w, rows, in_features, out_features, grad_x, grad_x2, grad_w, grad_b,         \
+                       accumulate, n_gx, gx_tj, gw_tj)
+    switch ((y_relu ? 4 : 0) | (grad_y2 ? 2 : 0) | (x_add ? 1 : 0)) {
+        case 0: CLIPOPS_JOIN_LAUNCH(false, false, false); break;
+        case 1: CLIPOPS_JOIN_LAUNCH(false, false, true); break;
+        case 2: CLIPOPS_JOIN_LAUNCH(false, true, false); break;
+        case 3: CLIPOPS_JOIN_LAUNCH(false, true, true); break;
+        case 4: CLIPOPS_JOIN_LAUNCH(true, false, false); break;
+        case 5: CLIPOPS_JOIN_LAUNCH(true, false, true); break;
+        case 6: CLIPOPS_JOIN_LAUNCH(true, true, false); break;
+        default: CLIPOPS_JOIN_LAUNCH(true, true, true); break;
+    }
+#undef CLIPOPS_JOIN_LAUNCH
+    return check_launch("linear_bwd_join_kernel");
+}
+
+int clipops_linear_fwd_add_f32(const float *x, const float *p, const float *w, const float *bias, int rows,
+                               int in_features, int out_features, int relu, float *y, void *stream) {
+    if (rows < 0 || in_features <= 0 || out_features <= 0) return fail(1, "clipops_linear_fwd_add_f32: bad dimension");
+    if (in_features % 4) return fail(2, "clipops_linear_fwd_add_f32: in_features must be a multiple of 4");
+    if (rows == 0) { g_err[0] = 0; return 0; }
+    if (!x || !p || !w || !y) return fail(1, "clipops_linear_fwd_add_f32: null pointer");
+    const int ti = (rows + 31) / 32, tj = (out_features + 31) / 32;
+    if (relu) hipLaunchKernelGGL((linear_fwd_kernel<true, true>), dim3(ti * tj), dim3(256), 0, (hipStream_t)stream, x, w, bias, rows, in_features, out_features, y, tj, p);
+    else hipLaunchKernelGGL((linear_fwd_kernel<false, true>), dim3(ti * tj), dim3(256), 0, (hipStream_t)stream, x, w, bias, rows, in_features, out_features, y, tj, p);
+    return check_launch("linear_fwd_add_kernel");
+}
+
+}
diff --git a/memotr_amd/functions/clip_ops.py b/memotr_amd/functions/clip_ops.py
--- a/memotr_amd/functions/clip_ops.py
+++ b/memotr_amd/functions/clip_ops.py
@@ -15,7 +15,7 @@
     return (os.environ.get("MEMOTR_FUSED_CLIP_OPS", "1"), os.environ.get("MEMOTR_COLSUM_TALL", "1"),
             os.environ.get("MEMOTR_ATTN_KERNELS", "1"), os.environ.get("MEMOTR_FUSED_LN", "1"),
             os.environ.get("MEMOTR_FUSED_SHIFT_RELU", "1"), os.environ.get("MEMOTR_FUSED_LINEAR_BWD", "1"),
-            os.environ.get("MEMOTR_FUSED_LINEAR_FWD", "1"))
+            os.environ.get("MEMOTR_FUSED_LINEAR_FWD", "1"), os.environ.get("MEMOTR_DEC_LAYER_NODE", "1"))
 
 
 def _lib():
@@ -463,6 +463,47 @@
     return y
 
 
+def linear_bwd_join(g2: torch.Tensor, g2b, y_relu, x2: torch.Tensor, weight: torch.Tensor, need_x=True, need_w=True,
+                    need_b=True, x_add: torch.Tensor = None, gx_into: torch.Tensor = None, gx_also: torch.Tensor = None, gw_into: torch.Tensor = None,
+                    gb_into: torch.Tensor = None, gw_out: torch.Tensor = None, gb_out: torch.Tensor = None):
+    g2 = g2.contiguous()
+    rows, out_f = g2.shape
+    in_f = x2.shape[1]
+    dev = g2.device
+    if g2b is not None:
+        g2b = g2b.contiguous()
+        assert g2b.shape == g2.shape and g2b.dtype == torch.float32
+    need_x = need_x or gx_also is not None
+    need_w = need_w or need_b
+    acc = (1 if gx_into is not None else 0) | (2 if gw_into is not None else 0) | (4 if gb_into is not None else 0)
+    first = lambda *ts: next((t for t in ts if t is not None), None)
+    new = lambda *shape: torch.empty(shape, dtype=torch.float32, device=dev)
+    gx = (gx_into if gx_into is not None else new(rows, in_f)) if need_x else None
+    gw = (first(gw_into, gw_out) if first(gw_into, gw_out) is not None else new(out_f, in_f)) if need_w else None
+    gb = (first(gb_into, gb_out) if first(gb_into, gb_out) is not None else new(out_f)) if need_b else None
+    for t, numel in ((gx, rows * in_f), (gx_also, rows * in_f), (gw, out_f * in_f), (gb, out_f)):
+        assert t is None or (t.is_contiguous() and t.dtype == torch.float32 and t.numel() == numel), \
+            "linear_bwd_join: outputs must be contiguous fp32 buffers of the gradient's size"
+    ptr = lambda t: None if t is None else t.data_ptr()
+    L_ = _lib()
+    L_.check(L_.lib.clipops_linear_bwd_join_f32(g2.data_ptr(), ptr(g2b), ptr(y_relu), x2.data_ptr(), ptr(x_add),
+                                                weight.data_ptr(), rows, in_f, out_f, ptr(gx), ptr(gx_also), ptr(gw),
+                                                ptr(gb), acc, _stream(g2)), "clipops_linear_bwd_join_f32")
+    return gx, gw, gb
+
+
+def linear_fwd_add(x2: torch.Tensor, p2: torch.Tensor, weight: torch.Tensor, bias, relu: bool) -> torch.Tensor:
+    assert p2.shape == x2.shape and p2.dtype == torch.float32 and p2.is_contiguous()
+    rows, in_f = x2.shape
+    out_f = weight.shape[0]
+    y = torch.empty((rows, out_f), dtype=torch.float32, device=x2.device)
+    L_ = _lib()
+    L_.check(L_.lib.clipops_linear_fwd_add_f32(x2.data_ptr(), p2.data_ptr(), weight.data_ptr(),
+                                               None if bias is None else bias.data_ptr(), rows, in_f, out_f,
+                                               1 if relu else 0, y.data_ptr(), _stream(x2)), "clipops_linear_fwd_add_f32")
+    return y
+
+
 def linear_bwd_reference(g2, y_relu, x2, weight):
     if y_relu is not None:
         g2 = g2 * (y_relu > 0).to(g2.dtype)
@@ -511,19 +552,38 @@
 MHA_HEAD_DIM = 32
 
 
+def self_attention_fwd(qk_p: torch.Tensor, v_p: torch.Tensor, key_mask, n_heads: int):
+    B, L, E2 = qk_p.shape
+    E = E2 // 2
+    out = torch.empty((B, L, E), dtype=torch.float32, device=qk_p.device)
+    lse = torch.empty((B, n_heads, L), dtype=torch.float32, device=qk_p.device)
+    scale = 1.0 / (E // n_heads) ** 0.5
+    mk = None if key_mask is None else key_mask.data_ptr()
+    L_ = _lib()
+    L_.check(L_.lib.clipops_mha_fwd_f32(qk_p.data_ptr(), qk_p.data_ptr() + 4 * E, v_p.data_ptr(), L * E2, E2, L * E2,
+                                        E2, L * E, E, mk, B, n_heads, L, scale, out.data_ptr(), lse.data_ptr(),
+                                        _stream(qk_p)), "clipops_mha_fwd_f32")
+    return out, lse, scale
+
+
+def self_attention_bwd(qk_p, v_p, key_mask, out, lse, g, n_heads: int, scale: float):
+    B, L, E2 = qk_p.shape
+    E = E2 // 2
+    g = g.contiguous()
+    g_qk, g_v = torch.empty_like(qk_p), torch.empty_like(v_p)
+    mk = None if key_mask is None else key_mask.data_ptr()
+    L_ = _lib()
+    L_.check(L_.lib.clipops_mha_bwd_f32(qk_p.data_ptr(), qk_p.data_ptr() + 4 * E, v_p.data_ptr(), L * E2, E2, L * E2,
+                                        E2, L * E, E, mk, out.data_ptr(), lse.data_ptr(), g.data_ptr(), B, n_heads,
+                                        L, scale, g_qk.data_ptr(), L * E2, E2, g_qk.data_ptr() + 4 * E, L * E2,
+                                        E2, g_v.data_ptr(), L * E, E, _stream(qk_p)), "clipops_mha_bwd_f32")
+    return g_qk, g_v
+
+
 class _SelfAttention(torch.autograd.Function):
     @staticmethod
     def forward(ctx, qk_p, v_p, key_mask, n_heads):
-        B, L, E2 = qk_p.shape
-        E = E2 // 2
-        out = torch.empty((B, L, E), dtype=torch.float32, device=qk_p.device)
-        lse = torch.empty((B, n_heads, L), dtype=torch.float32, device=qk_p.device)
-        scale = 1.0 / (E // n_heads) ** 0.5
-        mk = None if key_mask is None else key_mask.data_ptr()
-        L_ = _lib()
-        L_.check(L_.lib.clipops_mha_fwd_f32(qk_p.data_ptr(), qk_p.data_ptr() + 4 * E, v_p.data_ptr(), L * E2, E2, L * E2,
-                                            E2, L * E, E, mk, B, n_heads, L, scale, out.data_ptr(), lse.data_ptr(),
-                                            _stream(qk_p)), "clipops_mha_fwd_f32")
+        out, lse, scale = self_attention_fwd(qk_p, v_p, key_mask, n_heads)
         ctx.save_for_backward(qk_p, v_p, key_mask, out, lse)
         ctx.n_heads, ctx.scale = n_heads, scale
         return out
@@ -531,16 +591,7 @@
     @staticmethod
     def backward(ctx, g):
         qk_p, v_p, key_mask, out, lse = ctx.saved_tensors
-        B, L, E2 = qk_p.shape
-        E = E2 // 2
-        g = g.contiguous()
-        g_qk, g_v = torch.empty_like(qk_p), torch.empty_like(v_p)
-        mk = None if key_mask is None else key_mask.data_ptr()
-        L_ = _lib()
-        L_.check(L_.lib.clipops_mha_bwd_f32(qk_p.data_ptr(), qk_p.data_ptr() + 4 * E, v_p.data_ptr(), L * E2, E2, L * E2,
-                                            E2, L * E, E, mk, out.data_ptr(), lse.data_ptr(), g.data_ptr(), B, ctx.n_heads,
-                                            L, ctx.scale, g_qk.data_ptr(), L * E2, E2, g_qk.data_ptr() + 4 * E, L * E2,
-                                            E2, g_v.data_ptr(), L * E, E, _stream(qk_p)), "clipops_mha_bwd_f32")
+        g_qk, g_v = self_attention_bwd(qk_p, v_p, key_mask, out, lse, g, ctx.n_heads, ctx.scale)
         return g_qk, g_v, None, None
 
 
@@ -624,17 +675,22 @@
     @staticmethod
     def backward(ctx, g):
         s, stats, weight = ctx.saved_tensors
-        rows = s.numel() // LN_COLS
-        g = g.contiguous()
-        gs = torch.empty_like(s)
-        chunk = 16 if rows <= 4096 else 64
-        partial = torch.empty((-(-rows // chunk), 2 * LN_COLS), dtype=torch.float32, device=s.device)
-        L = _lib()
-        L.check(L.lib.clipops_add_layer_norm_bwd_f32(g.data_ptr(), s.data_ptr(), stats.data_ptr(), weight.data_ptr(), rows,
-                                                     chunk, gs.data_ptr(), partial.data_ptr(), _stream(s)),
-                "clipops_add_layer_norm_bwd_f32")
-        gwb = colsum(partial)
-        return gs, gs, gwb[:LN_COLS], gwb[LN_COLS:], None
+        gs, gw, gb = add_layer_norm_bwd(g, s, stats, weight)
+        return gs, gs, gw, gb, None
+
+
+def add_layer_norm_bwd(g: torch.Tensor, s: torch.Tensor, stats: torch.Tensor, weight: torch.Tensor):
+    rows = s.numel() // LN_COLS
+    g = g.contiguous()
+    gs = torch.empty_like(s)
+    chunk = 16 if rows <= 4096 else 64
+    partial = torch.empty((-(-rows // chunk), 2 * LN_COLS), dtype=torch.float32, device=s.device)
+    L = _lib()
+    L.check(L.lib.clipops_add_layer_norm_bwd_f32(g.data_ptr(), s.data_ptr(), stats.data_ptr(), weight.data_ptr(), rows,
+                                                 chunk, gs.data_ptr(), partial.data_ptr(), _stream(s)),
+            "clipops_add_layer_norm_bwd_f32")
+    gwb = colsum(partial)
+    return gs, gwb[:LN_COLS], gwb[LN_COLS:]
 
 
 def add_layer_norm_fwd(x: torch.Tensor, res: torch.Tensor, weight: torch.Tensor, bias: torch.Tensor, eps: float,
diff --git a/memotr_amd/functions/decoder_layer.py b/memotr_amd/functions/decoder_layer.py
--- /dev/null
+++ b/memotr_amd/functions/decoder_layer.py
@@ -0,0 +1,123 @@
+from __future__ import annotations
+
+import os
+
+import torch
+from torch.autograd.function import once_differentiable
+
+from . import clip_ops
+
+
+def enabled() -> bool:
+    return os.environ.get("MEMOTR_DEC_LAYER_NODE", "1") != "0"
+
+
+def _plain_fp32(*tensors) -> bool:
+    return all(t is not None and t.is_cuda and t.dtype == torch.float32 for t in tensors)
+
+
+def row_linear_add_usable(x: torch.Tensor, p: torch.Tensor, weight: torch.Tensor, bias) -> bool:
+    if not (enabled() and p is not None and bias is not None and _plain_fp32(x, p, weight, bias) and x.shape == p.shape
+            and torch.is_grad_enabled() and (weight.requires_grad or x.requires_grad or p.requires_grad)
+            and not torch.is_autocast_enabled() and clip_ops.fused(x, p)):
+        return False
+    x2 = x.reshape(-1, x.shape[-1])
+    return (x2.is_contiguous() and p.is_contiguous() and clip_ops.linear_fwd_usable(x2, weight, bias)
+            and weight.shape[0] <= clip_ops.LINEAR_BWD_MAX_OUT and clip_ops.linear_bwd_usable(x2, x2, weight))
+
+
+class RowLinearAdd(torch.autograd.Function):
+    calls = 0
+
+    @staticmethod
+    def forward(ctx, x, p, weight, bias):
+        RowLinearAdd.calls += 1
+        x2, p2 = x.reshape(-1, x.shape[-1]), p.reshape(-1, p.shape[-1])
+        y = clip_ops.linear_fwd_add(x2, p2, weight, bias, False)
+        ctx.save_for_backward(x2, p2, weight)
+        ctx.x_shape = x.shape
+        return y.view(*x.shape[:-1], weight.shape[0])
+
+    @staticmethod
+    @once_differentiable
+    def backward(ctx, g):
+        x2, p2, weight = ctx.saved_tensors
+        need_x = ctx.needs_input_grad[0] or ctx.needs_input_grad[1]
+        gx, gw, gb = clip_ops.linear_bwd_join(g.reshape(-1, g.shape[-1]), None, None, x2, weight, need_x,
+                                              ctx.needs_input_grad[2], ctx.needs_input_grad[3], x_add=p2)
+        gx = None if gx is None else gx.view(ctx.x_shape)
+        return (gx if ctx.needs_input_grad[0] else None), (gx if ctx.needs_input_grad[1] else None), gw, gb
+
+
+def row_linear_add(x: torch.Tensor, p: torch.Tensor, weight: torch.Tensor, bias: torch.Tensor) -> torch.Tensor:
+    return RowLinearAdd.apply(x, p, weight, bias)
+
+
+def self_attn_block_usable(mha, norm, tgt: torch.Tensor, query_pos: torch.Tensor) -> bool:
+    if not (enabled() and query_pos is not None and tgt.dim() == 3 and tgt.shape == query_pos.shape
+            and _plain_fp32(tgt, query_pos) and torch.is_grad_enabled() and not torch.is_autocast_enabled()
+            and mha.batch_first and mha._qkv_same_embed_dim and mha.in_proj_bias is not None and mha.bias_k is None
+            and not mha.add_zero_attn and not (mha.training and mha.dropout > 0)):
+        return False
+    w, b = mha.in_proj_weight, mha.in_proj_bias
+    wo, bo = mha.out_proj.weight, mha.out_proj.bias
+    E, H = mha.embed_dim, mha.num_heads
+    B, L, _ = tgt.shape
+    if not (w.requires_grad and _plain_fp32(w, b, wo, bo) and w.is_contiguous() and b.is_contiguous()
+            and tgt.is_contiguous() and query_pos.is_contiguous() and clip_ops.fused(tgt)
+            and clip_ops.add_layer_norm_supported(tgt, tgt, norm) and E % (2 * H) == 0):
+        return False
+    tgt2 = tgt.view(B * L, E)
+    return (os.environ.get("MEMOTR_ATTN_KERNELS", "1") != "0" and E // H == clip_ops.MHA_HEAD_DIM
+            and 0 < L <= clip_ops.MHA_MAX_L and 2 * E <= clip_ops.LINEAR_BWD_MAX_OUT
+            and clip_ops.linear_fwd_usable(tgt2, wo, bo) and clip_ops.linear_bwd_usable(tgt2, tgt2, wo)
+            and clip_ops.linear_bwd_usable(tgt2, tgt2, w[2 * E:]))
+
+
+class SelfAttnBlockNode(torch.autograd.Function):
+    calls = 0
+
+    @staticmethod
+    def forward(ctx, tgt, pos, key_mask, n_heads, eps, w, b, wo, bo, gamma, beta):
+        SelfAttnBlockNode.calls += 1
+        B, L, E = tgt.shape
+        tgt2, pos2 = tgt.view(B * L, E), pos.view(B * L, E)
+        qk2 = tgt2 + pos2
+        qk_p = torch.addmm(b[:2 * E], qk2, w[:2 * E].t())
+        v_p = torch.addmm(b[2 * E:], tgt2, w[2 * E:].t())
+        del qk2
+        qk_p, v_p = qk_p.view(B, L, 2 * E), v_p.view(B, L, E)
+        attn, lse, scale = clip_ops.self_attention_fwd(qk_p, v_p, key_mask, n_heads)
+        sa = clip_ops.linear_fwd(attn.view(B * L, E), wo, bo, False)
+        s, y, _, stats = clip_ops.add_layer_norm_fwd(tgt, sa.view(B, L, E), gamma, beta, eps)
+        ctx.save_for_backward(tgt2, pos2, key_mask, qk_p, v_p, attn, lse, s, stats, w, wo, gamma)
+        ctx.dims = (B, L, E, int(n_heads), scale)
+        return y
+
+    @staticmethod
+    @once_differentiable
+    def backward(ctx, g_y):
+        tgt2, pos2, key_mask, qk_p, v_p, attn, lse, s, stats, w, wo, gamma = ctx.saved_tensors
+        B, L, E, n_heads, scale = ctx.dims
+        d_sum, g_gamma, g_beta = clip_ops.add_layer_norm_bwd(g_y, s, stats, gamma)
+        d_sum2 = d_sum.view(B * L, E)
+        g_attn, gwo, gbo = clip_ops.linear_bwd(d_sum2, None, attn.view(B * L, E), wo)
+        g_qk, g_v = clip_ops.self_attention_bwd(qk_p, v_p, key_mask, attn, lse, g_attn.view(B, L, E), n_heads, scale)
+        gw, gb = torch.empty_like(w), torch.empty((3 * E,), dtype=w.dtype, device=w.device)
+        clip_ops.linear_bwd_join(g_v.view(B * L, E), None, None, tgt2, w[2 * E:], gx_into=d_sum2, gw_out=gw[2 * E:],
+                                 gb_out=gb[2 * E:])
+        g_pos = None
+        if ctx.needs_input_grad[1]:
+            g_pos = clip_ops.linear_bwd_join(g_qk.view(B * L, 2 * E), None, None, tgt2, w[:2 * E], x_add=pos2,
+                                             gx_also=d_sum2, gw_out=gw[:2 * E], gb_out=gb[:2 * E])[0].view(B, L, E)
+        else:
+            clip_ops.linear_bwd_join(g_qk.view(B * L, 2 * E), None, None, tgt2, w[:2 * E], x_add=pos2, gx_into=d_sum2,
+                                     gw_out=gw[:2 * E], gb_out=gb[:2 * E])
+        return d_sum, g_pos, None, None, None, gw, gb, gwo, gbo, g_gamma, g_beta
+
+
+def self_attn_block(mha, norm, tgt: torch.Tensor, query_pos: torch.Tensor, key_padding_mask) -> torch.Tensor:
+    no_pad = key_padding_mask is None or getattr(key_padding_mask, "_no_padding", False)
+    mask = None if no_pad else key_padding_mask.contiguous()
+    return SelfAttnBlockNode.apply(tgt, query_pos, mask, int(mha.num_heads), float(norm.eps), mha.in_proj_weight,
+                                   mha.in_proj_bias, mha.out_proj.weight, mha.out_proj.bias, norm.weight, norm.bias)
diff --git a/memotr_amd/models/deformable_decoder.py b/memotr_amd/models/deformable_decoder.py
--- a/memotr_amd/models/deformable_decoder.py
+++ b/memotr_amd/models/deformable_decoder.py
@@ -6,6 +6,7 @@
 
 from ..modules import MSDeformAttn
 from ..modules.ms_deform_attn import project_values
+from ..functions import decoder_layer as dec_node
 from ..functions.clip_ops import add_layer_norm, refine_boxes_split
 from ..modules.attention import self_attention
 from ..modules.linear import row_linear
@@ -21,6 +22,8 @@
                  visualize: bool = False):
         super().__init__()
         self.layers = get_clones(module=decoder_layer, n=num_layers)
+        for layer in self.layers:
+            layer.use_checkpoint = use_checkpoint
         self.num_layers = num_layers
         self.return_intermediate = return_intermediate
         self.merge_det_track_layer = merge_det_track_layer
@@ -170,6 +173,7 @@
         self.linear2 = nn.Linear(d_ffn, d_model)
         self.dropout4 = nn.Dropout(dropout)
         self.norm3 = nn.LayerNorm(d_model)
+        self.use_checkpoint = False
         self.extra_track_attn = extra_track_attn
         if extra_track_attn:
             self.track_attn = nn.MultiheadAttention(embed_dim=d_model, num_heads=n_heads, dropout=dropout,
@@ -182,6 +186,8 @@
         return tensor if pos is None else tensor + pos
 
     def forward_self_attn(self, tgt, query_pos, query_mask):
+        if not self.use_checkpoint and dec_node.self_attn_block_usable(self.self_attn, self.norm2, tgt, query_pos):
+            return dec_node.self_attn_block(self.self_attn, self.norm2, tgt, query_pos, query_mask)
         qk = self.with_pos_embed(tgt, query_pos)
         attn = self_attention(self.self_attn, qk, tgt, key_padding_mask=query_mask)
         return add_layer_norm(tgt, self.dropout2(attn), self.norm2)
@@ -216,8 +222,12 @@
         if self.extra_track_attn:
             tgt = self.forward_track_attn(tgt, query_pos, query_mask)
         tgt = self.forward_self_attn(tgt, query_pos, query_mask)
-        cross = self.cross_attn(self.with_pos_embed(tgt, query_pos), reference_points, src, src_spatial_shapes,
-                                level_start_index, src_padding_mask, value)
+        if query_pos is not None and not self.use_checkpoint:
+            cross = self.cross_attn(tgt, reference_points, src, src_spatial_shapes, level_start_index, src_padding_mask,
+                                    value, query_pos=query_pos)
+        else:
+            cross = self.cross_attn(self.with_pos_embed(tgt, query_pos), reference_points, src, src_spatial_shapes,
+                                    level_start_index, src_padding_mask, value)
         tgt = add_layer_norm(tgt, self.dropout1(cross), self.norm1)
         tgt = self.forward_ffn(tgt)
         if track_tgt is not None:
diff --git a/memotr_amd/modules/ms_deform_attn.py b/memotr_amd/modules/ms_deform_attn.py
--- a/memotr_amd/modules/ms_deform_attn.py
+++ b/memotr_amd/modules/ms_deform_attn.py
@@ -140,15 +140,23 @@
         xavier_uniform_(self.output_proj.weight.data)
         constant_(self.output_proj.bias.data, 0.0)
 
+    def _query_projection(self, query, query_pos=None):
+        w, b = self._fused_query_projection()
+        if query_pos is None:
+            return long_linear(query, w, b)
+        from ..functions import decoder_layer
+        if decoder_layer.row_linear_add_usable(query, query_pos, w, b):
+            return decoder_layer.row_linear_add(query, query_pos, w, b)
+        return long_linear(query + query_pos, w, b)
+
     def _forward_projected(self, query, reference_points, pv: "ProjectedValue", input_spatial_shapes,
-                           input_level_start_index):
+                           input_level_start_index, query_pos=None):
         M, P = self.n_heads, self.n_points
         site = self.__dict__.get("_msda_site")
         if site is None:
             site = self.__dict__["_msda_site"] = MSDA.new_call_site()
         MSDA.set_call_site(site)
-        w, b = self._fused_query_projection()
-        proj = long_linear(query, w, b)
+        proj = self._query_projection(query, query_pos)
         if reference_points.shape[-1] not in (2, 4):
             raise ValueError("Last dim of reference_points must be 2 or 4, but get {} instead.".format(
                 reference_points.shape[-1]))
@@ -209,13 +217,13 @@
         return new
 
     def forward(self, query, reference_points, input_flatten, input_spatial_shapes, input_level_start_index,
-                input_padding_mask=None, value: "ProjectedValue" = None):
+                input_padding_mask=None, value: "ProjectedValue" = None, query_pos=None):
         N, Lq, _ = query.shape
         S = input_flatten.shape[1]
         M, L, P = self.n_heads, self.n_levels, self.n_points
         if value is not None:
             return self._forward_projected(query, reference_points, value, input_spatial_shapes,
-                                           input_level_start_index)
+                                           input_level_start_index, query_pos)
         if input_flatten.is_cuda:
             site = self.__dict__.get("_msda_site")
             if site is None:
@@ -235,8 +243,7 @@
         value = long_linear(input_flatten, self.value_proj.weight, self.value_proj.bias, activation=zero)
 
         n_off = M * L * P * 2
-        w, b = self._fused_query_projection()
-        proj = long_linear(query, w, b)
+        proj = self._query_projection(query, query_pos)
         if proj.dtype == torch.bfloat16:
             proj = proj.float()
             reference_points = reference_points.float()
```

Result: no change. 42.20 (median of 2 runs) (+0.3%).
